# nyrahealth/CrisperWhisper

Measured on AMD Instinct MI355X. Metric: aligned words/s (RTF alongside), CrisperWhisper large-v3 geometry, 30 s chunks, full mel->encoder->decoder->DTW->words path, higher is better.
Workload: dtype bf16

## Files before the change

### crisperwhisper_amd/_native.py

```python
from __future__ import annotations

import ctypes as C
import os

_HERE = os.path.dirname(os.path.abspath(__file__))
LIB_PATH = os.environ.get("CW_LIB_PATH") or os.path.join(_HERE, "libcrisperwhisper.so")

CW_DTYPE_F32, CW_DTYPE_BF16, CW_DTYPE_F16 = 0, 1, 2
N_SAMPLES, N_FRAMES, N_CTX = 480000, 3000, 1500
STAGES = ("mel", "encoder", "cross_kv", "decode", "timestamps")
ALIGN_HEADS_MAX_BYTES = 8 << 30


class NativeLibraryError(RuntimeError):
    pass


class ModelDesc(C.Structure):
    _fields_ = [(n, C.c_int32) for n in (
        "d_model", "n_heads", "ffn_dim", "enc_layers", "dec_layers", "n_mels", "vocab_size",
        "max_target_positions", "median_filter_width", "dtype", "max_batch", "n_align")] + [
        ("align_layers", C.POINTER(C.c_int32)), ("align_heads", C.POINTER(C.c_int32))]


# ... 73 lines not shown
    "cw_get_top_logprobs": (_I, [_P, _P, _P, _I]),
    "cw_get_transcribe_top_logprobs": (_I, [_P, _P, _P, _I, _I]),
    "cw_set_sequence_bias": (_I, [_P, _I, _P, _P, _P]),
    "cw_get_logits": (_I, [_P, _P, _I]),
    "cw_set_logits_capture": (_I, [_P, _P, _I]),
    "cw_get_alignment": (_I, [_P, _P, _I, _I]),
    "cw_resampled_length": (C.c_int64, [C.c_int64, _I, _I]),
    "cw_ingest": (_I, [_P, _P, _I, _I, C.c_int64, _I, _I, _I, _P]),
    "cw_resample_taps": (_I, [_I, _I, _P, _I, _P, _P, _P]),
    "cw_flac_info": (_I, [_P, C.c_int64, _P, _P, _P, _P]),
    "cw_flac_decode": (_I, [_P, C.c_int64, _P, C.c_int64, _P]),
    "cw_flac_last_error": (C.c_char_p, []),
    "cw_token_timestamps": (_I, [_P, _I, _I, _I, _P, _P]),
    "cw_beam_begin": (_I, [_P, _I, _I, _P, _I, _I, _I]),
    "cw_beam_step": (_I, [_P, _I, _P, _P]),
    "cw_beam_advance": (_I, [_P, _P, _P]),
    "cw_beam_finish": (_I, [_P, _I, _I, _P]),
    "cw_transcribe": (_I, [_P, _I, _P, C.POINTER(TranscribeCfg), _P, _P, _P, _I, _P]),
    "cw_transcribe_prompted": (_I, [_P, _I, _P, C.POINTER(TranscribeCfg), _P, _I, _P, _P, _P, _I, _P]),
    "cw_align_tokens": (_I, [_P, _I, _P, _P, _I, _P, _I, _P]),
    "cw_align_prefill_runs": (_I, [_P]),
    "cw_align_heads": (_I, [_P, _I, _P, _P, _I, _P, _I, _I, _P, _P, _P, _P, _P, _I, _P]),
    "cw_align_heads_times": (_I, [_P, _P]),
    "cw_test_align_similarity": (_I, [_P, _P, _I, _I, _I, _I, _P, _P, _P, _I, _P]),
    "cw_set_alignment_scores": (_I, [_P, _I, _I]),
    "cw_get_alignment_scores": (_I, [_P, _P, _P, _I, _I]),
    "cw_get_transcribe_alignment_scores": (_I, [_P, _P, _P, _I, _I]),
    "cw_test_align_path_scores": (_I, [_P, _P, _I, _I, _I, _I, _P, _P, _I, _P, _P]),
    "cw_score_tokens": (_I, [_P, _I, _I, _P, _I, _P, _I, _P, _P, _P]),
    "cw_align_score_tokens": (_I, [_P, _I, _P, _P, _I, _P, _I, _P, _P, _P, _P]),
    "cw_align_cut_tokens": (_I, [_P, _I, _P, _P, _I, _P, _I, _P, _P, _P, _P, _P, _P, _P, _P, _P]),
    "cw_test_score_head_stop": (_I, [_P, _I, _I, _I, _P, _P, _P, _P, _P, _I, _I, _P, _P, _P, _P]),
    "cw_test_align_cut": (_I, [_P, _I, _I, _P, _P, _P, _P, _P, _P, _P]),
    "cw_score_prefill_runs": (_I, [_P]),
    "cw_set_score_top_logprobs": (_I, [_P, _I]),
    "cw_get_score_top_logprobs": (_I, [_P, _P, _P, _I, _I]),
    "cw_test_score_head_top": (_I, [_P, _I, _I, _I, _P, _P, _P, _P, _P, _I, _P, _P, _P, _P, _P, _P]),
    "cw_test_score_head_stop_top": (_I, [_P, _I, _I, _I, _P, _P, _P, _P, _P, _I, _I, _I, _P, _P, _P, _P, _P, _P, _P]),
    "cw_test_score_rows_top": (_I, [_P, _I, _I, _I, _P, _P, _I, _I, _I, _P, _P, _P, _P, _P, _P]),
    "cw_time_score_head_top": (_I, [_P, _I, _I, _I, _I, _P]),
    "cw_align_matrix": (_I, [_P, _P, _I, _I, _I, _I, _P, _I, _P]),
    "cw_dtw": (_I, [_P, _P, _I, _I, _P, _P, _P]),
    "cw_adjust_pauses": (_I, [_P, _P, _P, _I, C.c_double]),
    "cw_vocab_create": (_P, [_I, _P, _P, _P, _P, _I, _I, _I, _I, _I]),
    "cw_vocab_destroy": (None, [_P]),
    "cw_collate_begin": (_P, [_P, C.c_double]),
    "cw_beam_host_new": (_P, [_I, _I, _I, _I, _I, _I, _I, C.c_double, _I, _P]),
    "cw_beam_host_step": (_I, [_P, _P, _P, _P, _P]),
    "cw_beam_host_result": (_I, [_P, _P, _P, _P]),
    "cw_beam_host_token_logprobs": (_I, [_P, _P]),
    "cw_beam_host_free": (None, [_P]),
    "cw_collate_set_mode": (_I, [_P, _I]),
    "cw_collate_feed": (_I, [_P, _P, _I, _P, _I, _I, C.c_double, C.c_double, C.c_double]),
    "cw_collate_finish": (_I, [_P, _P, _P, _P, _P]),
    "cw_collate_get": (_I, [_P, _P, _P, _P, _P, _P]),
    "cw_collate_token_groups_total": (C.c_int64, [_P]),
    "cw_collate_get_token_groups": (_I, [_P, _P, _P]),
    "cw_collate_get_languages": (_I, [_P, _P]),
    "cw_collate_free": (None, [_P]),
    "cw_set_option": (_I, [_P, C.c_char_p, _I]),
    "cw_test_set_option": (_I, [C.c_char_p, _I]),
    "cw_test_gemm": (_I, [_P, _I, _I, _I, _P, _P, _P, _I, _P]),
    "cw_test_gemm_fp8": (_I, [_P, _I, _I, _I, _P, _P, _P, _I, _P]),
    "cw_test_gemm_epi": (_I, [_P, C.POINTER(GemmEpiArgs)]),
    "cw_test_rownorm": (_I, [_P, _I, _I, _I, _P, _P, _P, _P, _P, _P]),
    "cw_test_gemv": (_I, [_P, _I, _I, _I, _P, _P, _P, _P, _P, _I, _P]),
    "cw_has_experiments": (_I, []),
    "cw_test_skinny": (_I, [_P, _I, _I, _I, _I, _P, _P, _P, _I, _I, _P, _P]),
    "cw_test_attention": (_I, [_P, _I, _I, _I, _P, _P, _P, _P]),
    "cw_test_cross_attention": (_I, [_P, _I, _I, _I, _I, _P, _P, _P, _I, _P, _P, _P, _P]),
    "cw_test_cross_attention_fused": (_I, [_P, _I, _I, _I, _I, _P, _P, _P, _P, _P, _I, _P, _P, _I, _P, _P, _P, _P]),
    "cw_test_fold": (_I, [_P, C.POINTER(FoldArgs)]),
    "cw_test_gemv_stack": (_I, [_P, C.POINTER(GemvStackArgs)]),
    "cw_test_gemv_epi": (_I, [_P, C.POINTER(GemvEpiArgs)]),
    "cw_test_self_attention": (_I, [_P, _I, _I, _I, _I, _P, _P, _P, _P, _I, _P, _I, _I, _I, _I, _P, _P, _P]),
    "cw_test_beam_state": (_I, [_P, _I, _P, _P, _P]),
    "cw_test_prefill_gemm": (_I, [_P, _I, _I, _I, _I, _P, _P, _P, _P]),
    "cw_test_prefill_attention": (_I, [_P, _I, _I, _I, _I, _I, _I, _I, _P, _P, _P, _P]),
    "cw_test_prefill_align_attention": (_I, [_P, _I, _I, _I, _I, _I, _I, _P, _P, _P, _P, _P]),
    "cw_test_score_head": (_I, [_P, _I, _I, _I, _P, _P, _P, _P, _P, _P, _P, _P]),
    "cw_time_score_head": (_I, [_P, _I, _I, _I, _P]),
    "cw_test_beam_topk": (_I, [_P, _I, _P, _P, _I, _I, _I, _I, _P, _P]),
    "cw_test_beam_x": (_I, [_P, _I, _P]),
    "cw_test_sample": (_I, [_P, _I, _P, _P, _I, _I, _I, _I, _P]),
    "cw_test_sample_seeded": (_I, [_P, _I, _P, _P, _I, _I, _I, _I, C.c_float, C.c_uint64, _P, _P]),
    "cw_test_sample_logprobs": (_I, [_P, _I, _P, _P, _I, _I, _I, _I, C.c_float, C.c_uint64, _P, _P, _P, _P]),
    "cw_test_sample_top_logprobs": (_I, [_P, _I, _P, _P, _I, _I, _I, _I, C.c_float, C.c_uint64, _P, _P, _I, _P, _P, _P, _P]),
    "cw_test_sample_biased": (_I, [_P, _I, _P, _P, _I, _I, _I, _I, C.c_float, C.c_uint64, _P, _P, _I, _I, _P, _P, _P, _P, _P, _P, _P, _P]),
    "cw_stage_times": (_I, [_P, _P, _P, _I]),
    "cw_time_kernel": (_I, [_P, _I, _I, _I, _P, _P]),
    "cw_time_decode_stage": (_I, [_P, _I, _I, _I, _P, _P, _P, _P]),
    "cw_decode_stage_name": (C.c_char_p, [_I]),
    "cw_handoff_fallbacks": (_I, [_P]),
    "cw_handoff_resumes": (_I, [_P]),
    "cw_decode_stage_launches": (_I, [_P, _I]),
}

_lib = None


def exported_symbols():
    return sorted(_SIGS)


def load():
    global _lib
    if _lib is not None:
        return _lib
    if not os.path.exists(LIB_PATH):
        raise NativeLibraryError(
            f"{LIB_PATH} not found: build it with `python -c 'import __graft_entry__ as g; g.build()'` "
            "or `make -C crisperwhisper_amd/csrc` (hipcc, gfx950).  There is no CPU fallback.")
    try:
        lib = C.CDLL(LIB_PATH)
    except OSError as e:
        raise NativeLibraryError(f"cannot load {LIB_PATH}: {e}") from e
    for name, (res, args) in _SIGS.items():
        try:
            fn = getattr(lib, name)
        except AttributeError as e:
            raise NativeLibraryError(f"{LIB_PATH} does not export {name}") from e
        fn.restype = res
        fn.argtypes = args
    _lib = lib
    return lib
```

### crisperwhisper_amd/csrc/decfuse.hip

```cpp
#include "common.h"
#include "kernels.h"

namespace CW_NS {

typedef __attribute__((ext_vector_type(4))) unsigned int u32x4_t;
__device__ static inline f32x4_t mfma16x(bf16x8_t a, bf16x8_t b, f32x4_t c) { return cw_mfma_16x16x32(a, b, c); }

__global__ __launch_bounds__(256) void fold_product_kernel(const float* __restrict__ A, const float* __restrict__ s,
                                                           float scale, const float* __restrict__ B, int N, int J, int K,
                                                           bf16_t* __restrict__ C) {
    __shared__ float As[16][65];
    __shared__ float Bs[16][64];
    const int tid = threadIdx.x, tx = tid & 15, ty = tid >> 4;
    const int n0 = blockIdx.y * 64, k0 = blockIdx.x * 64;
    float acc[4][4] = {};
    for (int j0 = 0; j0 < J; j0 += 16) {
#pragma unroll
        for (int i = 0; i < 4; ++i) {
            const int idx = tid + 256 * i;
            const int n = idx >> 4, j = idx & 15;
            As[j][n] = A[(size_t)(n0 + n) * J + j0 + j] * (s ? s[j0 + j] : 1.0f) * scale;
            const int jb = idx >> 6, k = idx & 63;
            Bs[jb][k] = B[(size_t)(j0 + jb) * K + k0 + k];
        }
// ... 203 lines not shown
        const int r = tid >> 6;
        const float v = red[((0 * NT + t) * 4 + r) * 64 + lane] + red[((1 * NT + t) * 4 + r) * 64 + lane] +
                        red[((2 * NT + t) * 4 + r) * 64 + lane] + red[((3 * NT + t) * 4 + r) * 64 + lane];
        const int m = g * 4 + r, n = nloc[t];
        if (m < Mb && n >= 0) {
            const size_t o = (size_t)m * ldo + n;
            const float back = wsum ? smean[m] * wsum_v[t] : 0.f;
            if (epi == 0) {
                out[o] = v + bias_v[t] + back;
            } else if (epi == 2) {
                atomicAdd(out + o, v + bias_v[t] + back);
            } else {
                const float rv = resid_pre[t] + resid_grid(v + bias_v[t]);
                out[o] = rv;
                if (out2) out2[o] = rv;
                ps1 += rv; ps2 += rv * rv;
            }
        }
    }
    if (epi == 1 && pstats) {
#pragma unroll
        for (int sft = 0; sft < 4; ++sft) {
            ps1 += sft == 0 ? dpp_mov<0x111, 0xf>(0.f, ps1) : sft == 1 ? dpp_mov<0x112, 0xf>(0.f, ps1) : sft == 2 ? dpp_mov<0x114, 0xf>(0.f, ps1) : dpp_mov<0x118, 0xf>(0.f, ps1);
            ps2 += sft == 0 ? dpp_mov<0x111, 0xf>(0.f, ps2) : sft == 1 ? dpp_mov<0x112, 0xf>(0.f, ps2) : sft == 2 ? dpp_mov<0x114, 0xf>(0.f, ps2) : dpp_mov<0x118, 0xf>(0.f, ps2);
        }
        const int m = g * 4 + (tid >> 6);
        if (l15 == 15) *(float2*)(pstats + ((size_t)(bid - block0) * 16 + m) * 2) = make_float2(ps1, ps2);
    }
}

template <int RPW, int NT>
static int launch_stack_nt(StackParams& p, hipStream_t st) {
    int blocks = 0;
    for (int s = 0; s < p.nseg; ++s) {
        if (p.seg[s].nt <= 0 || p.seg[s].nt > NT) p.seg[s].nt = NT;
        p.seg[s].block0 = blocks;
        blocks += (p.seg[s].n_tiles + p.seg[s].nt - 1) / p.seg[s].nt;
    }
    if (p.zero && (long long)blocks * 256 < p.zero_n4) return CW_ERR_INVALID;
    const size_t lds = (size_t)16 * (p.K + 8) * 2 + (size_t)4 * NT * 4 * 64 * 4 + 16 * 4;
    const dim3 grid(blocks, (p.Mb + 15) / 16);
    if (p.K > 0xffff || p.Mb > 0xff || blocks > 0xffff) return CW_ERR_INVALID;
#define CW_STACK_LEAD(p)                                                                                                     \
    (p).W, (p).zero, (p).zero_n4, (unsigned)(p).K | (unsigned)(p).Mb << 16 | (unsigned)(p).nseg << 24 | ((p).wpk ? 1u << 26 : 0u), \
        (unsigned)((p).nseg > 1 ? (p).seg[1].block0 : 0) | (unsigned)((p).nseg > 2 ? (p).seg[2].block0 : 0) << 16, (p)
    if (p.K <= 256) hipLaunchKernelGGL((gemv_stack_kernel<RPW, 1, 1, NT>), grid, dim3(256), lds, st, CW_STACK_LEAD(p));
    else if (p.K <= 768) hipLaunchKernelGGL((gemv_stack_kernel<RPW, 2, 3, NT>), grid, dim3(256), lds, st, CW_STACK_LEAD(p));
    else {
        bool uni = p.wpk != 0;
        for (int s = 0; s < p.nseg; ++s) uni = uni && p.seg[s].nt == NT;
        if (uni && p.wnt && grid.y == 1) hipLaunchKernelGGL((gemv_stack_kernel<RPW, 3, 5, NT, true, true>), grid, dim3(256), lds, st, CW_STACK_LEAD(p));
        else if (uni) hipLaunchKernelGGL((gemv_stack_kernel<RPW, 3, 5, NT, true>), grid, dim3(256), lds, st, CW_STACK_LEAD(p));
        else hipLaunchKernelGGL((gemv_stack_kernel<RPW, 3, 5, NT>), grid, dim3(256), lds, st, CW_STACK_LEAD(p));
    }
#undef CW_STACK_LEAD
    return CW_OK;
}

int cw_launch_gemv_stack(const StackParams& p_in, int nt, hipStream_t st) {
    StackParams p = p_in;
    if (p.Mb < 1 || p.Mb > 64 || p.K % 128 || p.K > 1280 || p.nseg < 1 || p.nseg > 3) return CW_ERR_INVALID;
    if (nt <= 0) {
        nt = 1;
        for (;;) {
            int blocks = 0;
            for (int s = 0; s < p.nseg; ++s) {
                const int snt = p.seg[s].nt > 0 && p.seg[s].nt < nt ? p.seg[s].nt : nt;
                blocks += (p.seg[s].n_tiles + snt - 1) / snt;
            }
            if (blocks <= 256 || nt == 3) break;
            ++nt;
        }
    }
    if (p.Mb > 8) {
        if (nt == 1) return launch_stack_nt<4, 1>(p, st);
        if (nt == 2) return launch_stack_nt<4, 2>(p, st);
        return launch_stack_nt<4, 3>(p, st);
    }
    if (nt == 1) return launch_stack_nt<2, 1>(p, st);
    if (nt == 2) return launch_stack_nt<2, 2>(p, st);
    return launch_stack_nt<2, 3>(p, st);
}

#ifdef CW_EXPERIMENTS
#include "decfuse_experiments.inc"
#else
int cw_launch_gemv_fc2x(const Fc2xParams&, hipStream_t) { return CW_ERR_INVALID; }
int cw_launch_mlp_pair(const MlpPairParams&, hipStream_t) { return CW_ERR_INVALID; }
int cw_launch_rows_prep(const float*, int, int, void*, float*, int, hipStream_t) { return CW_ERR_INVALID; }
int cw_launch_gemv_rows(int, bool, const RowsParams&, hipStream_t) { return CW_ERR_INVALID; }
#endif

}
```

### crisperwhisper_amd/csrc/declayer.hip

```cpp
#include "common.h"
#include "kernels.h"
#include <mutex>

namespace CW_NS {

typedef __attribute__((ext_vector_type(4))) unsigned int dl_u32x4_t;
typedef unsigned long long dl_u64_t;

#define DL_THREADS 1024
#define DL_SPIN_LIMIT (1 << 17)

#if defined(CW_PHASE_TIMING) && !defined(CW_F16)
__device__ unsigned long long g_dl_phase[256 * 3 * 16];
#define DLPH(i)                                                                                                     \
    do {                                                                                                            \
        if ((threadIdx.x & 63) == 0 && blockIdx.x < 256) {                                                          \
            const int w_ = threadIdx.x >> 6;                                                                        \
            if (w_ == 0 || w_ == 4 || w_ == 8) g_dl_phase[(blockIdx.x * 3 + (w_ >> 2)) * 16 + (i)] = wall_clock64(); \
        }                                                                                                           \
    } while (0)
extern "C" int cw_debug_dl_phases(unsigned long long* out) {
    return (int)hipMemcpyFromSymbol(out, HIP_SYMBOL(g_dl_phase), sizeof(unsigned long long) * 256 * 3 * 16);
}
#define DLPHV(i, v)                                                                                                 \
// ... 324 lines not shown
                    }
                }
            }
#pragma unroll
            for (int r = 0; r < 4; ++r) red[(wave * 4 + r) * 64 + lane] = acc[r];
        }
        dl_chain_sync(cb, 2, lane);
        DLPH(6);
        {
            const int r = wave;
            const float v = red[(0 * 4 + r) * 64 + lane] + red[(1 * 4 + r) * 64 + lane] + red[(2 * 4 + r) * 64 + lane] + red[(3 * 4 + r) * 64 + lane];
            const int m = g * 4 + r;
            float ps1 = 0.f, ps2 = 0.f;
            if (m < Mb) {
                const size_t o = (size_t)m * K + ncl;
                const float back = wsum ? smean[m] * wsum_v : 0.f;
                if (si < 2) {
                    dl_gran_st(p.gq + ((size_t)si * 16 + m) * K + ncl, tag, __float_as_uint(v + bias_v + back));
                } else {
                    const float rv = resid_v + resid_grid(v + bias_v);
                    p.x1[o] = rv;
                    ps1 += rv; ps2 += rv * rv;
                }
            }
            if (si == 2) {
#pragma unroll
                for (int sft = 0; sft < 4; ++sft) {
                    ps1 += sft == 0 ? dpp_mov<0x111, 0xf>(0.f, ps1) : sft == 1 ? dpp_mov<0x112, 0xf>(0.f, ps1) : sft == 2 ? dpp_mov<0x114, 0xf>(0.f, ps1) : dpp_mov<0x118, 0xf>(0.f, ps1);
                    ps2 += sft == 0 ? dpp_mov<0x111, 0xf>(0.f, ps2) : sft == 1 ? dpp_mov<0x112, 0xf>(0.f, ps2) : sft == 2 ? dpp_mov<0x114, 0xf>(0.f, ps2) : dpp_mov<0x118, 0xf>(0.f, ps2);
                }
                if (l15 == 15) {
                    dl_gran_st(p.gps + ((size_t)tl * 16 + m) * 2, tag, __float_as_uint(ps1));
                    dl_gran_st(p.gps + ((size_t)tl * 16 + m) * 2 + 1, tag, __float_as_uint(ps2));
                }
            }
        }
    }
    DLPH(7);
    {
        const size_t col = (size_t)qh * 64 + lane;
        const dl_u64_t* ga = p.gq + ((size_t)0 * 16 + qb_row) * K + col;
        const dl_u64_t* gb = p.gq + ((size_t)1 * 16 + qb_row) * K + col;
        const dl_u64_t* g0 = p.gps + ((size_t)min(lane, TD - 1) * 16 + qb_row) * 2;
        const dl_u64_t* g1 = p.gps + ((size_t)min(lane + 64, TD - 1) * 16 + qb_row) * 2;
        dl_u64_t va = 0, vb = 0, v00 = 0, v01 = 0, v10 = 0, v11 = 0;
        bool ready = !q_mine;
        int npoll = 0; (void)npoll;
#pragma unroll 1
        for (int spins = 0; !ready; ++spins) {
            if (spins > DL_SPIN_LIMIT) { if (lane == 0) atomicCAS(p.err, 0, 1); break; }
            va = dl_gran_ld(ga); vb = dl_gran_ld(gb);
            v00 = dl_gran_ld(g0); v01 = dl_gran_ld(g0 + 1);
            v10 = dl_gran_ld(g1); v11 = dl_gran_ld(g1 + 1);
            const bool ok = (unsigned)(va >> 32) == tag && (unsigned)(vb >> 32) == tag && (unsigned)(v00 >> 32) == tag &&
                            (unsigned)(v01 >> 32) == tag && (unsigned)(v10 >> 32) == tag && (unsigned)(v11 >> 32) == tag;
            ready = __all(ok); ++npoll;
            if (spins == 0) DLPH(8);
        }
        if (q_mine) {
            const float qa1 = __uint_as_float((unsigned)va), qb1 = __uint_as_float((unsigned)vb);
            const float inv_d = 1.0f / (float)(H * 64);
            const float ps1 = (lane < TD ? __uint_as_float((unsigned)v00) : 0.f) + (lane + 64 < TD ? __uint_as_float((unsigned)v10) : 0.f);
            const float ps2 = (lane < TD ? __uint_as_float((unsigned)v01) : 0.f) + (lane + 64 < TD ? __uint_as_float((unsigned)v11) : 0.f);
            const float mean = wave_sum(ps1) * inv_d;
            const float var = fmaxf(wave_sum(ps2) * inv_d - mean * mean, 0.f);
            const float rstd = 1.0f / sqrtf(var + 1e-5f);
            c_q[wave * 64 + lane] = ((qa1 + qb1) - mean * qw1) * rstd + qc1;
        }
        DLPHV(13, npoll);
    }
    DLPH(9);
    dl_barrier();
    DLPH(10);
#pragma unroll
    for (int idx = 0; idx < 16; ++idx) {
        const uint4 t = *(const uint4*)(kvL + ((size_t)(wave * 16 + idx) * 64 + lane) * 16);
        if ((idx >> 2) & 1) vr[idx >> 3][idx & 3].a = t; else kr[idx >> 3][idx & 3].a = t;
    }
    dl_cross_items(p, it, kr, vr, grp, gw, gt, lane, c_q, c_smax, c_redl, c_red);
}
#undef DL_KV_LOAD
#endif

#define QS_THREADS 512
#define QS_GROUPS (QS_THREADS / 8)
#define QS_PRE 2

template <int NSLOT, int PER_LANE, bool WNT>
__global__ __launch_bounds__(QS_THREADS) void qkv_self_kernel(const float* __restrict__ x, const void* __restrict__ Wp,
                                                              const float* __restrict__ bias, void* sk, void* sv,
                                                              const int* __restrict__ pos, unsigned dims, int cap, QkvSelfParams p) {
    extern __shared__ __attribute__((aligned(16))) unsigned char qsm[];
    const int Mb = (int)(dims & 0xffu), H = (int)((dims >> 8) & 0xffu), K = (int)(dims >> 16), N = 3 * K;
    const int xs_stride = K + 8;
    bf16_t* xs = (bf16_t*)qsm;
    float* red = (float*)(qsm + (size_t)16 * xs_stride * 2);
    float* s_q = red + 4 * 4 * 64;
    bf16_t* s_kn = (bf16_t*)(s_q + 64);
    bf16_t* s_vn = s_kn + 64;
    float* dsm = (float*)(s_vn + 64);
    const int tid = threadIdx.x, lane = tid & 63;
    const int wave = __builtin_amdgcn_readfirstlane(tid >> 6);
    const int l15 = lane & 15, g = lane >> 4;
    const int bid = blockIdx.x;
    const int n0 = bid * 16;
    const int steps = K >> 7, nvec = K >> 2;
    const int nn = n0 + l15, ncl = nn < N ? nn : N - 1;

    const int n_items = Mb * H;
    const bool has_item = bid < n_items;
    const int ih = has_item ? bid % H : 0, ib = has_item ? bid / H : 0;
    const int sub = tid & 7, grp = tid >> 3;
    const bf16_t* Kh = (const bf16_t*)sk + ((size_t)ib * H + ih) * cap * 64;
    const bf16_t* Vh = (const bf16_t*)sv + ((size_t)ib * H + ih) * cap * 64;

    float bias_v = 0.f;
    int pos_m = 0;
    float4 xv[2][PER_LANE];
    dl_u32x4_t wq[NSLOT][4];
    if (wave < 4) {
        pos_m = pos[min(g * 4 + wave, Mb - 1)];
        bias_v = bias ? bias[ncl] : 0.f;
#pragma unroll
        for (int i = 0; i < 2; ++i) {
            int row = wave + 4 * i;
            row = row < Mb ? row : Mb - 1;
#pragma unroll
            for (int c = 0; c < PER_LANE; ++c) {
                int v4 = lane + 64 * c;
                v4 = v4 < nvec ? v4 : nvec - 1;
                xv[i][c] = *(const float4*)(x + (size_t)row * K + v4 * 4);
            }
        }
        const bf16_t* __restrict__ W = (const bf16_t*)Wp;
#pragma unroll
        for (int s = 0; s < NSLOT; ++s) {
            int step = wave + 4 * s;
            step = step < steps ? step : steps - 1;
            const dl_u32x4_t* wp = (const dl_u32x4_t*)(W + ((((size_t)(ncl >> 4) * (K >> 5)) + step * 4) * 64 + g * 16 + (ncl & 15)) * 8);
#pragma unroll
            for (int j = 0; j < 4; ++j) wq[s][j] = WNT ? CW_STREAM_LD(wp + j * 64) : wp[j * 64];
        }
    }
    __builtin_amdgcn_sched_barrier(0);
    DlRaw8 kpre[QS_PRE], vpre[QS_PRE];
#pragma unroll
    for (int u = 0; u < QS_PRE; ++u) kpre[u].ld(Kh + (size_t)min(grp + u * QS_GROUPS, cap - 1) * 64 + sub * 8);
#pragma unroll
    for (int u = 0; u < QS_PRE; ++u) vpre[u].ld(Vh + (size_t)min(grp + u * QS_GROUPS, cap - 1) * 64 + sub * 8);
    const int n_keys = pos[ib] + 1;
    const int pos0 = pos[0];
    __builtin_amdgcn_sched_barrier(0);
    const unsigned tag = (p.epoch[0] << 6) | (unsigned)p.layer;
    asm volatile("" : "+v"(pos_m));

    if (wave < 4) {
#pragma unroll
        for (int i = 0; i < 2; ++i) {
            float sx = 0.f;
#pragma unroll
            for (int c = 0; c < PER_LANE; ++c) {
                const float ok = (lane + 64 * c < nvec) ? 1.f : 0.f;
                sx += ok * ((xv[i][c].x + xv[i][c].y) + (xv[i][c].z + xv[i][c].w));
            }
            const float mean = wave_sum(sx) / (float)K;
            float q = 0.f;
#pragma unroll
            for (int c = 0; c < PER_LANE; ++c) {
                const float ok = (lane + 64 * c < nvec) ? 1.f : 0.f;
                const float a = xv[i][c].x - mean, b = xv[i][c].y - mean, cc = xv[i][c].z - mean, d = xv[i][c].w - mean;
                q += ok * cw_sumsq4(a, b, cc, d);
            }
            const float rstd = 1.0f / sqrtf(wave_sum(q) / (float)K + 1e-5f);
            const int row = wave + 4 * i;
#pragma unroll
            for (int c = 0; c < PER_LANE; ++c) {
// ... 52 lines not shown
        const dl_u64_t* gkp = p.gkv + ((size_t)(lane >> 5) * 16 + ib) * (K >> 1) + ih * 32 + (lane & 31);
        dl_u64_t vq = 0, vk = 0;
        bool ready = false;
        const int give_up_tag = pos0 + 1;
        const bool forced_fail = p.fail_pos >= 0 && pos0 == p.fail_pos && p.layer == 0;
#pragma unroll 1
        for (int spins = 0; !ready; ++spins) {
            if (forced_fail || spins > DL_SPIN_LIMIT || ((spins & 255) == 255 && __hip_atomic_load(p.err, __ATOMIC_RELAXED, __HIP_MEMORY_SCOPE_AGENT) != 0)) {
                if (lane == 0) atomicCAS(p.err, 0, give_up_tag);
                if (forced_fail) { vq = 0x3f800000ull; vk = 0; }
                break;
            }
            vq = dl_gran_ld(gqp); vk = dl_gran_ld(gkp);
            ready = __all((unsigned)(vq >> 32) == tag && (unsigned)(vk >> 32) == tag);
        }
        s_q[lane] = __uint_as_float((unsigned)vq);
        ((unsigned*)s_kn)[lane] = (unsigned)vk;
    }
    dl_barrier();
    float* sc = dsm;
    float* redd = dsm + ((cap + 63) & ~63);
    float* scratch = redd + QS_GROUPS * 64;
    float qv[8];
#pragma unroll
    for (int e = 0; e < 8; ++e) qv[e] = s_q[sub * 8 + e];
    const int kn = n_keys - 1;
    const uint4 kn_raw = *(const uint4*)(s_kn + sub * 8), vn_raw = *(const uint4*)(s_vn + sub * 8);
#pragma unroll
    for (int u = 0; u < QS_PRE; ++u)
        if (grp + u * QS_GROUPS == kn) { kpre[u].a = kn_raw; vpre[u].a = vn_raw; }

    if (n_keys <= QS_PRE * QS_GROUPS) {
        float* s_max = scratch;
        float* red8 = redd;
        float d[QS_PRE], mxl = -INFINITY;
#pragma unroll
        for (int u = 0; u < QS_PRE; ++u) {
            float kv[8];
            kpre[u].cvt(kv);
            float t = 0.f;
#pragma unroll
            for (int e = 0; e < 8; ++e) t = fmaf(qv[e], kv[e], t);
            t += __shfl_xor(t, 1, 64); t += __shfl_xor(t, 2, 64); t += __shfl_xor(t, 4, 64);
            d[u] = (grp + u * QS_GROUPS < n_keys) ? t : -INFINITY;
            mxl = fmaxf(mxl, d[u]);
        }
        mxl = wave_max(mxl);
        if (lane == 0) s_max[wave] = mxl;
        dl_barrier();
        mxl = s_max[0];
#pragma unroll
        for (int w = 1; w < QS_THREADS / 64; ++w) mxl = fmaxf(mxl, s_max[w]);
        float acc[8] = {};
        float lsum = 0.f;
#pragma unroll
        for (int u = 0; u < QS_PRE; ++u) {
            if (grp + u * QS_GROUPS < n_keys) {
                const float pk = expf(d[u] - mxl);
                if (sub == 0) lsum += pk;
                float vv[8];
                vpre[u].cvt(vv);
#pragma unroll
                for (int e = 0; e < 8; ++e) acc[e] = fmaf(pk, vv[e], acc[e]);
            }
        }
#pragma unroll
        for (int e = 0; e < 8; ++e) {
            float v = acc[e] + dpp_mov<0x128, 0xf>(0.f, acc[e]);
            acc[e] = xor32_sum(xor16_sum(v));
        }
        lsum = wave_sum(lsum);
        if (lane < 8) {
#pragma unroll
            for (int e = 0; e < 8; ++e) red8[wave * 64 + sub * 8 + e] = acc[e];
        }
        if (lane == 0) red8[8 * 64 + wave] = lsum;
        dl_barrier();
        if (tid < 64) {
            float r = 0.f, l = 0.f;
#pragma unroll
            for (int w = 0; w < QS_THREADS / 64; ++w) { r += red8[w * 64 + tid]; l += red8[8 * 64 + w]; }
            r *= 1.0f / l;
            p.out[(size_t)ib * H * 64 + ih * 64 + tid] = r;
        }
        return;
    }

    float mx = -INFINITY;
#pragma unroll
    for (int u = 0; u < QS_PRE; ++u) {
        const int k = grp + u * QS_GROUPS;
        float kv[8];
        kpre[u].cvt(kv);
        float d = 0.f;
#pragma unroll
        for (int e = 0; e < 8; ++e) d = fmaf(qv[e], kv[e], d);
        d += __shfl_xor(d, 1, 64); d += __shfl_xor(d, 2, 64); d += __shfl_xor(d, 4, 64);
        if (k < n_keys) {
            if (sub == 0) sc[k] = d;
            mx = fmaxf(mx, d);
        }
    }
    for (int k0 = grp + QS_PRE * QS_GROUPS; k0 < n_keys; k0 += 4 * QS_GROUPS) {
        float kv[4][8];
#pragma unroll
        for (int u = 0; u < 4; ++u) {
            const int k = min(k0 + u * QS_GROUPS, n_keys - 1);
            uint4 raw = *(const uint4*)(Kh + (size_t)k * 64 + sub * 8);
            if (k == kn) raw = kn_raw;
            h16_unpack8(raw, kv[u]);
        }
#pragma unroll
        for (int u = 0; u < 4; ++u) {
            const int k = k0 + u * QS_GROUPS;
            if (k < n_keys) {
                float d = 0.f;
#pragma unroll
                for (int e = 0; e < 8; ++e) d = fmaf(qv[e], kv[u][e], d);
                d += __shfl_xor(d, 1, 64); d += __shfl_xor(d, 2, 64); d += __shfl_xor(d, 4, 64);
                if (sub == 0) sc[k] = d;
                mx = fmaxf(mx, d);
            }
        }
    }
    mx = block_max(mx, scratch);
    float sum = 0.f;
    for (int k = tid; k < n_keys; k += QS_THREADS) { float e = expf(sc[k] - mx); sc[k] = e; sum += e; }
    sum = block_sum(sum, scratch);
    const float inv = 1.0f / sum;
    float acc[8] = {};
#pragma unroll
    for (int u = 0; u < QS_PRE; ++u) {
        const int k = grp + u * QS_GROUPS;
        float vv[8];
        vpre[u].cvt(vv);
        const float pk = (k < n_keys) ? sc[k] * inv : 0.f;
        if (k < n_keys) {
#pragma unroll
            for (int e = 0; e < 8; ++e) acc[e] = fmaf(pk, vv[e], acc[e]);
        }
    }
    for (int k0 = grp + QS_PRE * QS_GROUPS; k0 < n_keys; k0 += 4 * QS_GROUPS) {
        float vv[4][8];
#pragma unroll
        for (int u = 0; u < 4; ++u) {
            const int k = min(k0 + u * QS_GROUPS, n_keys - 1);
            uint4 raw = *(const uint4*)(Vh + (size_t)k * 64 + sub * 8);
            if (k == kn) raw = vn_raw;
            h16_unpack8(raw, vv[u]);
        }
#pragma unroll
        for (int u = 0; u < 4; ++u) {
            const int k = k0 + u * QS_GROUPS;
            if (k < n_keys) {
                const float pk = sc[k] * inv;
#pragma unroll
                for (int e = 0; e < 8; ++e) acc[e] = fmaf(pk, vv[u][e], acc[e]);
            }
        }
    }
#pragma unroll
    for (int e = 0; e < 8; ++e) redd[grp * 64 + sub * 8 + e] = acc[e];
    __syncthreads();
    if (tid < 64) {
        float r = 0.f;
        for (int gI = 0; gI < QS_GROUPS; ++gI) r += redd[gI * 64 + tid];
        p.out[(size_t)ib * H * 64 + ih * 64 + tid] = r;
    }
}

int cw_qkv_self_blocks_per_cu(int D, int cap) {
    const size_t lds = (size_t)16 * (D + 8) * 2 + (size_t)(4 * 4 * 64 + 64) * 4 + 2 * 64 * 2 + ((size_t)((cap + 63) & ~63) + QS_GROUPS * 64 + 64) * 4;
    const int by_lds = (int)((size_t)160 * 1024 / lds), by_threads = 2048 / QS_THREADS;
    return by_lds < by_threads ? by_lds : by_threads;
}

int cw_launch_qkv_self(const QkvSelfParams& p, hipStream_t st) {
    const int D = p.D;
    if (p.Mb < 1 || p.Mb > 8 || D % 128 || D > 1280 || p.H * 64 != D || p.cap < 1 || p.cap > 512) return CW_ERR_INVALID;
    if (p.Mb * p.H > 3 * (D / 16) || !p.gq || !p.gkv || !p.epoch || !p.err || !p.W || !p.x || !p.pos) return CW_ERR_INVALID;
    if (p.layer < 0 || p.layer >= 64) return CW_ERR_INVALID;
    const size_t lds = (size_t)16 * (D + 8) * 2 + (size_t)(4 * 4 * 64 + 64) * 4 + 2 * 64 * 2 +
                       ((size_t)((p.cap + 63) & ~63) + QS_GROUPS * 64 + 64) * 4;
    const dim3 grid(3 * (D / 16));
#define QS_LAUNCH_P(NS, PL, NTL)                                                                                            \
    do {                                                                                                                     \
        static std::once_flag attr;                                                                                          \
        std::call_once(attr, [] { (void)hipFuncSetAttribute((const void*)qkv_self_kernel<NS, PL, NTL>, hipFuncAttributeMaxDynamicSharedMemorySize, 100 * 1024); }); \
        hipLaunchKernelGGL((qkv_self_kernel<NS, PL, NTL>), grid, dim3(QS_THREADS), lds, st, p.x, p.W, p.bias, p.sk, p.sv, p.pos, \
                           (unsigned)p.Mb | (unsigned)p.H << 8 | (unsigned)D << 16, p.cap, p);                                \
    } while (0)
#define QS_LAUNCH(NS, PL) do { if (p.wnt) QS_LAUNCH_P(NS, PL, true); else QS_LAUNCH_P(NS, PL, false); } while (0)
    if (D <= 256) QS_LAUNCH(1, 1);
    else if (D <= 768) QS_LAUNCH(2, 3);
    else QS_LAUNCH(3, 5);
#undef QS_LAUNCH
#undef QS_LAUNCH_P
    return CW_OK;
}

#ifdef CW_EXPERIMENTS
template <int NS1, int PL1, int NS2>
__global__ __launch_bounds__(256) void mlp_chain_kernel(MlpChainParams p) {
    extern __shared__ __attribute__((aligned(16))) unsigned char msm[];
    const int tid = threadIdx.x, lane = tid & 63;
    const int wave = __builtin_amdgcn_readfirstlane(tid >> 6);
    const int l15 = lane & 15, g = lane >> 4;
    const int D = p.D, F = p.F, Mb = p.Mb;
    const int n1 = F >> 5;
    const unsigned tag = (p.epoch[0] << 6) | (unsigned)p.layer;
    const int bid = blockIdx.x;
    constexpr int NT = 2;
    if (bid < n1) {
        DLPH(0);
        const int K = D, N = F;
        const int xs_stride = K + 8;
        bf16_t* xs = (bf16_t*)msm;
        float* red = (float*)(msm + (size_t)16 * xs_stride * 2);
        const int n0 = bid * 16 * NT;
        const int steps = K >> 7, nvec = K >> 2;
        int nn[NT], ncl[NT];
#pragma unroll
        for (int t = 0; t < NT; ++t) { nn[t] = n0 + t * 16 + l15; ncl[t] = nn[t] < N ? nn[t] : N - 1; }
        float bias_v[NT];
#pragma unroll
        for (int t = 0; t < NT; ++t) bias_v[t] = p.b1 ? p.b1[ncl[t]] : 0.f;
        float4 xv[2][PL1];
#pragma unroll
        for (int i = 0; i < 2; ++i) {
            int row = wave + 4 * i;
            row = row < Mb ? row : Mb - 1;
#pragma unroll
            for (int c = 0; c < PL1; ++c) {
                int v4 = lane + 64 * c;
                v4 = v4 < nvec ? v4 : nvec - 1;
                xv[i][c] = *(const float4*)(p.x + (size_t)row * K + v4 * 4);
            }
        }
        dl_u32x4_t wq[NT][NS1][4];
        const bf16_t* __restrict__ W = (const bf16_t*)p.W1;
#pragma unroll
        for (int t = 0; t < NT; ++t) {
#pragma unroll
            for (int s = 0; s < NS1; ++s) {
                int step = wave + 4 * s;
                step = step < steps ? step : steps - 1;
                const dl_u32x4_t* wp = (const dl_u32x4_t*)(W + ((((size_t)(ncl[t] >> 4) * (K >> 5)) + step * 4) * 64 + g * 16 + (ncl[t] & 15)) * 8);
#pragma unroll
                for (int j = 0; j < 4; ++j) wq[t][s][j] = wp[j * 64];
            }
        }
        DLPH(1);
#pragma unroll
        for (int i = 0; i < 2; ++i) {
            float sx = 0.f;
#pragma unroll
            for (int c = 0; c < PL1; ++c) {
                const float ok = (lane + 64 * c < nvec) ? 1.f : 0.f;
                sx += ok * ((xv[i][c].x + xv[i][c].y) + (xv[i][c].z + xv[i][c].w));
            }
            const float mean = wave_sum(sx) / (float)K;
            float q = 0.f;
#pragma unroll
            for (int c = 0; c < PL1; ++c) {
                const float ok = (lane + 64 * c < nvec) ? 1.f : 0.f;
                const float a = xv[i][c].x - mean, b = xv[i][c].y - mean, cc = xv[i][c].z - mean, d = xv[i][c].w - mean;
                q += ok * cw_sumsq4(a, b, cc, d);
            }
            const float rstd = 1.0f / sqrtf(wave_sum(q) / (float)K + 1e-5f);
#pragma unroll
            for (int c = 0; c < PL1; ++c) {
                xv[i][c].x = (xv[i][c].x - mean) * rstd; xv[i][c].y = (xv[i][c].y - mean) * rstd;
                xv[i][c].z = (xv[i][c].z - mean) * rstd; xv[i][c].w = (xv[i][c].w - mean) * rstd;
            }
        }
// ... 229 lines not shown
```

### crisperwhisper_amd/csrc/engine.hip

```cpp
#include "engine_internal.h"

static thread_local char g_err[512] = "";

int fail(cw_ctx* c, int code, const char* fmt, ...) {
    va_list ap;
    va_start(ap, fmt);
    vsnprintf(c ? c->err : g_err, 512, fmt, ap);
    va_end(ap);
    if (c) c->err_set = true;
    return code;
}
int fail_ctx(cw_ctx* c, int code, const char* call, const char* file, int line) {
    if (c && c->err_set) return code;
    return fail(c, code, "%s -> %d (%s:%d)", call, code, file, line);
}

int upload_T(cw_ctx* c, void* dst, size_t off, const float* src, size_t n, float scale) {
    if (c->bf16) {
        std::vector<bf16_t> tmp(n);
        if (c->f16) for (size_t i = 0; i < n; ++i) tmp[i] = cw_host_f32_to_f16(src[i] * scale);
        else for (size_t i = 0; i < n; ++i) tmp[i] = cw_host_f32_to_bf16(src[i] * scale);
        HIPCHK(c, hipMemcpy((bf16_t*)dst + off, tmp.data(), n * 2, hipMemcpyHostToDevice));
    } else if (scale != 1.0f) {
        std::vector<float> tmp(n);
// ... 52 lines not shown
#pragma unroll
                for (int u = 0; u < 8; ++u) v[u] = *(const unsigned int*)(base + ((s + u * nthr) << 6));
#pragma unroll
                for (int u = 0; u < 8; ++u) acc ^= v[u];
            }
            for (; s < sectors; s += nthr) acc ^= *(const unsigned int*)(base + (s << 6));
        }
    }
    if (acc == 0x9e3779b9u && sink) *sink = acc;
}


#endif

extern "C" {

int32_t cw_abi_version(void) { return 1; }

const char* cw_last_error(cw_ctx* ctx) {
    if (!ctx) return g_err;
    ctx->err_set = false;
    return ctx->err;
}

int32_t cw_sync(cw_ctx* c) {
    HIPCHK(c, hipStreamSynchronize(c->st));
    return CW_OK;
}

static int create_impl(cw_ctx* c) {
    const cw_model_desc& d = c->d;
    const int D = d.d_model, H = d.n_heads, F = d.ffn_dim, V = d.vocab_size, Bm = d.max_batch;
    if (D != H * 64) return fail(c, CW_ERR_INVALID, "head_dim must be 64 (d_model=%d heads=%d)", D, H);
    if (D % 128 || F % 128 || d.n_mels % 64) return fail(c, CW_ERR_INVALID, "d_model/ffn must be multiples of 128, n_mels of 64");
    if (Bm < 1 || Bm > 64) return fail(c, CW_ERR_INVALID, "max_batch must be in 1..64");
    if (d.max_target_positions > 512) return fail(c, CW_ERR_INVALID, "max_target_positions > 512 unsupported");
    HIPCHK(c, hipSetDevice(c->device));
    HIPCHK(c, hipStreamCreate(&c->st));
    HIPCHK(c, hipEventCreate(&c->ev0));
    HIPCHK(c, hipEventCreate(&c->ev1));
    HIPCHK(c, hipEventCreateWithFlags(&c->ev_step[0], hipEventDisableTiming));
    HIPCHK(c, hipEventCreateWithFlags(&c->ev_step[1], hipEventDisableTiming));
#ifdef CW_EXPERIMENTS
    HIPCHK(c, hipStreamCreateWithFlags(&c->st2, hipStreamNonBlocking));
    HIPCHK(c, hipEventCreateWithFlags(&c->ev_pf[0], hipEventDisableTiming));
    HIPCHK(c, hipEventCreateWithFlags(&c->ev_pf[1], hipEventDisableTiming));
#endif
    HIPCHK(c, hipHostMalloc((void**)&c->h_nunf, 2 * 1024 * sizeof(int), hipHostMallocDefault));
    if (d.dtype != CW_DTYPE_F32 && d.dtype != CW_DTYPE_BF16 && d.dtype != CW_DTYPE_F16) return fail(c, CW_ERR_INVALID, "unknown dtype %d", d.dtype);
    c->f16 = d.dtype == CW_DTYPE_F16;
    c->bf16 = d.dtype == CW_DTYPE_BF16 || c->f16;
    const cw_sw::Switches sw = cw_sw::read_switches();
#ifndef CW_EXPERIMENTS
    {
        const struct { const char* name; bool set; } rejected[] = {{"CW_ROWS_LN", sw.rows_ln}, {"CW_FUSE_MLP", sw.fuse_mlp}, {"CW_MLP_PAIR", sw.mlp_pair},
                                                                   {"CW_SKINNY", sw.skinny != 0}, {"CW_PREFETCH", sw.prefetch != 0},
                                                                   {"CW_DECLAYER", sw.declayer}, {"CW_MLP_CHAIN", sw.mlp_chain}};
        for (const auto& r : rejected)
            if (r.set)
                return fail(c, CW_ERR_INVALID, "%s selects a measured-and-rejected kernel variant that is not in this build: make EXTRA=-DCW_EXPERIMENTS", r.name);
    }
#endif
    c->use_graph = !sw.no_graph;
    c->fuse_rows = !sw.no_fuse_rows;
    c->fuse_rows8 = !sw.no_fuse_rows8;
    c->fuse_beam = !sw.no_fuse_beam;
    c->own_cols = !sw.no_own_cols;
    c->short_hist_enabled = !sw.no_short_hist;
    c->fold_enabled = !sw.no_ln_fold;
    c->fuse6_enabled = !sw.no_fuse6;
    c->rows_ln_enabled = sw.rows_ln;
    c->rows_hilo = !sw.no_rows_hilo;
    c->skinny_mode = sw.skinny;
    c->stack_center = !sw.no_stack_center;
    c->mid16 = !sw.no_mid16;
    c->dtw_block = sw.dtw_block;
    c->fuse_mlp = sw.fuse_mlp;
    c->wpack_enabled = !sw.no_wpack;
    c->wnt = !sw.no_wnt;
    c->mlp_pair = sw.mlp_pair;
    c->mlp_pair_fence = sw.mlp_pair_fence;
    c->declayer = sw.declayer;
    c->qkv_self = !sw.no_qkv_self;
    c->mlp_chain = sw.mlp_chain;
    c->stack_nt3 = sw.stack_nt3;
    c->stack_nt5 = sw.stack_nt5;
    c->prefetch = sw.prefetch;
    c->esz = c->bf16 ? 2 : 4;
    c->Bm = Bm;
    c->S_pad = 1536;
    const size_t e = c->esz;
    const int TGT = d.max_target_positions;

    CWCHK(c, dmalloc(c, &c->conv1_w, (size_t)D * 3 * d.n_mels * e));
    CWCHK(c, dmalloc(c, &c->conv2_w, (size_t)D * 3 * D * e));
    CWCHK(c, dmalloc(c, &c->conv1_b, (size_t)D * 4));
    CWCHK(c, dmalloc(c, &c->conv2_b, (size_t)D * 4));
    CWCHK(c, dmalloc(c, &c->enc_pos, (size_t)CW_N_CTX * D * 4));
    CWCHK(c, dmalloc(c, &c->dec_pos, (size_t)TGT * D * 4));
    CWCHK(c, dmalloc(c, &c->embed, (size_t)V * D * e));
    CWCHK(c, dmalloc(c, &c->enc_ln_g, D * 4)); CWCHK(c, dmalloc(c, &c->enc_ln_b, D * 4));
    CWCHK(c, dmalloc(c, &c->dec_ln_g, D * 4)); CWCHK(c, dmalloc(c, &c->dec_ln_b, D * 4));
    c->enc.resize(d.enc_layers);
    c->dec.resize(d.dec_layers);
    auto alloc_common = [&](LayerW& L, bool stacked) -> int {
        CWCHK(c, dmalloc(c, &L.wqkv, (size_t)3 * D * D * e)); CWCHK(c, dmalloc(c, &L.bqkv, (size_t)3 * D * 4));
        if (!stacked) CWCHK(c, dmalloc(c, &L.wo, (size_t)D * D * e));
        CWCHK(c, dmalloc(c, &L.bo, D * 4));
        CWCHK(c, dmalloc(c, &L.ln1_g, D * 4)); CWCHK(c, dmalloc(c, &L.ln1_b, D * 4));
        if (!stacked) CWCHK(c, dmalloc(c, &L.w1, (size_t)F * D * e));
        CWCHK(c, dmalloc(c, &L.b1, F * 4));
        CWCHK(c, dmalloc(c, &L.w2, (size_t)D * F * e)); CWCHK(c, dmalloc(c, &L.b2, D * 4));
        CWCHK(c, dmalloc(c, &L.ln2_g, D * 4)); CWCHK(c, dmalloc(c, &L.ln2_b, D * 4));
        return CW_OK;
    };
    for (auto& L : c->enc) CWCHK(c, alloc_common(L, false));
    for (auto& L : c->dec) {
        const bool stacked = c->bf16;
        CWCHK(c, alloc_common(L, stacked));
        if (stacked) {
            CWCHK(c, dmalloc(c, &L.ws3, (size_t)3 * D * D * e));
            CWCHK(c, dmalloc(c, &L.ws5, ((size_t)2 * F + D) * D * e));
            L.wq_c = L.ws3; L.wo = (char*)L.ws3 + (size_t)2 * D * D * e;
            L.w1 = L.ws5;   L.wo_c = (char*)L.ws5 + (size_t)2 * F * D * e;
            CWCHK(c, dmalloc(c, &L.qa_bias, D * 4)); CWCHK(c, dmalloc(c, &L.q_wsum, D * 4));
            CWCHK(c, dmalloc(c, &L.u1_bias, F * 4)); CWCHK(c, dmalloc(c, &L.u1_wsum, F * 4));
            CWCHK(c, dmalloc(c, &L.qkv_wsum, (size_t)3 * D * 4));
        } else {
            CWCHK(c, dmalloc(c, &L.wq_c, (size_t)D * D * e));
            CWCHK(c, dmalloc(c, &L.wo_c, (size_t)D * D * e));
        }
        CWCHK(c, dmalloc(c, &L.bq_c, D * 4));
        CWCHK(c, dmalloc(c, &L.wkv_c, (size_t)2 * D * D * e)); CWCHK(c, dmalloc(c, &L.bkv_c, (size_t)2 * D * 4));
        CWCHK(c, dmalloc(c, &L.bo_c, D * 4));
        CWCHK(c, dmalloc(c, &L.lnc_g, D * 4)); CWCHK(c, dmalloc(c, &L.lnc_b, D * 4));
        CWCHK(c, dmalloc(c, &L.ck, (size_t)Bm * H * CW_N_CTX * 64 * e));
        CWCHK(c, dmalloc(c, &L.cv, (size_t)Bm * H * CW_N_CTX * 64 * e));
        CWCHK(c, dmalloc(c, &L.sk, (size_t)Bm * H * TGT * 64 * e));
        CWCHK(c, dmalloc(c, &L.sv, (size_t)Bm * H * TGT * 64 * e));
    }

    {
        std::vector<double> ct(400), sn(400), win(400);
        for (int i = 0; i < 400; ++i) {
            ct[i] = cos(2.0 * M_PI * i / 400.0);
            sn[i] = sin(2.0 * M_PI * i / 400.0);
            win[i] = (double)(float)(0.5 - 0.5 * cos(2.0 * M_PI * i / 400.0));
        }
        double *dct, *dsn, *dwin;
        CWCHK(c, dmalloc(c, &dct, 400 * 8)); CWCHK(c, dmalloc(c, &dsn, 400 * 8)); CWCHK(c, dmalloc(c, &dwin, 400 * 8));
        HIPCHK(c, hipMemcpy(dct, ct.data(), 400 * 8, hipMemcpyHostToDevice));
        HIPCHK(c, hipMemcpy(dsn, sn.data(), 400 * 8, hipMemcpyHostToDevice));
        HIPCHK(c, hipMemcpy(dwin, win.data(), 400 * 8, hipMemcpyHostToDevice));
        const int nm = d.n_mels, nb = 201;
        auto hz2mel = [](double f) { return f >= 1000.0 ? 15.0 + log(f / 1000.0) * (27.0 / log(6.4)) : 3.0 * f / 200.0; };
        auto mel2hz = [](double m) { return m >= 15.0 ? 1000.0 * exp((log(6.4) / 27.0) * (m - 15.0)) : 200.0 * m / 3.0; };
        std::vector<double> ff(nm + 2);
        const double m_lo = hz2mel(0.0), m_hi = hz2mel(8000.0);
        for (int i = 0; i < nm + 2; ++i) {
            double step = (m_hi - m_lo) / (nm + 1);
            double mv = (i == nm + 1) ? m_hi : m_lo + step * i;
            ff[i] = mel2hz(mv);
        }
        std::vector<float> fb((size_t)nb * nm);
        for (int k = 0; k < nb; ++k) {
            double fk = (k == nb - 1) ? 8000.0 : (8000.0 / (nb - 1)) * k;
            for (int m = 0; m < nm; ++m) {
                double down = -(ff[m] - fk) / (ff[m + 1] - ff[m]);
                double up = (ff[m + 2] - fk) / (ff[m + 2] - ff[m + 1]);
                double v = fmax(0.0, fmin(down, up));
                v *= 2.0 / (ff[m + 2] - ff[m]);
                fb[(size_t)k * nm + m] = (float)v;
            }
        }
        float* dfb;
        CWCHK(c, dmalloc(c, &dfb, fb.size() * 4));
        HIPCHK(c, hipMemcpy(dfb, fb.data(), fb.size() * 4, hipMemcpyHostToDevice));
        c->mel.cos_t = dct; c->mel.sin_t = dsn; c->mel.window = dwin; c->mel.filters = dfb;
        {
            std::vector<int> lo(nm, nb), hi(nm, -1);
            for (int m = 0; m < nm; ++m)
                for (int k = 0; k < nb; ++k)
                    if (fb[(size_t)k * nm + m] != 0.f) { if (k < lo[m]) lo[m] = k; if (k > hi[m]) hi[m] = k; }
            int *dlo, *dhi;
            CWCHK(c, dmalloc(c, &dlo, nm * 4)); CWCHK(c, dmalloc(c, &dhi, nm * 4));
            HIPCHK(c, hipMemcpy(dlo, lo.data(), nm * 4, hipMemcpyHostToDevice));
            HIPCHK(c, hipMemcpy(dhi, hi.data(), nm * 4, hipMemcpyHostToDevice));
            c->mel.fb_lo = dlo; c->mel.fb_hi = dhi;
        }
    }
    CWCHK(c, dmalloc(c, &c->d_pcm, (size_t)Bm * CW_N_SAMPLES * 4));
    CWCHK(c, dmalloc(c, &c->d_logspec, (size_t)Bm * CW_N_FRAMES * d.n_mels * 4));
    CWCHK(c, dmalloc(c, &c->d_gmax, Bm * 4));
    CWCHK(c, dmalloc(c, &c->d_feats_tm, (size_t)Bm * CW_N_FRAMES * d.n_mels * e));
    c->n_frames_items.assign(Bm, CW_N_FRAMES);

    const size_t MR = (size_t)Bm * CW_N_CTX;
    CWCHK(c, dmalloc(c, &c->c1, (size_t)Bm * CW_N_FRAMES * D * e));
    CWCHK(c, dmalloc(c, &c->x, MR * D * 4));
    CWCHK(c, dmalloc(c, &c->h, MR * D * e));
    CWCHK(c, dmalloc(c, &c->ao, MR * D * e));
    CWCHK(c, dmalloc(c, &c->enc_out, MR * D * e));
    CWCHK(c, dmalloc(c, &c->mid, MR * F * e));
    CWCHK(c, dmalloc(c, &c->qb, (size_t)Bm * H * c->S_pad * 64 * e));
    CWCHK(c, dmalloc(c, &c->kb, (size_t)Bm * H * c->S_pad * 64 * e));
    CWCHK(c, dmalloc(c, &c->vb, (size_t)Bm * H * c->S_pad * 64 * e));
    CWCHK(c, dmalloc(c, &c->d_row_off, Bm * 4)); CWCHK(c, dmalloc(c, &c->d_row_valid, Bm * 4));
    CWCHK(c, dmalloc(c, &c->d_row_off2, Bm * 4)); CWCHK(c, dmalloc(c, &c->d_row_valid2, Bm * 4));
    {
        std::vector<int> off2(Bm), val2(Bm, CW_N_FRAMES);
        for (int i = 0; i < Bm; ++i) off2[i] = i * CW_N_FRAMES;
        HIPCHK(c, hipMemcpy(c->d_row_off2, off2.data(), Bm * 4, hipMemcpyHostToDevice));
        HIPCHK(c, hipMemcpy(c->d_row_valid2, val2.data(), Bm * 4, hipMemcpyHostToDevice));
    }

    CWCHK(c, dmalloc(c, &c->dx, (size_t)Bm * D * 4)); CWCHK(c, dmalloc(c, &c->dxn, (size_t)Bm * D * 4));
    CWCHK(c, dmalloc(c, &c->dq, (size_t)Bm * D * 4)); CWCHK(c, dmalloc(c, &c->dattn, (size_t)Bm * D * 4));
    CWCHK(c, dmalloc(c, &c->dmid, (size_t)Bm * F * 4));
    CWCHK(c, dmalloc(c, &c->dx1, (size_t)Bm * D * 4)); CWCHK(c, dmalloc(c, &c->dx2c, (size_t)Bm * D * 4));
    CWCHK(c, dmalloc(c, &c->d_qa, (size_t)2 * Bm * D * 4)); c->d_qb = c->d_qa + (size_t)Bm * D;
    CWCHK(c, dmalloc(c, &c->d_u1, (size_t)Bm * F * 4)); CWCHK(c, dmalloc(c, &c->d_pstats, (size_t)128 * 64 * 2 * 4));
    CWCHK(c, dmalloc(c, &c->d_rstats, (size_t)((D > F ? D : F) / 16 + 1) * 64 * 2 * 4));
    CWCHK(c, dmalloc(c, &c->d_bar, 64 * 4));
    {
        CWCHK(c, dmalloc(c, &c->d_gq, (size_t)2 * 16 * D * 8)); CWCHK(c, dmalloc(c, &c->d_gps, (size_t)(D / 16) * 16 * 2 * 8));
        CWCHK(c, dmalloc(c, &c->d_gq2, (size_t)16 * D * 8)); CWCHK(c, dmalloc(c, &c->d_gkv, (size_t)2 * 16 * (D / 2) * 8));
        CWCHK(c, dmalloc(c, &c->d_gflag, (size_t)512 * 8));
        CWCHK(c, dmalloc(c, &c->d_epoch, 4));
        const unsigned int one = 1;
        HIPCHK(c, hipMemcpy(c->d_epoch, &one, 4, hipMemcpyHostToDevice));
        hipDeviceProp_t prop;
        HIPCHK(c, hipGetDeviceProperties(&prop, c->device));
        c->n_cu = prop.multiProcessorCount;
    }
    CWCHK(c, dmalloc(c, &c->d_xfrag, (size_t)64 * 5120 * 2));
#ifdef CW_EXPERIMENTS
    if (Bm > 16) {
        c->planes_cap = (size_t)4 * 64 * (3 * D > F ? 3 * D : F);
        CWCHK(c, dmalloc(c, &c->d_planes, c->planes_cap * 4, false));
        CWCHK(c, dmalloc(c, &c->d_sk_stats, (size_t)16 * 64 * 2 * 4));
    }
#endif
    CWCHK(c, dmalloc(c, &c->d_xfrag2, (size_t)64 * 5120 * 2));
    CWCHK(c, dmalloc(c, &c->d_cvec, 64 * 4)); CWCHK(c, dmalloc(c, &c->d_ostats, (size_t)96 * 64 * 2 * 4));
    c->Vpad = (V + 3) & ~3;
    CWCHK(c, dmalloc(c, &c->dlogits, (size_t)Bm * c->Vpad * 4));
    CWCHK(c, dmalloc(c, &c->d_ids, (size_t)Bm * TGT * 4)); CWCHK(c, dmalloc(c, &c->d_forced, (size_t)Bm * TGT * 4));
    CWCHK(c, dmalloc(c, &c->d_argmax, (size_t)Bm * TGT * 4));
    CWCHK(c, dmalloc(c, &c->d_last_ts, Bm * 4)); CWCHK(c, dmalloc(c, &c->d_finished, Bm * 4));
    CWCHK(c, dmalloc(c, &c->d_nunf, 8));
    c->d_err = c->d_nunf + 1;
#ifdef CW_EXPERIMENTS
    CWCHK(c, dmalloc(c, &c->d_pf_sink, 4));
#endif
    CWCHK(c, dmalloc(c, &c->d_pos, 64 * 4)); CWCHK(c, dmalloc(c, &c->d_cfg, 4 * 4));
    CWCHK(c, dmalloc(c, &c->d_mask, (size_t)V + 16));
    CWCHK(c, dmalloc(c, &c->d_sample_part, (size_t)Bm * 16 * 32));
    CWCHK(c, dmalloc(c, &c->d_sample_pert, (size_t)Bm * 16 * 16));
    CWCHK(c, dmalloc(c, &c->d_samp, (size_t)(4 + 2 * Bm) * 4));
    c->samp_host.assign((size_t)4 + 2 * Bm, 0u);
    CWCHK(c, dmalloc(c, &c->d_lp_sum, (size_t)Bm * 4)); CWCHK(c, dmalloc(c, &c->d_lp_cnt, (size_t)Bm * 4));
    CWCHK(c, dmalloc(c, &c->d_align_slot, (size_t)d.dec_layers * H * 4));
    {
        std::vector<int> slot((size_t)d.dec_layers * H, -1);
        for (int a = 0; a < d.n_align; ++a) {
            int l = c->align_layers[a], hh = c->align_heads[a];
            if (l < 0 || l >= d.dec_layers || hh < 0 || hh >= H) return fail(c, CW_ERR_INVALID, "bad alignment head (%d,%d)", l, hh);
            slot[(size_t)l * H + hh] = a;
        }
        HIPCHK(c, hipMemcpy(c->d_align_slot, slot.data(), slot.size() * 4, hipMemcpyHostToDevice));
    }
    const int Ha = d.n_align > 0 ? d.n_align : 1;
    c->align_rows = TGT;
    CWCHK(c, dmalloc(c, &c->d_align, (size_t)Bm * Ha * TGT * CW_N_CTX * 4));
    CWCHK(c, dmalloc(c, &c->d_part_o, (size_t)ATT_NS * Bm * D * 4));
    CWCHK(c, dmalloc(c, &c->d_part_ml, (size_t)Bm * H * ATT_NS * 2 * 4));
    CWCHK(c, dmalloc(c, &c->d_align_ml, (size_t)Bm * Ha * TGT * ATT_NS * 2 * 4));

    CWCHK(c, dmalloc(c, &c->d_mean, (size_t)Bm * Ha * CW_N_CTX * 4));
    CWCHK(c, dmalloc(c, &c->d_std, (size_t)Bm * Ha * CW_N_CTX * 4));
    CWCHK(c, dmalloc(c, &c->d_mat, (size_t)Bm * TGT * CW_N_CTX * 4));
    CWCHK(c, dmalloc(c, &c->d_trace, (size_t)Bm * TGT * CW_N_CTX));
    CWCHK(c, dmalloc(c, &c->d_first_col, (size_t)Bm * TGT * 4));
    CWCHK(c, dmalloc(c, &c->d_path_text, (size_t)Bm * (TGT + CW_N_CTX + 2) * 4));
    CWCHK(c, dmalloc(c, &c->d_path_time, (size_t)Bm * (TGT + CW_N_CTX + 2) * 4));
    CWCHK(c, dmalloc(c, &c->d_path_len, Bm * 4));
    CWCHK(c, dmalloc(c, &c->d_ncols, Bm * 4));
    HIPCHK(c, hipDeviceSynchronize());
    return CW_OK;
}

cw_ctx* cw_create(const cw_model_desc* desc, int32_t device) {
    if (!desc) { fail(nullptr, CW_ERR_INVALID, "null desc"); return nullptr; }
    cw_ctx* c = new cw_ctx();
    c->d = *desc;
    c->device = device;
    c->align_layers.assign(desc->align_layers, desc->align_layers + desc->n_align);
    c->align_heads.assign(desc->align_heads, desc->align_heads + desc->n_align);
    c->d.align_layers = c->align_layers.data();
    c->d.align_heads = c->align_heads.data();
    int r = create_impl(c);
    if (r != CW_OK) {
        snprintf(g_err, sizeof(g_err), "%s", c->err);
        cw_destroy(c);
        return nullptr;
    }
    return c;
}

void cw_destroy(cw_ctx* c) {
// ... 344 lines not shown
        EpiParams ep = epi0(); ep.out = c->c1; ep.bias = c->conv1_b; ep.ldo = D;
        CWCHK(c, KD(c, cw_launch_gemm, bf, EPI_GELU, ap, c->conv1_w, nb * CW_N_FRAMES, D, 3 * NM, ep, c->st));
    }
    {
        AParams ap{c->c1, 0, 1, S, D, 2, c->d_row_off2, c->d_row_valid2};
        EpiParams ep = epi0(); ep.outf = c->x; ep.bias = c->conv2_b; ep.ldo = D; ep.pos = c->enc_pos; ep.T = S;
        CWCHK(c, KD(c, cw_launch_gemm, bf, EPI_GELU_POS_F32, ap, c->conv2_w, nb * S, D, 3 * D, ep, c->st));
    }
    const int M = nb * S;
    for (int l = 0; l < c->d.enc_layers; ++l) {
        LayerW& L = c->enc[l];
        if (c->enc8_mask & 1) CWCHK(c, KD(c, cw_launch_layernorm_fp8, c->x, L.ln1_g, L.ln1_b, c->h8, c->sa8, M, D, c->st));
        else CWCHK(c, KD(c, cw_launch_layernorm, bf, c->x, L.ln1_g, L.ln1_b, c->h, M, D, c->st));
        {
            AParams ap{c->h, D, 0, 0, 0, 0, nullptr, nullptr};
            EpiParams ep = epi0(); ep.out = c->qb; ep.out1 = c->kb; ep.out2 = c->vb; ep.bias = L.bqkv;
            ep.T = S; ep.S_pad = c->S_pad; ep.H = H; ep.d_model = D;
            if (c->enc8_mask & 1) CWCHK(c, KD(c, cw_launch_gemm_fp8, EPI_HEADS, c->h8, D, L.wqkv8, M, 3 * D, D, c->sa8, L.sqkv, ep, c->st));
            else CWCHK(c, KD(c, cw_launch_gemm, bf, EPI_HEADS, ap, L.wqkv, M, 3 * D, D, ep, c->st));
        }
        CWCHK(c, KD(c, cw_launch_attn_encoder, bf, c->qb, c->kb, c->vb, c->ao, nb, H, S, c->S_pad, c->st));
        {
            AParams ap{c->ao, D, 0, 0, 0, 0, nullptr, nullptr};
            EpiParams ep = epi0(); ep.outf = c->x; ep.resid = c->x; ep.bias = L.bo; ep.ldo = D;
            CWCHK(c, KD(c, cw_launch_gemm, bf, EPI_RESID_F32, ap, L.wo, M, D, D, ep, c->st));
        }
        if (c->enc8_mask & 2) CWCHK(c, KD(c, cw_launch_layernorm_fp8, c->x, L.ln2_g, L.ln2_b, c->h8, c->sa8, M, D, c->st));
        else CWCHK(c, KD(c, cw_launch_layernorm, bf, c->x, L.ln2_g, L.ln2_b, c->h, M, D, c->st));
        {
            AParams ap{c->h, D, 0, 0, 0, 0, nullptr, nullptr};
            EpiParams ep = epi0(); ep.out = c->mid; ep.bias = L.b1; ep.ldo = F;
            if (c->enc8_mask & 2) CWCHK(c, KD(c, cw_launch_gemm_fp8, EPI_GELU, c->h8, D, L.w18, M, F, D, c->sa8, L.s1, ep, c->st));
            else CWCHK(c, KD(c, cw_launch_gemm, bf, EPI_GELU, ap, L.w1, M, F, D, ep, c->st));
        }
        {
            AParams ap{c->mid, F, 0, 0, 0, 0, nullptr, nullptr};
            EpiParams ep = epi0(); ep.outf = c->x; ep.resid = c->x; ep.bias = L.b2; ep.ldo = D;
            if (c->enc8_mask & 4) {
                CWCHK(c, KD(c, cw_launch_quant_rows_fp8, c->mid, M, F, c->mid8, c->smid8, c->st));
                CWCHK(c, KD(c, cw_launch_gemm_fp8, EPI_RESID_F32, c->mid8, F, L.w28, M, D, F, c->smid8, L.s2, ep, c->st));
            } else CWCHK(c, KD(c, cw_launch_gemm, bf, EPI_RESID_F32, ap, L.w2, M, D, F, ep, c->st));
        }
    }
    CWCHK(c, KD(c, cw_launch_layernorm, bf, c->x, c->enc_ln_g, c->enc_ln_b, c->enc_out, M, D, c->st));
    if (c->enc8_mask & 8) CWCHK(c, KD(c, cw_launch_layernorm_fp8, c->x, c->enc_ln_g, c->enc_ln_b, c->h8, c->sa8, M, D, c->st));
    KCHK(c);
    tm.stop();
    StageTimer tk(c, CW_STAGE_CROSS_KV);
    for (int l = 0; l < c->d.dec_layers; ++l) {
        LayerW& L = c->dec[l];
        AParams ap{c->enc_out, D, 0, 0, 0, 0, nullptr, nullptr};
        EpiParams ep = epi0(); ep.out = L.ck; ep.out1 = L.cv; ep.bias = L.bkv_c;
        ep.T = S; ep.S_pad = S; ep.H = H; ep.d_model = D;
        if (c->enc8_mask & 8) CWCHK(c, KD(c, cw_launch_gemm_fp8, EPI_HEADS, c->h8, D, L.wkv_c8, M, 2 * D, D, c->sa8, L.skv_c, ep, c->st));
        else CWCHK(c, KD(c, cw_launch_gemm, bf, EPI_HEADS, ap, L.wkv_c, M, 2 * D, D, ep, c->st));
        if (c->kv8) CWCHK(c, KD(c, cw_launch_kv_quant_fp8, L.ck, L.cv, L.ck8, L.cv8, L.kvs, nb, H, S, c->st));
    }
    KCHK(c);
    tk.stop();
    c->nb_encoded = nb;
    return CW_OK;
}

int32_t cw_get_encoder_output(cw_ctx* c, float* out, int32_t nb) {
    if (nb < 1 || nb > c->nb_encoded) return fail(c, CW_ERR_STATE, "only %d windows encoded", c->nb_encoded);
    HIPCHK(c, hipStreamSynchronize(c->st));
    return download_T(c, c->enc_out, 0, out, (size_t)nb * CW_N_CTX * c->d.d_model);
}

int gemv_ln(cw_ctx* c, int epi, const float* x, int Mb, int K, const void* W, int N, const float* g,
                   const float* b, const EpiParams& ep) {
    if (c->bf16 || !g) return KD(c, cw_launch_gemv, c->bf16, epi, x, Mb, K, W, N, g, b, ep, c->st, nullptr, (Mb <= 16 || c->wpacked) ? c->d_xfrag : nullptr, c->bf16 && c->wpacked, c->wnt);
    int r = KD(c, cw_launch_layernorm_f32, x, g, b, c->dxn, Mb, K, c->st);
    if (r != CW_OK) return r;
    return KD(c, cw_launch_gemv, false, epi, c->dxn, Mb, K, W, N, nullptr, nullptr, ep, c->st);
}

int launch_logits(cw_ctx* c, int nb, const float* x) {
    EpiParams ep = epi0(); ep.outf = c->dlogits; ep.ldo = c->Vpad;
    return gemv_ln(c, EPI_STORE_F32, x, nb, c->d.d_model, (c->bf16 && c->wpacked) ? c->embed_pk : c->embed, c->d.vocab_size, c->dec_ln_g, c->dec_ln_b, ep);
}

struct StepPlan {
    bool frag, fuse, own, qs, short_hist, mid16; int nt3;
#ifdef CW_EXPERIMENTS
    bool fuse_mlp, mlp_pair, mlp_chain, dl, sk_ok, skinny, xfull, rows, pf; int lo_off;
#else
    static constexpr bool fuse_mlp = false, mlp_pair = false, mlp_chain = false, dl = false, sk_ok = false, skinny = false, xfull = false, rows = false, pf = false;
    static constexpr int lo_off = 0;
#endif
};
static StepPlan plan_step(const cw_ctx* c, int nb) {
    const int D = c->d.d_model, H = c->d.n_heads, F = c->d.ffn_dim, TGT = c->d.max_target_positions;
    StepPlan P{};
    P.frag = c->bf16 && nb > 16 && c->wpacked;
    const bool ab17 = nb > 16 && (c->rows_ln_enabled || c->skinny_mode != 0);
    P.fuse = c->bf16 && c->fuse6_ready && c->fuse6_enabled && c->ln_folded && !ab17 && (nb <= 16 || P.frag) && (nb <= 16 || (c->fuse_rows && nb <= 64 && (!c->kv8 || c->fuse_rows8))) &&
             (c->beam_K == 0 || (c->fuse_beam && !c->kv8 && c->beam_K <= 16 && !c->fuse_mlp)) &&
             (!c->kv8 || (KD(c, cw_cross8_is_mfma, CW_N_CTX) && !c->fuse_mlp)) && !((c->fuse_mlp || c->mlp_pair) && nb > 8);
    P.own = c->own_cols && P.fuse && P.frag && nb > 32 && !c->fuse_mlp && !c->mlp_pair && c->rows_ln_ready && D % 32 == 0 && D / 16 <= 96 && D <= 1536 &&
            D % 128 == 0 && F % 32 == 0;
    P.nt3 = c->stack_nt3 > 0 ? c->stack_nt3 : (nb > 16 ? 2 : 1);
    P.qs = c->qkv_self && c->bf16 && c->ln_folded && c->wpacked && nb <= 8 && c->beam_K == 0 && D <= 1280 && nb * H <= 3 * (D / 16) && TGT <= 512 &&
           c->d.dec_layers <= 64 && 3 * (D / 16) <= c->n_cu * KD(c, cw_qkv_self_blocks_per_cu, D, TGT);
    P.short_hist = c->hist_short && c->short_hist_enabled && nb > 8;
    P.mid16 = P.fuse && !P.frag && F > 1280 && c->mid16;
#ifdef CW_EXPERIMENTS
    P.fuse_mlp = c->fuse_mlp;
    P.mlp_pair = c->mlp_pair && F % D == 0 && D % 32 == 0 && F / 32 <= 256 && F / D <= 32;
    P.mlp_chain = c->mlp_chain && c->wpacked && c->mid16 && nb <= 8 && KD(c, cw_mlp_chain_ok, nb, D, F);
    P.dl = P.fuse && c->declayer && !c->kv8 && !c->fuse_mlp && P.nt3 == 1 && c->wpacked && nb <= 8 && 3 * (D / 16) <= c->n_cu &&
           nb * H * ATT_NS <= 4 * c->n_cu && D / 16 <= 128 && KD(c, cw_dec_layer_lds, D) <= (size_t)160 * 1024;
    P.sk_ok = P.frag && c->wpacked && c->ln_folded && c->rows_ln_ready && c->d_planes;
    P.skinny = P.sk_ok && c->skinny_mode >= 2;
    P.xfull = P.frag && c->skinny_mode >= 1 && c->beam_K == 0 && !c->kv8 && !c->rows_ln_enabled && H <= 20 && CW_N_CTX <= 24 * 64;
    P.rows = !P.skinny && P.frag && c->rows_ln_ready && c->rows_ln_enabled && c->ln_folded && D <= 1280;
    P.lo_off = (c->rows_hilo && !c->f16) ? 64 * (D / 8) : 0;
    P.pf = c->prefetch > 0 && c->bf16 && c->beam_K == 0 && !c->kv8;
#endif
    return P;
}
static int stage_launches(const StepPlan& P, int kind) {
    const bool prepared = kind == DST_QKV || kind == DST_CROSS_Q || kind == DST_FC1 || kind == DST_CROSS_O, owned = P.own && (kind == DST_FC1 || kind == DST_CROSS_O);
    return (P.frag && !P.skinny && !P.rows && !P.xfull && prepared && !owned) ? 2 : 1;
}
static bool stage(cw_ctx* c, const StepPlan& P, int kind) {
    const int s = c->stage_count++;
    if (s < CW_MAX_DEC_STAGES) { c->stage_kind[s] = kind; c->stage_launches[s] = stage_launches(P, kind); }
    return c->stage_sel < 0 || c->stage_sel == s;
}
#define STG(kind, call) do { if (stage(c, P, (kind))) CWCHK(c, call); } while (0)
static EpiParams resid_epi(float* x, const float* bias, int D) { EpiParams ep = epi0(); ep.outf = x; ep.resid = x; ep.bias = bias; ep.ldo = D; return ep; }
EpiParams qkv_epi(cw_ctx* c, LayerW& L) {
    EpiParams ep = epi0(); ep.outf = c->dq; ep.out1 = L.sk; ep.out2 = L.sv; ep.bias = L.bqkv;
    ep.H = c->d.n_heads; ep.S_pad = c->d.max_target_positions; ep.d_model = c->d.d_model; ep.row_pos = c->d_pos;
    return ep;
}
EpiParams cross_q_epi(cw_ctx* c, LayerW& L) { EpiParams ep = epi0(); ep.outf = c->dq; ep.bias = L.bq_c; ep.ldo = c->d.d_model; return ep; }
static EpiParams fc1_epi(cw_ctx* c, LayerW& L) { EpiParams ep = epi0(); ep.outf = c->dmid; ep.out = c->d_xfrag2; ep.bias = L.b1; ep.ldo = c->d.ffn_dim; return ep; }
int gemv_resid(cw_ctx* c, bool frag, const float* a, void* xf, int nb, int K, const void* W, const float* bias, float* x, int x16) {
    const int D = c->d.d_model;
    EpiParams ep = resid_epi(x, bias, D); ep.x16 = x16;
    if (frag) return KD(c, cw_launch_gemv, true, EPI_RESID_F32, nullptr, nb, K, W, D, nullptr, nullptr, ep, c->st, nullptr, xf, c->wpacked);
    return gemv_ln(c, EPI_RESID_F32, a, nb, K, W, D, nullptr, nullptr, ep);
}
static CrossSplitParams cross_params(cw_ctx* c, const StepPlan& P, LayerW& L, int l, int nb, const float* q) {
    const int H = c->d.n_heads;
    CrossSplitParams p{q, L.ck, L.cv, CW_N_CTX, c->d_part_o, c->d_part_ml, c->d.n_align > 0 ? c->d_align : nullptr, c->d_align_ml,
                       c->d_align_slot + (size_t)l * H, c->d_pos, c->d.n_align, c->align_rows, nb, H};
    p.kv_div = c->beam_K > 0 ? c->beam_K : 1;
    if (!q) { p.qa = c->d_qa; p.qb = c->d_qb; p.qw = L.q_wsum; p.qbias = L.bq_c; p.pstats = c->d_pstats; p.n_pstats = (c->d.d_model / 16 + P.nt3 - 1) / P.nt3; }
    return p;
}
int cross_attn(cw_ctx* c, LayerW& L, CrossSplitParams p) {
    if (c->kv8) { p.K = L.ck8; p.V = L.cv8; p.kv_scale = L.kvs; return KD(c, cw_launch_attn_cross_split_fp8, p, c->st); }
    return KD(c, cw_launch_attn_cross_split, true, p, c->st);
}
static int cross_out(cw_ctx* c, const StepPlan& P, LayerW& L, int nb, float* x) {
    const int D = c->d.d_model;
    const CombineParams cb{c->d_part_ml, c->d.n_heads, nb * D};
    return KD(c, cw_launch_gemv, true, EPI_RESID_F32, c->d_part_o, nb, D, L.wo_c, D, nullptr, nullptr, resid_epi(x, L.bo_c, D), c->st, &cb, (nb <= 16 || P.frag) ? c->d_xfrag : nullptr, c->wpacked);
}
static int launch_mlp(cw_ctx* c, const StepPlan& P, LayerW& L, int nb, float* x) {
    const int D = c->d.d_model, F = c->d.ffn_dim;
    STG(DST_FC1, gemv_ln(c, P.frag ? EPI_GELU_FRAG : P.mid16 ? EPI_GELU : EPI_GELU_F32, x, nb, D, L.w1, F, L.ln2_g, c->ln_folded ? nullptr : L.ln2_b, fc1_epi(c, L)));
    STG(DST_FC2, gemv_resid(c, P.frag, P.mid16 ? (const float*)c->d_xfrag2 : c->dmid, c->d_xfrag2, nb, F, L.w2, L.b2, x, P.mid16 ? 1 : 0));
    return CW_OK;
}
static int self_attn(cw_ctx* c, const StepPlan& P, LayerW& L, int nb) {
    DecAttnParams p = dec_attn(c->dq, L.sk, L.sv, c->d.max_target_positions, 0, c->d_pos, c->dattn, nb, c->d.n_heads);
    if (P.frag && !P.fuse) p.out_frag = (unsigned short*)c->d_xfrag2;
    if (c->beam_K > 0) p.anc = c->d_anc;
    p.short_hist = P.short_hist ? 1 : 0;
    return KD(c, cw_launch_attn_decode, c->bf16, p, c->st);
}
static int layer_self_attention(cw_ctx* c, const StepPlan& P, int l, int nb, const float* x) {
    const int D = c->d.d_model, H = c->d.n_heads, TGT = c->d.max_target_positions;
    LayerW& L = c->dec[l];
    if (!P.qs) {
        STG(DST_QKV, gemv_ln(c, EPI_QKV_CACHE, x, nb, D, L.wqkv, 3 * D, L.ln1_g, c->ln_folded ? nullptr : L.ln1_b, qkv_epi(c, L)));
        STG(DST_SELF_ATTN, self_attn(c, P, L, nb));
        return CW_OK;
    }
    QkvSelfParams qp = zeroed<QkvSelfParams>();
    qp.x = x; qp.W = L.wqkv; qp.bias = L.bqkv; qp.sk = L.sk; qp.sv = L.sv; qp.cap = TGT; qp.pos = c->d_pos; qp.out = c->dattn;
    qp.gq = c->d_gq2; qp.gkv = c->d_gkv; qp.epoch = c->d_epoch; qp.layer = l; qp.err = c->d_err; qp.Mb = nb; qp.D = D; qp.H = H; qp.fail_pos = c->fail_pos; qp.wnt = c->wnt ? 1 : 0;
    const int dbg = cw_sw::cw_switches().qkv_self_dbg;
    if (dbg) { qp.q_plain = c->dq; qp.no_attn = 1; }
    STG(DST_QKV_SELF, KD(c, cw_launch_qkv_self, qp, c->st));
    if (dbg) STG(DST_SELF_ATTN, self_attn(c, P, L, nb));
    return CW_OK;
}
static StackParams stack_params(cw_ctx* c, LayerW& L, int nb, const float* xin, float* xalt) {
    const int D = c->d.d_model, TD = D / 16;
    StackParams sp = zeroed<StackParams>();
    sp.W = L.ws3; sp.wpk = c->wpacked ? 1 : 0; sp.wnt = c->wnt ? 1 : 0; sp.K = D; sp.Mb = nb; sp.nseg = 3;
    sp.seg[0].x = xin;      sp.seg[0].bias = L.qa_bias; sp.seg[0].out = c->d_qa; sp.seg[0].tile0 = 0;      sp.seg[0].n_tiles = TD; sp.seg[0].epi = 0;
    sp.seg[0].wsum = c->stack_center ? L.q_wsum : nullptr;
    sp.seg[1].x = c->dattn; sp.seg[1].bias = nullptr;   sp.seg[1].out = c->d_qb; sp.seg[1].tile0 = TD;     sp.seg[1].n_tiles = TD; sp.seg[1].epi = 0;
    sp.seg[2].x = c->dattn; sp.seg[2].bias = L.bo;      sp.seg[2].out = xalt;    sp.seg[2].tile0 = 2 * TD; sp.seg[2].n_tiles = TD; sp.seg[2].epi = 1;
    sp.seg[2].resid = xin; sp.seg[2].pstats = c->d_pstats;
    return sp;
}
static int layer_fused(cw_ctx* c, const StepPlan& P, int l, int nb, float*& xin, float*& xalt) {
    const int D = c->d.d_model, H = c->d.n_heads, F = c->d.ffn_dim;
    LayerW& L = c->dec[l];
    STG(DST_STACK, KD(c, cw_launch_gemv_stack, stack_params(c, L, nb, xin, xalt), P.nt3, c->st));
    const CrossSplitParams p = cross_params(c, P, L, l, nb, nullptr);
    STG(DST_CROSS_ATTN, cross_attn(c, L, p));
    if (P.own) {
        const CombineParams cb{c->d_part_ml, H, nb * D, c->d_pstats, p.n_pstats, c->d_cvec};
        STG(DST_OTHER, KD(c, cw_launch_rows_combine, c->d_part_o, nb, D, cb, c->d_xfrag, c->st));
        STG(DST_CROSS_O, KD(c, cw_launch_gemv_own, c->d_xfrag, nb, D, L.wo_c, D, resid_epi(xalt, L.bo_c, D), c->d_cvec, c->d_xfrag2, c->d_ostats, c->st, c->wpacked));
        EpiParams ep = epi0(); ep.out = c->d_xfrag; ep.bias = L.b1; ep.ldo = F;
        STG(DST_FC1, KD(c, cw_launch_gemv_lna, c->d_xfrag2, nb, D, L.w1, F, ep, c->d_ostats, D / (16 * KD(c, cw_gemv_own_nt, D)), L.u1_wsum, c->st, c->wpacked));
        STG(DST_FC2, gemv_resid(c, true, nullptr, c->d_xfrag, nb, F, L.w2, L.b2, xalt));
    } else {
        STG(DST_CROSS_O, cross_out(c, P, L, nb, xalt));
        CWCHK(c, launch_mlp(c, P, L, nb, xalt));
    }
    std::swap(xin, xalt);
    return CW_OK;
}
static int layer_unfused(cw_ctx* c, const StepPlan& P, int l, int nb) {
    const int D = c->d.d_model, H = c->d.n_heads;
    LayerW& L = c->dec[l];
    STG(DST_O_PROJ, gemv_resid(c, P.frag, c->dattn, c->d_xfrag2, nb, D, L.wo, L.bo, c->dx));
    STG(DST_CROSS_Q, gemv_ln(c, EPI_STORE_F32, c->dx, nb, D, L.wq_c, D, L.lnc_g, c->ln_folded ? nullptr : L.lnc_b, cross_q_epi(c, L)));
    if (c->bf16) {
        STG(DST_CROSS_ATTN, cross_attn(c, L, cross_params(c, P, L, l, nb, c->dq)));
        STG(DST_CROSS_O, cross_out(c, P, L, nb, c->dx));
    } else {
        DecAttnParams p = dec_attn(c->dq, L.ck, L.cv, CW_N_CTX, CW_N_CTX, c->d_pos, c->dattn, nb, H);
        p.align_out = c->d.n_align > 0 ? c->d_align : nullptr; p.align_slot = c->d_align_slot + (size_t)l * H;
        p.n_align = c->d.n_align; p.align_rows = c->align_rows; p.kv_div = c->beam_K > 0 ? c->beam_K : 1;
        STG(DST_CROSS_ATTN, KD(c, cw_launch_attn_decode, c->bf16, p, c->st));
        STG(DST_CROSS_O, gemv_resid(c, false, c->dattn, nullptr, nb, D, L.wo_c, L.bo_c, c->dx));
    }
    return launch_mlp(c, P, L, nb, c->dx);
}
DecLayerParams dec_layer_params(cw_ctx* c, int l, int nb, const float* xin, float* xalt) {
    const int D = c->d.d_model, H = c->d.n_heads, TGT = c->d.max_target_positions;
    LayerW& L = c->dec[l];
    DecLayerParams dp = zeroed<DecLayerParams>();
    dp.Ws = L.ws3; dp.x = xin; dp.a = c->dattn; dp.qa_bias = L.qa_bias; dp.q_wsum = c->stack_center ? L.q_wsum : nullptr;
    dp.bo = L.bo; dp.x1 = xalt;
    dp.K = L.ck; dp.V = L.cv; dp.n_keys = CW_N_CTX; dp.part_o = c->d_part_o; dp.part_ml = c->d_part_ml;
    dp.align_out = c->d.n_align > 0 ? c->d_align : nullptr; dp.align_ml = c->d_align_ml;
    dp.align_slot = c->d_align_slot + (size_t)l * H; dp.pos = c->d_pos; dp.n_align = c->d.n_align; dp.align_rows = c->align_rows;
    dp.qw = L.q_wsum; dp.qbias = L.bq_c;
    dp.gq = c->d_gq; dp.gps = c->d_gps; dp.epoch = c->d_epoch; dp.layer = l; dp.err = c->d_err;
    dp.Mb = nb; dp.D = D; dp.H = H;
    dp.kv_wait = cw_sw::cw_switches().dl_kvwait;
    return dp;
}

#ifdef CW_EXPERIMENTS
static int launch_prefetch_layer(cw_ctx* c, const StepPlan& P, int l, int nb) {
    HIPCHK(c, hipEventRecord(c->ev_pf[0], c->st));
    HIPCHK(c, hipStreamWaitEvent(c->st2, c->ev_pf[0], 0));
    const int D = c->d.d_model, F = c->d.ffn_dim, H = c->d.n_heads;
    const size_t e = c->esz;
    LayerW& L = c->dec[l];
    PrefetchRanges r = zeroed<PrefetchRanges>();
    auto add = [&](const void* p, size_t bytes) { if (p && bytes && r.count < 8) { r.p[r.count] = (const char*)p; r.n[r.count] = bytes; ++r.count; } };
    add(L.wqkv, (size_t)3 * D * D * e);
    if (P.fuse) add(L.ws3, (size_t)3 * D * D * e);
    else { add(L.wo, (size_t)D * D * e); add(L.wq_c, (size_t)D * D * e); }
    add(L.ck, (size_t)nb * H * CW_N_CTX * 64 * e);
    add(L.cv, (size_t)nb * H * CW_N_CTX * 64 * e);
    add(L.wo_c, (size_t)D * D * e);
    add(L.w1, (size_t)F * D * e);
    add(L.w2, (size_t)D * F * e);
    const int wide = cw_sw::cw_switches().prefetch_wide;
    const int what = cw_sw::cw_switches().prefetch_what;
    if (!(what & 1)) { int k = 0; for (int i = 0; i < r.count; ++i) if (r.p[i] == (const char*)L.ck || r.p[i] == (const char*)L.cv) { r.p[k] = r.p[i]; r.n[k] = r.n[i]; ++k; } r.count = k; }
    if (!(what & 2)) { int k = 0; for (int i = 0; i < r.count; ++i) if (r.p[i] != (const char*)L.ck && r.p[i] != (const char*)L.cv) { r.p[k] = r.p[i]; r.n[k] = r.n[i]; ++k; } r.count = k; }
    if (wide) hipLaunchKernelGGL(prefetch_kernel<1>, dim3(c->prefetch), dim3(256), 0, c->st2, r, c->d_pf_sink);
    else hipLaunchKernelGGL(prefetch_kernel<0>, dim3(c->prefetch), dim3(256), 0, c->st2, r, c->d_pf_sink);
    return CW_OK;
}

static int layer_unfused_ab(cw_ctx* c, const StepPlan& P, int l, int nb, int& ln_nblk) {
    const int D = c->d.d_model, H = c->d.n_heads, F = c->d.ffn_dim;
    LayerW& L = c->dec[l];
    auto sk_ln = [&](int epi, const void* W, int N, const float* wsum, const EpiParams& ep) -> int {
        SkinnyParams sp = zeroed<SkinnyParams>();
        sp.x = c->dx; sp.W = W; sp.Mb = nb; sp.K = D; sp.N = N; sp.planes = c->d_planes; sp.stats = c->d_sk_stats;
        int smax = (int)(c->planes_cap / ((size_t)nb * N));
        if (smax > 16) smax = 16;
// ... 1948 lines not shown
    }
    for (auto& L : c->dec) CWCHK(c, KD(c, cw_launch_quant_rows_fp8, L.wkv_c, 2 * D, D, L.wkv_c8, L.skv_c, c->st));
    KCHK(c);
    c->enc8_stale = false;
    return CW_OK;
}

int32_t cw_set_option(cw_ctx* c, const char* name, int32_t value) {
    if (!name) return fail(c, CW_ERR_INVALID, "cw_set_option: null option name");
    if (!strcmp(name, "prompt_prefix")) {
        if (value < 0 || value >= c->d.max_target_positions) return fail(c, CW_ERR_INVALID, "prompt_prefix=%d out of range", value);
        c->pf_prefix = value;
        return CW_OK;
    }
    if (!strcmp(name, "prompt_prefill")) {
        c->prompt_prefill = value != 0;
        return CW_OK;
    }
    if (!strcmp(name, "align_prefill")) {
        c->align_prefill = value != 0;
        return CW_OK;
    }
    if (!strcmp(name, "score_prefill")) {
        c->score_prefill = value != 0;
        return CW_OK;
    }
    if (!strcmp(name, "cross_kv_fp8")) {
        if (!value) { c->kv8 = false; return CW_OK; }
        if (!c->bf16) return fail(c, CW_ERR_INVALID, "cross_kv_fp8 needs the bf16 engine (the f32 engine is the parity mode)");
        if (!c->dec[0].ck8) {
            const size_t n = (size_t)c->Bm * c->d.n_heads * CW_N_CTX * 64;
            const size_t nv = (size_t)c->Bm * cw_bf16::cw_kv8_v_bytes(c->d.n_heads, CW_N_CTX);
            for (auto& L : c->dec) {
                CWCHK(c, dmalloc(c, &L.ck8, n, false)); CWCHK(c, dmalloc(c, &L.cv8, nv, false));
                CWCHK(c, dmalloc(c, &L.kvs, (size_t)c->Bm * c->d.n_heads * 2 * 4));
            }
        }
        c->kv8 = true;
        c->nb_encoded = 0;
        drop_step_graphs(c);
        return CW_OK;
    }
    if (!strcmp(name, "encoder_gemm_fp8")) {
        if (!value) { c->enc8 = false; c->enc8_mask = 0; c->nb_encoded = 0; return CW_OK; }
        if (!c->bf16) return fail(c, CW_ERR_INVALID, "encoder_gemm_fp8 needs a 16-bit engine (the f32 engine is the parity mode)");
        const int D = c->d.d_model, F = c->d.ffn_dim;
        if (D % 256 != 0 || F % 256 != 0 || D > 2048) return fail(c, CW_ERR_INVALID, "encoder_gemm_fp8: d_model / ffn_dim must be multiples of 256 (d_model <= 2048)");
        CWCHK(c, cw_check_weights(c));
        if (!c->h8) {
            const size_t MR = (size_t)c->Bm * CW_N_CTX;
            CWCHK(c, dmalloc(c, &c->h8, MR * D, false)); CWCHK(c, dmalloc(c, &c->mid8, MR * F, false));
            CWCHK(c, dmalloc(c, &c->sa8, MR * 4)); CWCHK(c, dmalloc(c, &c->smid8, MR * 4));
            for (auto& L : c->enc) {
                CWCHK(c, dmalloc(c, &L.wqkv8, (size_t)3 * D * D, false)); CWCHK(c, dmalloc(c, &L.sqkv, (size_t)3 * D * 4));
                CWCHK(c, dmalloc(c, &L.w18, (size_t)F * D, false)); CWCHK(c, dmalloc(c, &L.s1, (size_t)F * 4));
                CWCHK(c, dmalloc(c, &L.w28, (size_t)D * F, false)); CWCHK(c, dmalloc(c, &L.s2, (size_t)D * 4));
            }
            for (auto& L : c->dec) { CWCHK(c, dmalloc(c, &L.wkv_c8, (size_t)2 * D * D, false)); CWCHK(c, dmalloc(c, &L.skv_c, (size_t)2 * D * 4)); }
        }
        CWCHK(c, enc8_quantise(c));
        c->enc8 = true;
        c->enc8_mask = value >= 16 ? ((value - 16) & 15) : 15;
        c->nb_encoded = 0;
        return CW_OK;
    }
#ifndef CW_EXPERIMENTS
    if ((!strcmp(name, "rows_ln") || !strcmp(name, "skinny")) && value != 0)
        return fail(c, CW_ERR_INVALID, "option %s selects a measured-and-rejected kernel variant that is not in this build (make EXTRA=-DCW_EXPERIMENTS)", name);
#endif
    if (!strcmp(name, "test_epoch_forwards")) {
        c->forwards_since_reset = (long long)value;
        return CW_OK;
    }
    if (!strcmp(name, "handoff_fail_pos")) {
        c->fail_pos = value;
        drop_step_graphs(c);
        return CW_OK;
    }
    if (!strcmp(name, "no_wnt")) {
        c->wnt = value == 0;
        drop_step_graphs(c);
        return CW_OK;
    }
    if (!strcmp(name, "rows_ln")) {
        c->rows_ln_enabled = value != 0;
        drop_step_graphs(c);
        return CW_OK;
    }
    if (!strcmp(name, "skinny")) {
        c->skinny_mode = value;
        drop_step_graphs(c);
        return CW_OK;
    }
    return fail(c, CW_ERR_INVALID, "unknown option %s", name);
}

int32_t cw_has_experiments(void) {
#ifdef CW_EXPERIMENTS
    return 1;
#else
    return 0;
#endif
}

}
```

### crisperwhisper_amd/csrc/engine_hooks.hip

```cpp
#include "engine_internal.h"

extern "C" {

static int g_test_no_wnt = 0;
static int g_test_cross_fp8 = 0;
static int g_test_attn_poison_qpad = 0;
int32_t cw_test_set_option(const char* name, int32_t value) {
    if (!strcmp(name, "no_wnt")) { g_test_no_wnt = value; return CW_OK; }
    if (!strcmp(name, "cross_test_fp8")) { g_test_cross_fp8 = value; return CW_OK; }
    if (!strcmp(name, "attn_poison_qpad")) { g_test_attn_poison_qpad = value; return CW_OK; }
    if (!strcmp(name, "gemm256_min_tiles")) { cw_bf16::cw_gemm_set_256_min_tiles(value); cw_f16::cw_gemm_set_256_min_tiles(value); return CW_OK; }
    if (!strcmp(name, "beam_topk_1block")) { cw_bf16::cw_beam_topk_set_1block(value); cw_f16::cw_beam_topk_set_1block(value); return CW_OK; }
    if (!strcmp(name, "gemm_pp")) { cw_bf16::cw_gemm_set_pp(value); cw_f16::cw_gemm_set_pp(value); return CW_OK; }
    if (!strcmp(name, "gemm_8ph")) { cw_bf16::cw_gemm_set_8ph(value); cw_f16::cw_gemm_set_8ph(value); return CW_OK; }
    if (!strcmp(name, "gemm_gm")) {
#ifndef CW_EXPERIMENTS
        return CW_ERR_INVALID;
#endif
        cw_bf16::cw_gemm_set_gm(value); cw_f16::cw_gemm_set_gm(value); return CW_OK;
    }
    if (!strcmp(name, "gemv_loop")) { cw_bf16::cw_gemv_set_loop(value); cw_f16::cw_gemv_set_loop(value); return CW_OK; }
    if (!strcmp(name, "mt_variant")) { cw_bf16::cw_gemv_set_mt_variant(value); cw_f16::cw_gemv_set_mt_variant(value); return CW_OK; }
    if (!strcmp(name, "comb_rowgroups")) { cw_bf16::cw_gemv_set_comb_rowgroups(value); cw_f16::cw_gemv_set_comb_rowgroups(value); return CW_OK; }
    if (!strcmp(name, "gemm_w128")) { cw_bf16::cw_gemm_set_w128(value); cw_f16::cw_gemm_set_w128(value); return CW_OK; }
// ... 1291 lines not shown
    }
    int r = KD(c, cw_launch_attn_decode, c->bf16, p, c->st);
    if (r != CW_OK) return fail(c, r, "test_self_attention: launch rejected");
    { hipError_t er = hipStreamSynchronize(c->st); if (er != hipSuccess) return fail(c, CW_ERR_HIP, "test_self_attention: %s", hipGetErrorString(er)); }
    if (out_frag) {
        std::vector<unsigned short> f((size_t)Mpad * D);
        HIPCHK(c, hipMemcpy(f.data(), dfrag, f.size() * 2, hipMemcpyDeviceToHost));
        for (int b = 0; b < B; ++b)
            for (int j = 0; j < D; ++j) {
                const unsigned short h = f[frag_index(b, j, D)];
                out[(size_t)b * D + j] = c->f16 ? cw_host_f16_to_f32(h) : cw_host_bf16_to_f32(h);
            }
        int ok = 1;
        for (int b = B; b < Mpad; ++b)
            for (int j = 0; j < D; ++j) ok &= f[frag_index(b, j, D)] == 0xA5A5;
        *frag_tail_ok = ok;
    } else {
        HIPCHK(c, hipMemcpy(out, dout, (size_t)B * D * 4, hipMemcpyDeviceToHost));
    }
    if (align_head >= 0) HIPCHK(c, hipMemcpy(align, dal, nal * 4, hipMemcpyDeviceToHost));
    return CW_OK;
}

int32_t cw_test_beam_state(cw_ctx* c, int32_t rows, int32_t* ids, int32_t* anc, int32_t* pos) {
    const int TGT = c->d.max_target_positions;
    if (c->beam_K <= 0 || !c->d_anc) return fail(c, CW_ERR_STATE, "cw_beam_begin not called");
    if (rows < 1 || rows > c->Bm || rows > 64 || !ids || !anc || !pos) return fail(c, CW_ERR_INVALID, "test_beam_state: rows=%d", rows);
    HIPCHK(c, hipStreamSynchronize(c->st));
    HIPCHK(c, hipMemcpy(ids, c->d_ids, (size_t)rows * TGT * 4, hipMemcpyDeviceToHost));
    HIPCHK(c, hipMemcpy(anc, c->d_anc, (size_t)rows * TGT * 4, hipMemcpyDeviceToHost));
    HIPCHK(c, hipMemcpy(pos, c->d_pos, (size_t)rows * 4, hipMemcpyDeviceToHost));
    return CW_OK;
}

int32_t cw_test_beam_topk(cw_ctx* c, int32_t nb, const float* logits, const int32_t* ids, int32_t t, int32_t n_prompt,
                          int32_t min_new_tokens, int32_t n_cand, float* cand_val, int32_t* cand_id) {
    const int V = c->d.vocab_size, TGT = c->d.max_target_positions, Bm = c->Bm;
    if (!logits || !ids || !cand_val || !cand_id) return fail(c, CW_ERR_INVALID, "test_beam_topk: null argument");
    if (!c->gen_set) return fail(c, CW_ERR_STATE, "cw_set_generation not called");
    if (c->beam_K > 0) return fail(c, CW_ERR_STATE, "test_beam_topk: a beam search is open (the hook overwrites its state)");
    if (nb < 1 || nb > Bm || nb > 64) return fail(c, CW_ERR_INVALID, "test_beam_topk: nb=%d outside 1 .. %d", nb, Bm < 64 ? Bm : 64);
    if (n_cand < 1 || n_cand > 64) return fail(c, CW_ERR_INVALID, "test_beam_topk: n_cand=%d outside 1 .. 64", n_cand);
    if (n_prompt < 1 || t < n_prompt || t >= TGT) return fail(c, CW_ERR_INVALID, "test_beam_topk: t=%d / n_prompt=%d out of range", t, n_prompt);
    if (min_new_tokens < 0) return fail(c, CW_ERR_INVALID, "test_beam_topk: min_new_tokens=%d is negative", min_new_tokens);
    std::vector<int> hid((size_t)nb * TGT, c->gen.pad_token_id), posv(nb, t - 1);
    for (int b = 0; b < nb; ++b)
        for (int k = 0; k < t; ++k) {
            const int tok = ids[(size_t)b * t + k];
            if (tok < 0 || tok >= V) return fail(c, CW_ERR_INVALID, "test_beam_topk: token %d out of range", tok);
            hid[(size_t)b * TGT + k] = tok;
        }
    CWCHK(c, beam_alloc(c));
    HIPCHK(c, hipStreamSynchronize(c->st));
    HIPCHK(c, hipMemcpy(c->d_ids, hid.data(), hid.size() * 4, hipMemcpyHostToDevice));
    HIPCHK(c, hipMemcpy(c->d_pos, posv.data(), (size_t)nb * 4, hipMemcpyHostToDevice));
    const int cfg[4] = {n_prompt, min_new_tokens, TGT, 0};
    HIPCHK(c, hipMemcpy(c->d_cfg, cfg, sizeof(cfg), hipMemcpyHostToDevice));
    HIPCHK(c, hipMemcpy2D(c->dlogits, (size_t)c->Vpad * 4, logits, (size_t)V * 4, (size_t)V * 4, nb, hipMemcpyHostToDevice));
    const int n_padcol = c->Vpad - V;
    if (n_padcol > 0) {
        const std::vector<float> hot((size_t)nb * n_padcol, 75.0f);
        HIPCHK(c, hipMemcpy2D(c->dlogits + V, (size_t)c->Vpad * 4, hot.data(), (size_t)n_padcol * 4, (size_t)n_padcol * 4, nb, hipMemcpyHostToDevice));
    }
    HIPCHK(c, hipMemset(c->d_cand_val, 0xff, (size_t)Bm * 64 * 4));
    HIPCHK(c, hipMemset(c->d_cand_id, 0xff, (size_t)Bm * 64 * 4));
    const std::vector<float> poison(KD(c, cw_beam_topk_scratch_floats, Bm), 1e30f);
    HIPCHK(c, hipMemcpy(c->d_topk_scratch, poison.data(), poison.size() * 4, hipMemcpyHostToDevice));
    const int r = launch_beam_topk(c, nb, n_cand);
    if (r != CW_OK) fail(c, r, "test_beam_topk: launch rejected");
    hipError_t er = hipStreamSynchronize(c->st);
    if (er == hipSuccess) er = hipGetLastError();
    if (n_padcol > 0) HIPCHK(c, hipMemset2D(c->dlogits + V, (size_t)c->Vpad * 4, 0, (size_t)n_padcol * 4, nb));
    if (r != CW_OK) return r;
    if (er != hipSuccess) return fail(c, CW_ERR_HIP, "test_beam_topk: %s", hipGetErrorString(er));
    HIPCHK(c, hipMemcpy(cand_val, c->d_cand_val, (size_t)Bm * 64 * 4, hipMemcpyDeviceToHost));
    HIPCHK(c, hipMemcpy(cand_id, c->d_cand_id, (size_t)Bm * 64 * 4, hipMemcpyDeviceToHost));
    return CW_OK;
}

int32_t cw_test_beam_x(cw_ctx* c, int32_t rows, float* x) {
    if (rows < 1 || rows > c->Bm || !x) return fail(c, CW_ERR_INVALID, "test_beam_x: rows=%d", rows);
    HIPCHK(c, hipStreamSynchronize(c->st));
    HIPCHK(c, hipMemcpy(x, c->dx, (size_t)rows * c->d.d_model * 4, hipMemcpyDeviceToHost));
    return CW_OK;
}

static int test_sample(cw_ctx* c, int32_t nb, const float* logits, const int32_t* ids, int32_t t, int32_t n_prompt,
                       int32_t min_new_tokens, int32_t max_length, int32_t* choice_out, const int32_t* forced_tok = nullptr,
                       float* lp_out = nullptr, int32_t* top_id_out = nullptr, float* top_lp_out = nullptr);
int32_t cw_test_sample(cw_ctx* c, int32_t nb, const float* logits, const int32_t* ids, int32_t t, int32_t n_prompt,
                       int32_t min_new_tokens, int32_t max_length, int32_t* choice_out) {
    return test_sample(c, nb, logits, ids, t, n_prompt, min_new_tokens, max_length, choice_out);
}
int32_t cw_test_sample_seeded(cw_ctx* c, int32_t nb, const float* logits, const int32_t* ids, int32_t t, int32_t n_prompt,
                              int32_t min_new_tokens, int32_t max_length, float temperature, uint64_t seed,
                              const uint64_t* row_streams, int32_t* choice_out) {
    if (!logits || !ids || !choice_out) return fail(c, CW_ERR_INVALID, "test_sample_seeded: null argument");
    if (nb < 1 || nb > c->Bm || nb > 64) return fail(c, CW_ERR_INVALID, "test_sample_seeded: nb=%d outside 1 .. %d", nb, c->Bm < 64 ? c->Bm : 64);
    if (max_length <= n_prompt || max_length > c->d.max_target_positions || min_new_tokens < 0)
        return fail(c, CW_ERR_INVALID, "test_sample_seeded: max_length=%d / min_new_tokens=%d out of range", max_length, min_new_tokens);
    if (temperature > 0.f && !row_streams) return fail(c, CW_ERR_INVALID, "test_sample_seeded: a positive temperature needs row_streams");
    const std::vector<unsigned int> keep = c->samp_host;
    CWCHK(c, write_sampling(c, temperature, seed, row_streams, nb, "test_sample_seeded"));
    const int r = test_sample(c, nb, logits, ids, t, n_prompt, min_new_tokens, max_length, choice_out);
    HIPCHK(c, hipStreamSynchronize(c->st));
    HIPCHK(c, hipMemcpy(c->d_samp, keep.data(), keep.size() * 4, hipMemcpyHostToDevice));
    c->samp_host = keep;
    return r;
}
int32_t cw_test_sample_logprobs(cw_ctx* c, int32_t nb, const float* logits, const int32_t* ids, int32_t t, int32_t n_prompt,
                                int32_t min_new_tokens, int32_t max_length, float temperature, uint64_t seed,
                                const uint64_t* row_streams, const int32_t* forced_tok, int32_t* choice_out, float* lp_out) {
    if (!logits || !ids || !choice_out || !lp_out) return fail(c, CW_ERR_INVALID, "test_sample_logprobs: null argument");
    if (nb < 1 || nb > c->Bm || nb > 64) return fail(c, CW_ERR_INVALID, "test_sample_logprobs: nb=%d outside 1 .. %d", nb, c->Bm < 64 ? c->Bm : 64);
    if (max_length <= n_prompt || max_length > c->d.max_target_positions || min_new_tokens < 0)
        return fail(c, CW_ERR_INVALID, "test_sample_logprobs: max_length=%d / min_new_tokens=%d out of range", max_length, min_new_tokens);
    if (temperature > 0.f && !row_streams) return fail(c, CW_ERR_INVALID, "test_sample_logprobs: a positive temperature needs row_streams");
    if (forced_tok)
        for (int b = 0; b < nb; ++b)
            if (forced_tok[b] >= c->d.vocab_size) return fail(c, CW_ERR_INVALID, "test_sample_logprobs: forced token %d out of range", forced_tok[b]);
    const bool was_on = c->tok_lp_on;
    CWCHK(c, cw_set_token_logprobs(c, 1));
    const std::vector<unsigned int> keep = c->samp_host;
    CWCHK(c, write_sampling(c, temperature, seed, row_streams, nb, "test_sample_logprobs"));
    const int r = test_sample(c, nb, logits, ids, t, n_prompt, min_new_tokens, max_length, choice_out, forced_tok, lp_out);
    HIPCHK(c, hipStreamSynchronize(c->st));
    HIPCHK(c, hipMemcpy(c->d_samp, keep.data(), keep.size() * 4, hipMemcpyHostToDevice));
    c->samp_host = keep;
    if (!was_on) CWCHK(c, cw_set_token_logprobs(c, 0));
    return r;
}
int32_t cw_test_sample_top_logprobs(cw_ctx* c, int32_t nb, const float* logits, const int32_t* ids, int32_t t, int32_t n_prompt,
                                    int32_t min_new_tokens, int32_t max_length, float temperature, uint64_t seed,
                                    const uint64_t* row_streams, const int32_t* forced_tok, int32_t k, int32_t* choice_out,
                                    float* lp_out, int32_t* top_id_out, float* top_lp_out) {
    if (!logits || !ids || !choice_out || !lp_out || !top_id_out || !top_lp_out) return fail(c, CW_ERR_INVALID, "test_sample_top_logprobs: null argument");
    if (k < 1 || k > CW_TOP_LOGPROBS_MAX) return fail(c, CW_ERR_INVALID, "test_sample_top_logprobs: k=%d outside 1 .. %d", k, CW_TOP_LOGPROBS_MAX);
    if (nb < 1 || nb > c->Bm || nb > 64) return fail(c, CW_ERR_INVALID, "test_sample_top_logprobs: nb=%d outside 1 .. %d", nb, c->Bm < 64 ? c->Bm : 64);
    if (max_length <= n_prompt || max_length > c->d.max_target_positions || min_new_tokens < 0)
        return fail(c, CW_ERR_INVALID, "test_sample_top_logprobs: max_length=%d / min_new_tokens=%d out of range", max_length, min_new_tokens);
    if (temperature > 0.f && !row_streams) return fail(c, CW_ERR_INVALID, "test_sample_top_logprobs: a positive temperature needs row_streams");
    if (forced_tok)
        for (int b = 0; b < nb; ++b)
            if (forced_tok[b] >= c->d.vocab_size) return fail(c, CW_ERR_INVALID, "test_sample_top_logprobs: forced token %d out of range", forced_tok[b]);
    const bool was_on = c->tok_lp_on;
    const int was_k = c->top_k;
    CWCHK(c, cw_set_token_logprobs(c, 1));
    CWCHK(c, cw_set_top_logprobs(c, k));
    const std::vector<unsigned int> keep = c->samp_host;
    CWCHK(c, write_sampling(c, temperature, seed, row_streams, nb, "test_sample_top_logprobs"));
    const int r = test_sample(c, nb, logits, ids, t, n_prompt, min_new_tokens, max_length, choice_out, forced_tok, lp_out, top_id_out, top_lp_out);
    HIPCHK(c, hipStreamSynchronize(c->st));
    HIPCHK(c, hipMemcpy(c->d_samp, keep.data(), keep.size() * 4, hipMemcpyHostToDevice));
    c->samp_host = keep;
    CWCHK(c, cw_set_top_logprobs(c, was_on ? was_k : 0));
    if (!was_on) CWCHK(c, cw_set_token_logprobs(c, 0));
    return r;
}
int32_t cw_test_sample_biased(cw_ctx* c, int32_t nb, const float* logits, const int32_t* ids, int32_t t, int32_t n_prompt,
                              int32_t min_new_tokens, int32_t max_length, float temperature, uint64_t seed,
                              const uint64_t* row_streams, const int32_t* forced_tok, int32_t k, int32_t n_seq,
                              const int32_t* seq_tokens, const int32_t* seq_lengths, const float* seq_bias, int32_t* choice_out,
                              float* lp_out, int32_t* top_id_out, float* top_lp_out, float* proc_lp_out) {
    if (!proc_lp_out) return fail(c, CW_ERR_INVALID, "test_sample_biased: null argument");
    if (c->beam_K > 0) return fail(c, CW_ERR_STATE, "test_sample_biased: a beam search is open");
    std::vector<int> tab;
// ... 325 lines not shown
```

### crisperwhisper_amd/csrc/engine_internal.h

```cpp
#pragma once
#include <chrono>
#include <hip/hip_runtime.h>
#include <stdarg.h>
#include <stdlib.h>
#include <string.h>
#include <set>
#include <string>
#include <vector>
#include <limits>
#include <functional>
#include <algorithm>

#include "../../include/crisperwhisper.h"
#include "kernels.h"

#pragma GCC visibility push(hidden)

#define KD(c, fn, ...) ((c)->f16 ? cw_f16::fn(__VA_ARGS__) : cw_bf16::fn(__VA_ARGS__))

#define CW_MAX_DEC_STAGES 24
enum DecStageKind { DST_OTHER = 0, DST_QKV_SELF, DST_QKV, DST_SELF_ATTN, DST_O_PROJ, DST_STACK, DST_STACK_CROSS, DST_CROSS_Q, DST_CROSS_ATTN,
                    DST_CROSS_O, DST_FC1, DST_FC2, DST_MLP_PAIR, DST_MLP_CHAIN, DST_N };
static const char* const kDecStageName[DST_N] = {
    "other (A/B path)", "LayerNorm + q/k/v projection + self-attention (qkv_self_kernel)", "LayerNorm + q/k/v projection + cache append",
    "self-attention", "self-attention out-projection", "fused out-projection + cross-query stage (gemv_stack_kernel)",
    "fused stage + cross-attention (dec_layer_a_kernel)", "LayerNorm + cross-attention query projection", "cross-attention",
    "cross-attention out-projection (combines the key-split partials)", "LayerNorm + fc1 + GELU", "fc2", "fc1 + fc2 (mlp_pair_kernel)",
    "LayerNorm + fc1 + GELU + fc2 in one launch (mlp_chain_kernel)"};

struct LayerW {
    void* wqkv = nullptr; float* bqkv = nullptr;
    void *wqkv8 = nullptr, *w18 = nullptr, *w28 = nullptr, *wkv_c8 = nullptr;
    float *sqkv = nullptr, *s1 = nullptr, *s2 = nullptr, *skv_c = nullptr;
    void* wo = nullptr; float* bo = nullptr;
    float *ln1_g = nullptr, *ln1_b = nullptr;
    void* wq_c = nullptr; float* bq_c = nullptr;
    void* wkv_c = nullptr; float* bkv_c = nullptr;
    void* wo_c = nullptr; float* bo_c = nullptr;
    float *lnc_g = nullptr, *lnc_b = nullptr;
    void* w1 = nullptr; float* b1 = nullptr;
    void* w2 = nullptr; float* b2 = nullptr;
    float *ln2_g = nullptr, *ln2_b = nullptr;
    void *ck = nullptr, *cv = nullptr;
    void *ck8 = nullptr, *cv8 = nullptr;
    float* kvs = nullptr;
    void *sk = nullptr, *sv = nullptr;
    void *ws3 = nullptr, *ws5 = nullptr;
    float *qa_bias = nullptr, *q_wsum = nullptr;
    float *u1_bias = nullptr, *u1_wsum = nullptr;
    float* qkv_wsum = nullptr;
};

struct cw_ctx {
    cw_model_desc d;
    bool bf16 = false;
    bool f16 = false;
    int device = 0;
    int Bm = 0, S_pad = 0, Vpad = 0;
    size_t esz = 4;
    hipStream_t st = nullptr;
    hipStream_t st2 = nullptr;
    hipEvent_t ev_pf[2] = {nullptr, nullptr};
    int prefetch = 0;
    unsigned int* d_pf_sink = nullptr;
    std::vector<void*> allocs;
    char err[512] = "";
    bool err_set = false;
    std::vector<int> align_layers, align_heads;
    struct Fold { float* stage; int N, K; void* w_dst; size_t w_off; float* b_dst; size_t b_off; float scale; int layer, which; };
    std::vector<Fold> folds;
    struct OutStage { float* stage; int layer, which; };
    std::vector<OutStage> out_stages;
    bool fuse6_ready = false;
    bool rows_ln_ready = false;
    bool rows_ln_enabled = false;
    bool rows_hilo = true;
    bool mid16 = true;
    bool dtw_block = false;
    bool stack_center = true;
    int skinny_mode = 0;
    float* d_planes = nullptr;
    size_t planes_cap = 0;
    float* d_sk_stats = nullptr;
    float* d_rstats = nullptr;
    bool fuse6_enabled = true;
    bool fuse_mlp = false;
    bool mlp_pair_fence = false;
    bool mlp_pair = false;
    unsigned int* d_bar = nullptr; int* d_err = nullptr;
    int handoff_fallbacks = 0;
    int handoff_resumes = 0;
    long long forwards_since_reset = 0;
    int fail_pos = -1;
    bool declayer = false;
    bool qkv_self = true;
    unsigned long long *d_gq = nullptr, *d_gps = nullptr, *d_gq2 = nullptr, *d_gkv = nullptr, *d_gflag = nullptr;
    bool mlp_chain = false;
    unsigned int* d_epoch = nullptr;
    int n_cu = 0;
    int stack_nt3 = 0, stack_nt5 = 0;
    bool ln_folded = false;
    bool fold_enabled = true;
    std::set<std::string> loaded;
    bool weights_ok = false;
    bool wpacked = false;
    bool wpack_enabled = true;
    bool wnt = true;
    void* embed_pk = nullptr;

    void *conv1_w = nullptr, *conv2_w = nullptr, *embed = nullptr;
    float *conv1_b = nullptr, *conv2_b = nullptr, *enc_pos = nullptr, *dec_pos = nullptr;
    float *enc_ln_g = nullptr, *enc_ln_b = nullptr, *dec_ln_g = nullptr, *dec_ln_b = nullptr;
    std::vector<LayerW> enc, dec;

    MelTables mel{};
    float *d_pcm = nullptr, *d_logspec = nullptr, *d_feats_hf = nullptr;
    unsigned int* d_gmax = nullptr;
    void* d_feats_tm = nullptr;
    std::vector<int> n_frames_items;

    void *c1 = nullptr, *h = nullptr, *qb = nullptr, *kb = nullptr, *vb = nullptr, *ao = nullptr, *mid = nullptr,
         *enc_out = nullptr;
    float* x = nullptr;
    int *d_row_off = nullptr, *d_row_valid = nullptr, *d_row_off2 = nullptr, *d_row_valid2 = nullptr;
    int nb_encoded = 0;

    float *dx = nullptr, *dxn = nullptr, *dq = nullptr, *dattn = nullptr, *dmid = nullptr, *dlogits = nullptr;
    float *dx1 = nullptr, *dx2c = nullptr, *d_qa = nullptr, *d_qb = nullptr, *d_u1 = nullptr, *d_pstats = nullptr;
    float *d_cvec = nullptr, *d_ostats = nullptr;
    bool own_cols = true;
    void *d_xfrag = nullptr, *d_xfrag2 = nullptr;
    int *d_ids = nullptr, *d_forced = nullptr, *d_argmax = nullptr, *d_last_ts = nullptr, *d_finished = nullptr,
        *d_nunf = nullptr, *d_align_slot = nullptr;
    unsigned char* d_mask = nullptr;
    float* d_lp_sum = nullptr; int* d_lp_cnt = nullptr;
    bool score_tokens = false;
    float* d_tok_lp = nullptr;
    bool tok_lp_on = false;
    std::vector<std::vector<float>> tr_lp;
    int top_k = 0;
    int* d_top_id = nullptr; float* d_top_lp = nullptr;
    void* d_top_part = nullptr;
    std::vector<std::vector<int>> tr_top_id;
    std::vector<std::vector<float>> tr_top_lp;
    int* d_seq_bias = nullptr;
    std::vector<int> sb_host;
    int sb_n = 0;
    float logprob_thr = NAN, no_speech_thr = NAN;
    void* d_sample_part = nullptr;
    void* d_sample_pert = nullptr;
    unsigned int* d_samp = nullptr;
    std::vector<unsigned int> samp_host;
    float* d_align = nullptr;
    int align_rows = 0;
    float *d_part_o = nullptr, *d_part_ml = nullptr, *d_align_ml = nullptr;
    bool align_unnormalized = false;
    int* h_nunf = nullptr;
    int *d_pos = nullptr, *d_cfg = nullptr;
    hipGraphExec_t step_graph[130] = {};
    bool hist_short = false;
    bool short_hist_enabled = true;
    bool use_graph = true;
    bool fuse_rows = true;
    bool fuse_beam = true;
    bool fuse_rows8 = true;
    cw_gen_cfg gen{};
    bool gen_set = false;
    bool kv8 = false;
    bool enc8 = false;
    int enc8_mask = 0;
    bool enc8_stale = false;
    void *h8 = nullptr, *mid8 = nullptr; float *sa8 = nullptr, *smid8 = nullptr;
    int beam_K = 0, beam_items = 0, beam_n_prompt = 0;
    int beam_pos = 0, beam_max_len = 0;
    int *d_anc = nullptr, *d_anc_tmp = nullptr, *d_ids_tmp = nullptr, *d_parent = nullptr, *d_tok = nullptr, *d_cand_id = nullptr,
        *d_rowmap = nullptr;
    float *d_cand_val = nullptr, *d_align_g = nullptr, *d_topk_scratch = nullptr;
    const float* align_cur = nullptr;
    float* logits_capture = nullptr;
// ... 47 lines not shown
    int *cut_base = nullptr, *cut_ntok = nullptr, *cut_out = nullptr;
    float* cut_score = nullptr;
    unsigned char *cut_force = nullptr, *cut_ok = nullptr;
    int sc_top_k = 0;
    size_t sc_tparts = 0, sc_alt_rows = 0;
    ScoreTopPart* sc_tpart = nullptr;
    int *sc_alt_id = nullptr, *sc_step_alt_id = nullptr;
    float *sc_alt_lp = nullptr, *sc_step_alt_lp = nullptr;
    std::vector<int32_t> sc_top_ids;
    std::vector<float> sc_top_lps;
    int sc_top_rows = 0, sc_top_stride = 0;
    int stage_kind[CW_MAX_DEC_STAGES] = {};
    int stage_launches[CW_MAX_DEC_STAGES] = {};
    float stage_ms[CW_N_STAGES] = {};
    int stage_calls[CW_N_STAGES] = {};
};

int fail(cw_ctx* c, int code, const char* fmt, ...);
int fail_ctx(cw_ctx* c, int code, const char* call, const char* file, int line);

#define HIPCHK(c, call)                                                                             \
    do {                                                                                            \
        hipError_t e_ = (call);                                                                     \
        if (e_ != hipSuccess) return fail(c, CW_ERR_HIP, "%s failed: %s (%s:%d)", #call,            \
                                          hipGetErrorString(e_), __FILE__, __LINE__);               \
    } while (0)
#define CWCHK(c, call)                                                          \
    do {                                                                        \
        int r_ = (call);                                                        \
        if (r_ != CW_OK) return fail_ctx(c, r_, #call, __FILE__, __LINE__); \
    } while (0)
#define KCHK(c) HIPCHK(c, hipGetLastError())

template <typename P>
static int dmalloc(cw_ctx* c, P** p, size_t bytes, bool zero = true) {
    void* q = nullptr;
    if (bytes == 0) bytes = 16;
    hipError_t e = hipMalloc(&q, bytes);
    if (e != hipSuccess) return fail(c, CW_ERR_NOMEM, "hipMalloc(%zu) failed: %s", bytes, hipGetErrorString(e));
    if (zero) hipMemset(q, 0, bytes);
    c->allocs.push_back(q);
    *p = (P*)q;
    return CW_OK;
}

struct StageTimer {
    cw_ctx* c; int stage;
    StageTimer(cw_ctx* c_, int s) : c(c_), stage(s) { hipEventRecord(c->ev0, c->st); }
    void stop() {
        hipEventRecord(c->ev1, c->st);
        hipEventSynchronize(c->ev1);
        float ms = 0.f;
        hipEventElapsedTime(&ms, c->ev0, c->ev1);
        c->stage_ms[stage] += ms;
        c->stage_calls[stage] += 1;
    }
};

struct DevScope {
    std::vector<void*> ptrs;
    template <typename P> hipError_t get(P** p, size_t bytes) {
        void* q = nullptr;
        const hipError_t e = hipMalloc(&q, bytes ? bytes : 1);
        if (e == hipSuccess) ptrs.push_back(q);
        *p = (P*)q;
        return e;
    }
    ~DevScope() { for (void* q : ptrs) hipFree(q); }
};

int upload_T(cw_ctx* c, void* dst, size_t off, const float* src, size_t n, float scale = 1.0f);
int download_T(cw_ctx* c, const void* src, size_t off, float* dst, size_t n);
extern "C" {
EpiParams epi0();
DecAttnParams dec_attn(const float* q, const void* K, const void* V, int cap, int n_keys, const int* pos, float* out, int B, int H);
int gemv_ln(cw_ctx* c, int epi, const float* x, int Mb, int K, const void* W, int N, const float* g, const float* b, const EpiParams& ep);
int launch_logits(cw_ctx* c, int nb, const float* x);
EpiParams qkv_epi(cw_ctx* c, LayerW& L);
EpiParams cross_q_epi(cw_ctx* c, LayerW& L);
int gemv_resid(cw_ctx* c, bool frag, const float* a, void* xf, int nb, int K, const void* W, const float* bias, float* x, int x16 = 0);
int cross_attn(cw_ctx* c, LayerW& L, CrossSplitParams p);
DecLayerParams dec_layer_params(cw_ctx* c, int l, int nb, const float* xin, float* xalt);
int decode_step(cw_ctx* c, int nb, bool want_logits);
int launch_sample(cw_ctx* c, int nb);
void drop_step_graphs(cw_ctx* c);
int epoch_hygiene(cw_ctx* c, long long upcoming_forwards);
int seq_bias_table(cw_ctx* c, int n_seq, const int32_t* tokens, const int32_t* lengths, const float* bias, std::vector<int>* out, const char* who);
int seq_bias_install(cw_ctx* c, const std::vector<int>& tab, int n_seq);
int write_sampling(cw_ctx* c, float temperature, uint64_t seed, const uint64_t* row_streams, int nb, const char* who);
int check_lang_ids(cw_ctx* c, const char* who, const int32_t* lang_ids, int n_lang);
int language_probs(cw_ctx* c, int nb, const int32_t* lang_ids, int n_lang, int ns_tok, int32_t* best, float* prob, float* no_speech);
int beam_alloc(cw_ctx* c);
int launch_beam_topk(cw_ctx* c, int rows, int n_cand);
}

#pragma GCC visibility pop
```

### crisperwhisper_amd/csrc/kernels.h

```cpp
#pragma once
#include "switches.h"
#include "common.h"

struct AParams {
    const void* A;
    int lda;
    int amode;
    int T_out, C_in, stride;
    const int* row_off;
    const int* row_valid;
};

struct CombineParams;


struct SampleParams {
    const float* logits;
    int V, B, ldv;
    const unsigned char* mask;
    int eos, pad, timestamp_begin, max_initial_timestamp_index;
    const int* cfg;
    int* pos;
    int ids_stride;
    int* ids;
// ... 39 lines not shown
};

struct DecAttnParams {
    const float* q;
    const void* K;
    const void* V;
    int cap;
    int n_keys;
    const int* pos;
    float* out;
    unsigned short* out_frag;
    float* align_out;
    const int* align_slot;
    int n_align, align_rows;
    int B, H;
    int kv_div;
    const int* anc;
    int short_hist;
};

#ifndef ATT_NS
#define ATT_NS 6
#endif
#ifndef CROSS_THREADS
#define CROSS_THREADS 512
#endif
struct CrossSplitParams {
    const float* q;
    const void* K;
    const void* V;
    int n_keys;
    float* part_o;
    float* part_ml;
    float* align_out;
    float* align_ml;
    const int* align_slot;
    const int* pos;
    int n_align, align_rows, B, H;
    const float* kv_scale;
    int kv_div;
    const float* xstat;
    const float* pstats;
    int n_pstats;
    const float* qa;
    const float* qb;
    const float* qw;
    const float* qbias;
    float* a_out;
    void* a_frag;
    int q_planes;
    int q_plane_stride;
};
struct CombineParams {
    const float* part_ml;
    int H;
    int plane;
    const float* pstats;
    int n_pstats;
    float* cvec_out;
};

struct StackSeg {
    const float* x;
    const float* bias;
    const float* wsum;
    const float* resid;
    float* out;
    float* out2;
    float* pstats;
    int tile0, n_tiles;
    int nt;
    int block0;
    int epi;
};
struct StackParams {
    const void* W;
    int wpk;
    int K, Mb, nseg;
    StackSeg seg[3];
    float* zero;
    int zero_n4;
    int wnt;
};
struct Fc2xParams {
    const float* xstat;
    const float* u;
    const float* w1sum;
    const float* b1;
    const void* W2;
    const float* b2;
    float* x;
    int Mb, D, F;
    int wpk;
};

struct MlpPairParams {
    float* x;
    const void* W1;
    const float* b1;
    const void* W2;
    const float* b2;
    void* mid;
    unsigned int* bar;
    int* err;
    int Mb, D, F;
    int wpk;
    int fence;
};

struct RowsParams {
    const void* xf;
    const void* W;
    int Mb, K, N, wpk;
    EpiParams ep;
    const float* ln_pstats;
    int ln_nblk;
    const float* ln_wsum;
    int lo_off;
    void* xf_out;
    float* pstats_out;
};

struct SkinnyParams {
    const float* x;
    const void* xf;
    const void* W;
    int Mb, K, N;
    int Kb;
    float* planes;
    float* stats;
    float* outf;
    const float* bias;
    int ldo;
    int dbg;
};
struct SkinnyFinishParams {
    const float* planes;
    int S, Mb, N;
    const float* x;
    const float* stats;
    int K;
    const float* wsum;
    EpiParams ep;
};

struct DecLayerParams {
    const void* Ws;
    const float* x;
    const float* a;
    const float* qa_bias;
    const float* q_wsum;
    const float* bo;
    float* x1;
    const void* K;
    const void* V;
    int n_keys;
    float* part_o;
    float* part_ml;
    float* align_out;
    float* align_ml;
    const int* align_slot;
    const int* pos;
    int n_align, align_rows;
    const float* qw;
    const float* qbias;
    unsigned long long* gq;
    unsigned long long* gps;
    const unsigned int* epoch;
    int layer;
    int* err;
    int Mb, D, H;
    int kv_wait;
};

struct QkvSelfParams {
    const float* x;
    const void* W;
    const float* bias;
    void* sk;
    void* sv;
    int cap;
    const int* pos;
    float* out;
    float* q_plain;
    int no_attn;
    unsigned long long* gq;
    unsigned long long* gkv;
    const unsigned int* epoch;
    int layer;
    int* err;
    int Mb, D, H;
    int fail_pos;
    int wnt;
};

struct MlpChainParams {
    const float* x;
    const void* W1;
    const float* b1;
    const void* W2;
    const float* b2;
    float* xio;
    void* mid;
    unsigned long long* flags;
    const unsigned int* epoch;
    int layer;
    int* err;
    int Mb, D, F;
    int Kb2;
    int delay;
};

struct MelTables {
    const double* cos_t;
    const double* sin_t;
    const double* window;
    const float* filters;
    const int* fb_lo;
    const int* fb_hi;
    int dbg;
};


enum PrefillMode { PF_STORE = 0, PF_QKV = 1, PF_RESID = 2, PF_GELU = 3 };
struct PrefillEpi {
    int mode;
    const float* bias;
    void* out;
    float* x;
    void* sk; void* sv;
    int D, H, cap, n_pos;
};
struct PrefillAlign {
    float* out;
    float* ml;
    const int* slot;
    int n_align, rows;
};

struct ScorePart {
    float mx, sum;
    float tl;
    float bv; int bi;
};
struct ScoreStopPart {
    float mx, sum;
};
struct ScoreTopPart {
    float v; int i;
};
struct ScoreRowsOut {
    float* logprob; int* top_id; float* top_logprob;
    float* stop_logprob; int eos, ts_begin;
    int k; int* alt_id; float* alt_logprob;
};
struct ScoreHeadOut : ScoreRowsOut {
    ScorePart* part; ScoreStopPart* spart; ScoreTopPart* tpart;
};

#define CW_DTYPE_KERNEL_DECLS \
    int cw_launch_gemm(bool bf16, int epi, const AParams& ap, const void* W, int M, int N, int K, const EpiParams& ep, hipStream_t st); \
    void cw_gemm_set_256_min_tiles(int n); \
    void cw_gemm_set_pp(int on); \
    void cw_gemm_set_8ph(int on); \
    void cw_gemm_set_gm(int gm); \
    void cw_gemm_set_w128(int on); \
    void cw_gemv_set_comb_rowgroups(int on); \
    void cw_gemv_set_mt_variant(int v); \
    void cw_gemv_set_loop(int on); \
    int cw_launch_gemm_w128(int epi, const bf16_t* A, int lda, const bf16_t* W, int M, int N, int K, const EpiParams& ep, int tm2, int tn2, hipStream_t st); \
    void cw_cross_set_valu(int on); \
    void cw_cross_set_per_row(int on); \
    int cw_launch_layernorm_fp8(const float* x, const float* g, const float* b, void* out8, float* scale, int rows, int d, hipStream_t st); \
    int cw_launch_quant_rows_fp8(const void* x, int rows, int K, void* out8, float* scale, hipStream_t st); \
    int cw_launch_gemm_fp8(int epi, const void* A8, int lda, const void* W8, int M, int N, int K, const float* sa, const float* sw, const EpiParams& ep, hipStream_t st); \
    int cw_launch_fold_layernorm(const float* Wf, int N, int K, const float* g, const float* beta, float scale, void* w_out, float* bias, hipStream_t st); \
    int cw_launch_gemv(bool bf16, int epi, const float* x, int Mb, int K, const void* W, int N, const float* ln_g, const float* ln_b, const EpiParams& ep, hipStream_t st, const CombineParams* comb = nullptr, void* scratch = nullptr, bool wpacked = false, bool wnt = false); \
    int cw_gemv_own_nt(int N); \
    int cw_launch_gemv_own(const void* xf, int Mb, int K, const void* W, int N, const EpiParams& ep, const float* cvec, void* xf_out, float* stats_out, hipStream_t st, bool wpacked); \
    int cw_launch_gemv_lna(const void* xf, int Mb, int K, const void* W, int N, const EpiParams& ep, const float* stats_in, int n_stats, const float* wsum, hipStream_t st, bool wpacked); \
    size_t cw_wfrag_elems(int N, int K); \
    int cw_launch_wfrag_pack(const void* src, int N, int K, void* dst, hipStream_t st); \
    int cw_launch_fold_product(const float* A, const float* s, float scale, const float* B, int N, int J, int K, void* C16, hipStream_t st); \
    int cw_launch_fold_rowvec(const float* A, const float* s, float scale, const float* v, const void* W16, int N, int J, float* c_out, float* w_out, hipStream_t st); \
    int cw_launch_gemv_stack(const StackParams& p, int nt, hipStream_t st); \
    int cw_launch_dec_layer(const DecLayerParams& p, int n_cu, hipStream_t st); \
    bool cw_mlp_chain_ok(int Mb, int D, int F); \
    int cw_launch_mlp_chain(const MlpChainParams& p, hipStream_t st); \
    int cw_launch_qkv_self(const QkvSelfParams& p, hipStream_t st); \
    int cw_qkv_self_blocks_per_cu(int D, int cap); \
    size_t cw_dec_layer_lds(int D); \
    int cw_launch_gemv_fc2x(const Fc2xParams& p, hipStream_t st); \
    int cw_launch_mlp_pair(const MlpPairParams& p, hipStream_t st); \
    int cw_launch_gemv_rows(int epi, bool produce, const RowsParams& p, hipStream_t st); \
    int cw_launch_rows_combine(const float* part_o, int Mb, int K, const CombineParams& cb, void* xf, hipStream_t st); \
    int cw_launch_rows_prep(const float* x, int Mb, int K, void* xf, float* pstats, int lo_off, hipStream_t st); \
    int cw_skinny_pick_nks(int N, int K, int s_max); \
    int cw_launch_skinny(int mode, const SkinnyParams& p, int nks, hipStream_t st); \
    int cw_launch_skinny_finish(int epi, const SkinnyFinishParams& p, hipStream_t st); \
    void cw_launch_skinny_empty(hipStream_t st); \
    int cw_launch_layernorm(bool bf16_out, const float* x, const float* g, const float* b, void* out, int rows, int d, hipStream_t st); \
    int cw_launch_layernorm_f32(const float* x, const float* g, const float* b, float* out, int rows, int d, hipStream_t st); \
    int cw_launch_sample(const SampleParams& p, hipStream_t st); \
    int cw_launch_beam_topk(const SampleParams& p, int n_cand, float* cand_val, int* cand_id, float* scratch, hipStream_t st); \
    size_t cw_beam_topk_scratch_floats(int rows); \
    void cw_beam_topk_set_1block(int on); \
    int cw_launch_beam_advance(const BeamAdvanceParams& p, hipStream_t st); \
    int cw_launch_align_gather(const float* align, const int* row_of_pos, int n_items, int n_align, int align_rows, int L, int n_keys, float* out, hipStream_t st); \
    int cw_launch_set_pos(int* pos, int value, int B, hipStream_t st, unsigned int* epoch = nullptr); \
    int cw_launch_embed(const int* ids, int ids_stride, int t, const void* embed, int embed_bf16, const float* pos_embed, float* x_out, int B, int d, hipStream_t st); \
    int cw_launch_prefill_embed(const int* ids, int ids_stride, int n_pos, const void* embed, const float* pos_embed, float* x, int M, int D, hipStream_t st); \
    int cw_launch_prefill_ln(const float* x, void* out, int M, int D, hipStream_t st); \
    int cw_launch_prefill_gemm(const void* A, const void* W, const PrefillEpi& ep, int M, int N, int K, hipStream_t st); \
    int cw_launch_prefill_attn(const void* Q, const void* K, const void* V, void* out, int rows, int n_q, int H, int cap, int n_keys, int causal, int kv_div, hipStream_t st); \
    int cw_launch_prefill_attn_align(const void* Q, const void* K, const void* V, void* out, int rows, int n_q, int H, int cap, int n_keys, int causal, int kv_div, const PrefillAlign& al, hipStream_t st); \
    int cw_launch_score_ln(const float* x, const int* src, const float* g, const float* b, void* out, int M, int D, hipStream_t st); \
    int cw_score_head_splits(int M, int V, int* tiles_per_split); \
    int cw_launch_score_head(const void* A, const void* W, const int* target, int M, int V, int K, const ScoreHeadOut& out, hipStream_t st); \
    int cw_launch_score_head_unfused(const void* A, const void* W, const int* target, float* logits, int ldv, int M, int V, int K, float* logprob, int* top_id, float* top_logprob, hipStream_t st); \
    int cw_launch_score_rows(const float* logits, int ldv, int V, const int* target, int t_stride, int t, int rows, const ScoreRowsOut& out, hipStream_t st); \
    int cw_launch_score_head_store(const void* A, const void* W, const int* target, float* logits, int ldv, int M, int V, int K, hipStream_t st); \
    int cw_launch_attn_encoder(bool bf16, const void* Q, const void* K, const void* V, void* out, int B, int H, int S, int S_pad, hipStream_t st); \
    int cw_launch_attn_decode(bool bf16, const DecAttnParams& p, hipStream_t st); \
    int cw_launch_attn_cross_split(bool bf16, const CrossSplitParams& p, hipStream_t st); \
    int cw_launch_kv_quant_fp8(const void* K, const void* V, void* K8, void* V8, float* kv_scale, int B, int H, int S, hipStream_t st); \
    bool cw_cross8_is_mfma(int n_keys); \
    int cw_launch_attn_cross_split_fp8(const CrossSplitParams& p, hipStream_t st); \
    size_t cw_kv8_v_bytes(int H, int S); \
    int cw_launch_align_normalize(float* align, const float* align_ml, int B, int n_align, int align_rows, int L, int n_keys, hipStream_t st); \
    int cw_launch_mel(const MelTables& t, const float* pcm, int B, int n_mels, float* logspec_tm, unsigned int* gmax, hipStream_t st); \
    int cw_launch_mel_finish(const float* logspec_tm, const unsigned int* gmax, int B, int n_mels, void* feats_tm, int feats_bf16, float* feats_hf, hipStream_t st);
namespace cw_bf16 { CW_DTYPE_KERNEL_DECLS }
namespace cw_f16 { CW_DTYPE_KERNEL_DECLS }

int cw_launch_pcm_to_mono(const void* raw, int fmt, int channels, long long n_frames, float* out, hipStream_t st);
int cw_launch_normalise(float* x, long long n, double* acc2, hipStream_t st);
int cw_launch_resample(const float* x, long long n_in, const float* taps_t, int orig, int nw, int width,
                       long long n_out, float* out, hipStream_t st);

int cw_launch_language_probs(const float* logits, int ldv, int V, const int* lang_ids, int n_lang, int ns_tok, int rows,
                             float* out, hipStream_t st);

int cw_launch_align_stats(const float* w, int B, int Ha, int rows_cap, int S, int row0, int N, const int* n_cols,
                          float* mean, float* stdv, hipStream_t st);
int cw_launch_align_filter(const float* w, int B, int Ha, int rows_cap, int S, int row0, int N, const int* n_cols,
                           const float* mean, const float* stdv, int width, float* mat, hipStream_t st);
int cw_launch_align_similarity(const float* w, int B, int Ha, int rows_cap, int S, int row0, int N, const int* n_cols,
                               const float* ref_begin, const float* ref_end, int clip, float* out, hipStream_t st);
int cw_launch_align_path_score(const float* w, int B, int Ha, int rows_cap, int S, int row0, int N, const int* n_cols,
                               const int* first_col, int collar, float* mass, float* spread, hipStream_t st);
int cw_launch_align_cut(const float* logprob, const float* stop_logprob, const int* base, const int* n_tok,
                        const unsigned char* cut_ok, int ok_stride, const unsigned char* force, int rows, int* cut,
                        float* cut_score, hipStream_t st);
size_t cw_dtw_skew_floats(int B, int N, int S);
int cw_launch_dtw(const float* mat, int B, int N, int S, const int* n_cols, unsigned char* trace, int* first_col,
                  int* path_text, int* path_time, int* path_len, hipStream_t st, float* skew = nullptr);
int cw_launch_pauses(double* start, double* end, int W, double thr, hipStream_t st);
```

### crisperwhisper_amd/csrc/switches.cpp

```cpp
#include "switches.h"
#include <cstdlib>

namespace cw_sw {

static bool flag(const char* name) { return getenv(name) != nullptr; }
static int num(const char* name, int dflt) { const char* v = getenv(name); return v ? atoi(v) : dflt; }

Switches read_switches() {
    Switches s{};
    s.no_graph = flag("CW_NO_GRAPH");
    s.no_ln_fold = flag("CW_NO_LN_FOLD");
    s.no_fuse6 = flag("CW_NO_FUSE6");
    s.rows_ln = flag("CW_ROWS_LN");
    s.no_rows_hilo = flag("CW_NO_ROWS_HILO");
    s.no_stack_center = flag("CW_NO_STACK_CENTER");
    s.no_mid16 = flag("CW_NO_MID16");
    s.dtw_block = flag("CW_DTW_BLOCK");
    s.fuse_mlp = flag("CW_FUSE_MLP");
    s.no_wpack = flag("CW_NO_WPACK");
    s.no_wnt = flag("CW_NO_WNT");
    s.mlp_pair = flag("CW_MLP_PAIR");
    s.mlp_pair_fence = flag("CW_MLP_PAIR_FENCE");
    s.declayer = flag("CW_DECLAYER");
    s.no_qkv_self = flag("CW_NO_QKV_SELF");
    s.mlp_chain = flag("CW_MLP_CHAIN");
    s.no_fuse_rows = flag("CW_NO_FUSE_ROWS");
    s.no_fuse_rows8 = flag("CW_NO_FUSE_ROWS8");
    s.no_fuse_beam = flag("CW_NO_FUSE_BEAM");
    s.no_own_cols = flag("CW_NO_OWN_COLS");
    s.no_short_hist = flag("CW_NO_SHORT_HIST");
    s.skinny = num("CW_SKINNY", 0);
    s.prefetch = num("CW_PREFETCH", 0);
    s.prefetch_wide = num("CW_PREFETCH_WIDE", 0);
    s.prefetch_what = num("CW_PREFETCH_WHAT", 3);
    s.stack_nt3 = num("CW_STACK_NT3", 0);
    s.stack_nt5 = num("CW_STACK_NT5", 0);
    s.attn_v1 = flag("CW_ATTN_V1");
    s.anc_attn_v1 = flag("CW_ANC_ATTN_V1");
    s.cross_per_row = flag("CW_CROSS_PER_ROW");
    s.cross_valu = flag("CW_CROSS_VALU");
    s.cross_no_tr = flag("CW_CROSS_NO_TR");
    s.cross8_valu = flag("CW_CROSS8_VALU");
    s.cross_mfma1 = flag("CW_CROSS_MFMA1");
    s.cross_lds_pad = num("CW_CROSS_LDS_PAD", 0);
    s.cross8_nsb = num("CW_CROSS8_NSB", 0);
    s.dl_depth = num("CW_DL_DEPTH", 16);
    s.dl_kvwait = num("CW_DL_KVWAIT", 0);
    s.mlp_chain_delay = num("CW_MLP_CHAIN_DELAY", 0);
    s.qkv_self_dbg = num("CW_QKV_SELF_DBG", 0);
    s.no_glds = flag("CW_NO_GLDS");
    s.no_gemm256 = flag("CW_NO_GEMM256");
    s.no_gemm_pp = flag("CW_NO_GEMM_PP");
    s.no_gemm_8ph = flag("CW_NO_GEMM_8PH");
    s.gemm_w128 = flag("CW_GEMM_W128");
    s.no_gemv_loop = flag("CW_NO_GEMV_LOOP");
    s.comb_nt2 = flag("CW_COMB_NT2");
    s.comb_no_rowgroups = flag("CW_COMB_NO_ROWGROUPS");
    s.comb_g4 = flag("CW_COMB_G4");
    s.mt_no_prea = flag("CW_MT_NO_PREA");
    s.gemv_loop_cap = num("CW_GEMV_LOOP_CAP", 512);
    s.fc2_ksplit = num("CW_FC2_KSPLIT", 0);
    s.mt_variant = num("CW_MT_VARIANT", -1);
    s.own_nt = num("CW_OWN_NT", 1);
    if (s.mt_variant < -1 || s.mt_variant > 2) s.mt_variant = -1;
    s.beam_topk_1block = flag("CW_BEAM_TOPK_1BLOCK");
    s.mel_valu = flag("CW_MEL_VALU");
    s.mel_dbg = num("CW_MEL_DBG", 0);
    s.test_gemm_reps = num("CW_TEST_GEMM_REPS", 0);
    s.test_attn_reps = num("CW_TEST_ATTN_REPS", 0);
    if (s.gemv_loop_cap < 1) s.gemv_loop_cap = 1;
    if (s.fc2_ksplit < 0) s.fc2_ksplit = 0;
    if (s.cross_lds_pad < 0) s.cross_lds_pad = 0;
    if (s.cross_lds_pad > 150 * 1024) s.cross_lds_pad = 150 * 1024;
    if (s.stack_nt3 < 0 || s.stack_nt3 > 3) s.stack_nt3 = 0;
    if (s.stack_nt5 < 0 || s.stack_nt5 > 3) s.stack_nt5 = 0;
    if (s.prefetch < 0) s.prefetch = 0;
    if (s.mlp_chain_delay < 0 || s.mlp_chain_delay > 4096) s.mlp_chain_delay = 0;
    if (s.test_gemm_reps < 0) s.test_gemm_reps = 0;
    if (s.test_attn_reps < 0) s.test_attn_reps = 0;
    return s;
}

const Switches& cw_switches() {
    static const Switches s = read_switches();
    return s;
}

}
```

### crisperwhisper_amd/csrc/switches.h

```cpp
#pragma once

namespace cw_sw {

struct Switches {
    bool no_graph, no_ln_fold, no_fuse6, rows_ln, no_rows_hilo, no_stack_center, no_mid16, dtw_block, fuse_mlp, no_wpack, no_wnt, mlp_pair, mlp_pair_fence, declayer, no_qkv_self, mlp_chain, no_fuse_rows, no_fuse_rows8, no_fuse_beam, no_own_cols, no_short_hist;
    int skinny, prefetch, prefetch_wide, prefetch_what, stack_nt3, stack_nt5;
    bool attn_v1, anc_attn_v1, cross_per_row, cross_valu, cross_no_tr, cross8_valu, cross_mfma1;
    int cross_lds_pad, cross8_nsb, dl_depth, dl_kvwait, mlp_chain_delay, qkv_self_dbg;
    bool no_glds, no_gemm256, no_gemm_pp, no_gemm_8ph, gemm_w128, no_gemv_loop, comb_nt2, comb_no_rowgroups, mt_no_prea, comb_g4;
    int gemv_loop_cap, fc2_ksplit, mt_variant, own_nt;
    bool beam_topk_1block, mel_valu;
    int mel_dbg;
    int test_gemm_reps, test_attn_reps;
};

const Switches& cw_switches();
Switches read_switches();

}
```

### crisperwhisper_amd/engine.py

```python
from __future__ import annotations

import ctypes as C
import dataclasses
from typing import Dict, List, Optional, Sequence

import numpy as np

from . import _native as N

_GemvEpiArgs = N.GemvEpiArgs


def _ptr(a: Optional[np.ndarray]):
    return None if a is None else a.ctypes.data_as(C.c_void_p)


def _i32(x) -> np.ndarray:
    return np.ascontiguousarray(np.asarray(x, dtype=np.int32))


@dataclasses.dataclass
class ModelSpec:
    d_model: int
    n_heads: int
# ... 917 lines not shown
            if sg.get("pstats") is not None:
                q.pstats_blocks = int(sg.get("pstats_blocks", sg["pstats"].shape[1]))
        if zero is not None:
            assert zero.dtype == np.float32 and zero.flags["C_CONTIGUOUS"] and zero.size % 4 == 0
            a.zero, a.zero_n4 = _ptr(zero), zero.size // 4
        self._chk(self.lib.cw_test_gemv_stack(self.ctx, C.byref(a)))

    def test_gemv_epi(self, *, op=0, epi=0, Mb, N, K, W=None, ldo=None, wpk=False, x16=False, inplace=False, frag_in=False, H=0, cap=0,
                      d_model=0, x=None, bias=None, ln_g=None, ln_b=None, resid=None, part_o=None, part_ml=None, pstats=None,
                      n_pstats=0, pos=None, cvec_in=None, stats_in=None, n_stats=0, wsum=None, out=None, sk=None, sv=None, y=None,
                      stats=None, cvec=None):
        a = _GemvEpiArgs()
        keep = []
        a.op, a.epi, a.Mb, a.N, a.K = int(op), int(epi), int(Mb), int(N), int(K)
        a.ldo = int(N if ldo is None else ldo)
        a.wpk, a.x16, a.inplace, a.frag_in = int(bool(wpk)), int(bool(x16)), int(bool(inplace)), int(bool(frag_in))
        a.H, a.cap, a.d_model, a.n_pstats, a.n_stats = int(H), int(cap), int(d_model), int(n_pstats), int(n_stats)
        for name, t in (("x", x), ("W", W), ("bias", bias), ("ln_g", ln_g), ("ln_b", ln_b), ("resid", resid), ("part_o", part_o),
                        ("part_ml", part_ml), ("pstats", pstats), ("cvec_in", cvec_in), ("stats_in", stats_in), ("wsum", wsum)):
            if t is not None:
                t = np.ascontiguousarray(t, np.float32)
                keep.append(t)
                setattr(a, name, _ptr(t))
        if pos is not None:
            pos = _i32(pos)
            a.pos = _ptr(pos)
        for name, t in (("out", out), ("sk", sk), ("sv", sv), ("y", y), ("stats", stats), ("cvec", cvec)):
            if t is not None:
                assert t.dtype == np.float32 and t.flags["C_CONTIGUOUS"] and t.flags["WRITEABLE"], name
                setattr(a, name, _ptr(t))
        nt, tail = np.zeros(1, np.int32), np.zeros(1, np.int32)
        a.nt, a.frag_tail_ok = _ptr(nt), _ptr(tail)
        self._chk(self.lib.cw_test_gemv_epi(self.ctx, C.byref(a)))
        return {"nt": int(nt[0]), "frag_tail_ok": bool(tail[0])}

    def test_self_attention(self, q, k, v, pos, n_keys=0, anc=None, kv_div=1, short_hist=False, out_frag=False,
                            align_head=-1, align_rows=0, align_init=None):
        q, k, v = (np.ascontiguousarray(t, np.float32) for t in (q, k, v))
        B = q.shape[0]
        H, cap = k.shape[1], k.shape[2]
        pos = _i32(pos)
        a = None if anc is None else _i32(anc)
        out = np.zeros((B, H * 64), np.float32)
        al = None
        if align_head >= 0:
            al = (np.zeros((B, align_rows, n_keys), np.float32) if align_init is None
                  else np.ascontiguousarray(align_init, np.float32).copy())
        tail = np.zeros(1, np.int32)
        self._chk(self.lib.cw_test_self_attention(self.ctx, B, H, cap, int(kv_div), _ptr(q), _ptr(k), _ptr(v), _ptr(pos),
                                                  int(n_keys), _ptr(a), 1 if short_hist else 0, 1 if out_frag else 0,
                                                  int(align_head), int(align_rows), _ptr(out), _ptr(al), _ptr(tail)))
        res = (out,)
        if out_frag:
            res += (bool(tail[0]),)
        if align_head >= 0:
            res += (al,)
        return res[0] if len(res) == 1 else res

    def test_beam_state(self, rows: int):
        tgt = self.spec.max_target_positions
        ids = np.zeros((rows, tgt), np.int32); anc = np.zeros((rows, tgt), np.int32); pos = np.zeros(rows, np.int32)
        self._chk(self.lib.cw_test_beam_state(self.ctx, int(rows), _ptr(ids), _ptr(anc), _ptr(pos)))
        return ids, anc, pos

    def test_beam_topk(self, logits: np.ndarray, ids: np.ndarray, n_prompt: int, n_cand: int, min_new_tokens: int = 0):
        lg = np.ascontiguousarray(logits, np.float32)
        ids = _i32(ids)
        if ids.ndim != 2 or lg.shape != (ids.shape[0], self.spec.vocab_size):
            raise ValueError(f"logits must be [nb][{self.spec.vocab_size}] and ids [nb][t], got {lg.shape} and {ids.shape}")
        nb, t = ids.shape
        val = np.zeros(self.max_batch * 64, np.float32)
        tok = np.zeros(self.max_batch * 64, np.int32)
        self._chk(self.lib.cw_test_beam_topk(self.ctx, nb, _ptr(lg), _ptr(ids), t, int(n_prompt), int(min_new_tokens), int(n_cand),
                                             _ptr(val), _ptr(tok)))
        n = nb * int(n_cand)
        untouched = bool(np.all(val[n:].view(np.uint32) == 0xffffffff) and np.all(tok[n:] == -1))
        return val[:n].reshape(nb, n_cand).copy(), tok[:n].reshape(nb, n_cand).copy(), untouched

    def test_beam_x(self, rows: int) -> np.ndarray:
        x = np.zeros((int(rows), self.spec.d_model), np.float32)
        self._chk(self.lib.cw_test_beam_x(self.ctx, int(rows), _ptr(x)))
        return x

    def test_sample(self, logits: np.ndarray, ids: np.ndarray, n_prompt: int, min_new_tokens: int = 0,
                    max_length: Optional[int] = None) -> np.ndarray:
        lg = np.ascontiguousarray(logits, np.float32)
        ids = _i32(ids)
        nb, t = ids.shape
        out = np.zeros(nb, np.int32)
        self._chk(self.lib.cw_test_sample(self.ctx, nb, _ptr(lg), _ptr(ids), t, int(n_prompt), int(min_new_tokens),
                                          int(max_length or self.spec.max_target_positions), _ptr(out)))
        return out

    def test_sample_seeded(self, logits: np.ndarray, ids: np.ndarray, n_prompt: int, temperature: float, seed: int,
                           row_streams, min_new_tokens: int = 0, max_length: Optional[int] = None) -> np.ndarray:
        lg = np.ascontiguousarray(logits, np.float32)
        ids = _i32(ids)
        nb, t = ids.shape
        if lg.shape != (nb, self.spec.vocab_size):
            raise ValueError(f"logits must be [{nb}][{self.spec.vocab_size}], got {lg.shape}")
        rs = None if row_streams is None else np.ascontiguousarray(row_streams, dtype=np.uint64)
        if rs is not None and rs.shape != (nb,):
            raise ValueError(f"row_streams must hold one id per row ({nb}), got shape {rs.shape}")
        out = np.zeros(nb, np.int32)
        self._chk(self.lib.cw_test_sample_seeded(self.ctx, nb, _ptr(lg), _ptr(ids), t, int(n_prompt), int(min_new_tokens),
                                                 int(max_length or self.spec.max_target_positions), float(temperature),
                                                 int(seed) & (2 ** 64 - 1), _ptr(rs), _ptr(out)))
        return out

    def test_sample_logprobs(self, logits: np.ndarray, ids: np.ndarray, n_prompt: int, temperature: float = 0.0, seed: int = 0,
                             row_streams=None, forced=None, min_new_tokens: int = 0, max_length: Optional[int] = None):
        lg = np.ascontiguousarray(logits, np.float32)
        ids = _i32(ids)
        nb, t = ids.shape
        if lg.shape != (nb, self.spec.vocab_size):
            raise ValueError(f"logits must be [{nb}][{self.spec.vocab_size}], got {lg.shape}")
        rs = None if row_streams is None else np.ascontiguousarray(row_streams, dtype=np.uint64)
        if rs is not None and rs.shape != (nb,):
            raise ValueError(f"row_streams must hold one id per row ({nb}), got shape {rs.shape}")
        fr = None if forced is None else _i32(forced)
        if fr is not None and fr.shape != (nb,):
            raise ValueError(f"forced must hold one token per row ({nb}), got shape {fr.shape}")
        out = np.zeros(nb, np.int32)
        lp = np.zeros(nb, np.float32)
        self._chk(self.lib.cw_test_sample_logprobs(self.ctx, nb, _ptr(lg), _ptr(ids), t, int(n_prompt), int(min_new_tokens),
                                                   int(max_length or self.spec.max_target_positions), float(temperature),
                                                   int(seed) & (2 ** 64 - 1), _ptr(rs), _ptr(fr), _ptr(out), _ptr(lp)))
        return out, lp

    def test_sample_top_logprobs(self, logits: np.ndarray, ids: np.ndarray, n_prompt: int, k: int, temperature: float = 0.0,
                                 seed: int = 0, row_streams=None, forced=None, min_new_tokens: int = 0,
                                 max_length: Optional[int] = None):
        lg = np.ascontiguousarray(logits, np.float32)
        ids = _i32(ids)
        nb, t = ids.shape
        if lg.shape != (nb, self.spec.vocab_size):
            raise ValueError(f"logits must be [{nb}][{self.spec.vocab_size}], got {lg.shape}")
        if not 1 <= int(k) <= 8:
            raise ValueError(f"k must be in 1 .. 8, got {k}")
        rs = None if row_streams is None else np.ascontiguousarray(row_streams, dtype=np.uint64)
        if rs is not None and rs.shape != (nb,):
            raise ValueError(f"row_streams must hold one id per row ({nb}), got shape {rs.shape}")
        fr = None if forced is None else _i32(forced)
        if fr is not None and fr.shape != (nb,):
            raise ValueError(f"forced must hold one token per row ({nb}), got shape {fr.shape}")
        out = np.zeros(nb, np.int32)
        lp = np.zeros(nb, np.float32)
        top_id = np.zeros((nb, int(k)), np.int32)
        top_lp = np.zeros((nb, int(k)), np.float32)
        self._chk(self.lib.cw_test_sample_top_logprobs(self.ctx, nb, _ptr(lg), _ptr(ids), t, int(n_prompt), int(min_new_tokens),
                                                       int(max_length or self.spec.max_target_positions), float(temperature),
                                                       int(seed) & (2 ** 64 - 1), _ptr(rs), _ptr(fr), int(k), _ptr(out), _ptr(lp),
                                                       _ptr(top_id), _ptr(top_lp)))
        return out, lp, top_id, top_lp

    def test_sample_biased(self, logits: np.ndarray, ids: np.ndarray, n_prompt: int, k: int, table=None, temperature: float = 0.0,
                           seed: int = 0, row_streams=None, forced=None, min_new_tokens: int = 0,
                           max_length: Optional[int] = None):
        lg = np.ascontiguousarray(logits, np.float32)
        ids = _i32(ids)
        nb, t = ids.shape
        if lg.shape != (nb, self.spec.vocab_size):
            raise ValueError(f"logits must be [{nb}][{self.spec.vocab_size}], got {lg.shape}")
        if not 1 <= int(k) <= 8:
            raise ValueError(f"k must be in 1 .. 8, got {k}")
        rs = None if row_streams is None else np.ascontiguousarray(row_streams, dtype=np.uint64)
# ... 44 lines not shown
```

### include/crisperwhisper.h

```cpp
#ifndef CRISPERWHISPER_H
#define CRISPERWHISPER_H

#include <stdint.h>

#ifdef __cplusplus
extern "C" {
#endif

typedef struct cw_ctx cw_ctx;

#define CW_DTYPE_F32 0
#define CW_DTYPE_BF16 1
#define CW_DTYPE_F16 2

#define CW_N_SAMPLES 480000
#define CW_N_FRAMES 3000
#define CW_N_CTX 1500

typedef struct {
    int32_t d_model, n_heads, ffn_dim, enc_layers, dec_layers, n_mels, vocab_size;
    int32_t max_target_positions;
    int32_t median_filter_width;
    int32_t dtype;
    int32_t max_batch;
// ... 220 lines not shown
int32_t cw_test_score_rows_top(cw_ctx* ctx, int32_t rows, int32_t V, int32_t ldv, const float* logits, const int32_t* targets,
                               int32_t k, int32_t eos, int32_t timestamp_begin, float* logprob, int32_t* top_id,
                               float* top_logprob, float* stop_logprob, int32_t* alt_id, float* alt_logprob);
int32_t cw_time_score_head_top(cw_ctx* ctx, int32_t M, int32_t k, int32_t stop, int32_t iters, float* avg_ms);
int32_t cw_test_prefill_gemm(cw_ctx* ctx, int32_t mode, int32_t M, int32_t N, int32_t K, const float* A, const float* W,
                             const float* bias, float* out);
int32_t cw_test_prefill_attention(cw_ctx* ctx, int32_t rows, int32_t n_q, int32_t H, int32_t cap, int32_t n_keys, int32_t causal,
                                  int32_t kv_div, const float* q, const float* k, const float* v, float* out);
int32_t cw_test_prefill_align_attention(cw_ctx* ctx, int32_t rows, int32_t n_q, int32_t H, int32_t n_keys, int32_t kv_div,
                                        int32_t align_head, const float* q, const float* k, const float* v, float* out,
                                        float* align);
int32_t cw_test_cross_attention(cw_ctx* ctx, int32_t B, int32_t H, int32_t S, int32_t kv_div, const float* q, const float* k,
                                const float* v, int32_t align_head, float* part_o, float* part_ml, float* align,
                                float* align_ml);
int32_t cw_test_cross_attention_fused(cw_ctx* ctx, int32_t B, int32_t H, int32_t S, int32_t kv_div, const float* qa,
                                      const float* qb, const float* qw, const float* qbias, const float* pstats,
                                      int32_t n_pstats, const float* k, const float* v, int32_t align_head, float* part_o,
                                      float* part_ml, float* align, float* align_ml);
typedef struct cw_test_fold_args {
    int32_t op, N, J, K;
    float scale;
    const float* a;
    const float* s;
    const float* v;
    const float* w16;
    float* out16;
    float* c_out;
    float* w_out;
    uint16_t* image;
} cw_test_fold_args;
int32_t cw_test_fold(cw_ctx* ctx, const cw_test_fold_args* args);
typedef struct cw_test_stack_seg {
    const float* x;
    const float* bias;
    const float* wsum;
    const float* resid;
    int32_t n_tiles, nt, epi, pstats_blocks;
    float* out;
    float* out2;
    float* pstats;
} cw_test_stack_seg;
typedef struct cw_test_gemv_stack_args {
    int32_t Mb, K, nt, wpk, nseg;
    const float* W;
    cw_test_stack_seg seg[3];
    float* zero;
    int32_t zero_n4;
} cw_test_gemv_stack_args;
int32_t cw_test_gemv_stack(cw_ctx* ctx, const cw_test_gemv_stack_args* args);
typedef struct cw_test_gemv_epi_args {
    int32_t op, epi, Mb, N, K, ldo, wpk, x16, inplace, frag_in;
    int32_t H, cap, d_model, n_pstats, n_stats;
    const float* x;
    const float* W;
    const float* bias;
    const float* ln_g;
    const float* ln_b;
    const float* resid;
    const float* part_o;
    const float* part_ml;
    const float* pstats;
    const int32_t* pos;
    const float* cvec_in;
    const float* stats_in;
    const float* wsum;
    float* out;
    float* sk;
    float* sv;
    float* y;
    float* stats;
    float* cvec;
    int32_t* nt;
    int32_t* frag_tail_ok;
} cw_test_gemv_epi_args;
int32_t cw_test_gemv_epi(cw_ctx* ctx, const cw_test_gemv_epi_args* args);
int32_t cw_test_self_attention(cw_ctx* ctx, int32_t B, int32_t H, int32_t cap, int32_t kv_div, const float* q, const float* k,
                               const float* v, const int32_t* pos, int32_t n_keys, const int32_t* anc, int32_t short_hist,
                               int32_t out_frag, int32_t align_head, int32_t align_rows, float* out, float* align,
                               int32_t* frag_tail_ok);
int32_t cw_test_beam_state(cw_ctx* ctx, int32_t rows, int32_t* ids, int32_t* anc, int32_t* pos);
int32_t cw_test_beam_topk(cw_ctx* ctx, int32_t nb, const float* logits, const int32_t* ids, int32_t t, int32_t n_prompt,
                          int32_t min_new_tokens, int32_t n_cand, float* cand_val, int32_t* cand_id);
int32_t cw_test_beam_x(cw_ctx* ctx, int32_t rows, float* x);
int32_t cw_test_sample(cw_ctx* ctx, int32_t nb, const float* logits, const int32_t* ids, int32_t t, int32_t n_prompt,
                       int32_t min_new_tokens, int32_t max_length, int32_t* choice_out);
int32_t cw_test_sample_seeded(cw_ctx* ctx, int32_t nb, const float* logits, const int32_t* ids, int32_t t, int32_t n_prompt,
                              int32_t min_new_tokens, int32_t max_length, float temperature, uint64_t seed,
                              const uint64_t* row_streams, int32_t* choice_out);
int32_t cw_test_sample_logprobs(cw_ctx* ctx, int32_t nb, const float* logits, const int32_t* ids, int32_t t, int32_t n_prompt,
                                int32_t min_new_tokens, int32_t max_length, float temperature, uint64_t seed,
                                const uint64_t* row_streams, const int32_t* forced_tok, int32_t* choice_out, float* lp_out);
int32_t cw_test_sample_top_logprobs(cw_ctx* ctx, int32_t nb, const float* logits, const int32_t* ids, int32_t t, int32_t n_prompt,
                                    int32_t min_new_tokens, int32_t max_length, float temperature, uint64_t seed,
                                    const uint64_t* row_streams, const int32_t* forced_tok, int32_t k, int32_t* choice_out,
                                    float* lp_out, int32_t* top_id_out, float* top_lp_out);
int32_t cw_test_sample_biased(cw_ctx* ctx, int32_t nb, const float* logits, const int32_t* ids, int32_t t, int32_t n_prompt,
                              int32_t min_new_tokens, int32_t max_length, float temperature, uint64_t seed,
                              const uint64_t* row_streams, const int32_t* forced_tok, int32_t k, int32_t n_seq,
                              const int32_t* seq_tokens, const int32_t* seq_lengths, const float* seq_bias, int32_t* choice_out,
                              float* lp_out, int32_t* top_id_out, float* top_lp_out, float* proc_lp_out);

#define CW_STAGE_MEL 0
#define CW_STAGE_ENCODER 1
#define CW_STAGE_CROSS_KV 2
#define CW_STAGE_DECODE 3
#define CW_STAGE_TIMESTAMPS 4
#define CW_N_STAGES 5
int32_t cw_stage_times(cw_ctx* ctx, float* ms , int32_t* calls , int32_t reset);
int32_t cw_time_kernel(cw_ctx* ctx, int32_t which, int32_t nb, int32_t iters, float* avg_ms, double* algo_bytes);
int32_t cw_time_decode_stage(cw_ctx* ctx, int32_t nb, int32_t stage, int32_t iters, float* avg_ms, double* algo_bytes,
                             int32_t* kind, int32_t* n_stages);
const char* cw_decode_stage_name(int32_t kind);
int32_t cw_decode_stage_launches(cw_ctx* ctx, int32_t stage);
int32_t cw_handoff_fallbacks(cw_ctx* ctx);
int32_t cw_handoff_resumes(cw_ctx* ctx);

#ifdef __cplusplus
}
#endif
#endif
```

Measured before the change: 789.7.

## Fold cross-attention query projection into fused QKV self-attention kernel

Adds an XQ variant of the fused QKV/self-attention kernel in which the V-tile blocks also compute the next cross-attention query projection. They layer-normalise the residual input, optionally mean-centre it, and run a second MFMA GEMV with the cross-Q weights. The attention output is also written as bf16, and a new stack GEMV consumes that bf16 activation directly, fusing the output projection with residual add and layernorm partial stats. The goal is to remove a separate query-projection launch and an fp32 to bf16 conversion per decoder layer. In exchange it adds register and LDS pressure to those blocks and a tighter validity constraint on batch×heads, with an env or config switch to turn it off.

```diff
diff --git a/crisperwhisper_amd/_native.py b/crisperwhisper_amd/_native.py
--- a/crisperwhisper_amd/_native.py
+++ b/crisperwhisper_amd/_native.py
@@ -179,6 +179,7 @@
     "cw_time_score_head": (_I, [_P, _I, _I, _I, _P]),
     "cw_test_beam_topk": (_I, [_P, _I, _P, _P, _I, _I, _I, _I, _P, _P]),
     "cw_test_beam_x": (_I, [_P, _I, _P]),
+    "cw_test_decode_state": (_I, [_P, _I, _I, _I, _I, _P]),
     "cw_test_sample": (_I, [_P, _I, _P, _P, _I, _I, _I, _I, _P]),
     "cw_test_sample_seeded": (_I, [_P, _I, _P, _P, _I, _I, _I, _I, C.c_float, C.c_uint64, _P, _P]),
     "cw_test_sample_logprobs": (_I, [_P, _I, _P, _P, _I, _I, _I, _I, C.c_float, C.c_uint64, _P, _P, _P, _P]),
diff --git a/crisperwhisper_amd/csrc/decfuse.hip b/crisperwhisper_amd/csrc/decfuse.hip
--- a/crisperwhisper_amd/csrc/decfuse.hip
+++ b/crisperwhisper_amd/csrc/decfuse.hip
@@ -309,6 +309,117 @@
     return launch_stack_nt<2, 3>(p, st);
 }
 
+template <int NSLOT, int PL16, bool WNT>
+__global__ __launch_bounds__(256) void gemv_stack_a16_kernel(const void* __restrict__ Wp, const void* a16, const float* resid, const float* bias, unsigned dims,
+                                                             StackA16Out p) {
+    extern __shared__ __attribute__((aligned(16))) unsigned char smem_a[];
+    const int K = (int)(dims & 0xffffu), Mb = (int)(dims >> 16), TD = K >> 4;
+    const int xs_stride = K + 8;
+    bf16_t* xs = (bf16_t*)smem_a;
+    float* red = (float*)(smem_a + (size_t)16 * xs_stride * 2);
+    const int tid = threadIdx.x, lane = tid & 63;
+    const int wave = __builtin_amdgcn_readfirstlane(tid >> 6);
+    const int l15 = lane & 15, g = lane >> 4;
+    const int bid = blockIdx.x;
+    const bool seg_x1 = bid >= TD;
+    const int tl = seg_x1 ? bid - TD : bid;
+    const int steps = K >> 7, nv8 = K >> 3;
+    const int n = tl * 16 + l15;
+    const float bias_ld = bias[n];
+    const float resid_pre = resid[(size_t)min(g * 4 + wave, Mb - 1) * K + n];
+    u32x4_t av[2][PL16];
+#pragma unroll
+    for (int i = 0; i < 2; ++i) {
+        int row = wave + 4 * i;
+        row = row < Mb ? row : Mb - 1;
+#pragma unroll
+        for (int c = 0; c < PL16; ++c) {
+            int v8 = lane + 64 * c;
+            v8 = v8 < nv8 ? v8 : nv8 - 1;
+            av[i][c] = *(const u32x4_t*)((const bf16_t*)a16 + (size_t)row * K + v8 * 8);
+        }
+    }
+    __builtin_amdgcn_sched_barrier(0);
+    u32x4_t wq[NSLOT][4];
+    const bf16_t* __restrict__ W = (const bf16_t*)Wp;
+#pragma unroll
+    for (int s = 0; s < NSLOT; ++s) {
+        int step = wave + 4 * s;
+        step = step < steps ? step : steps - 1;
+        const u32x4_t* wp = (const u32x4_t*)(W + ((((size_t)(TD + bid) * (K >> 5)) + step * 4) * 64 + lane) * 8);
+#pragma unroll
+        for (int j = 0; j < 4; ++j) wq[s][j] = WNT ? CW_STREAM_LD(wp + j * 64) : wp[j * 64];
+    }
+    __builtin_amdgcn_sched_barrier(0);
+#pragma unroll
+    for (int i = 0; i < 2; ++i) {
+        const int row = wave + 4 * i;
+#pragma unroll
+        for (int c = 0; c < PL16; ++c) {
+            int v8 = lane + 64 * c;
+            v8 = v8 < nv8 ? v8 : nv8 - 1;
+            *(u32x4_t*)(xs + (size_t)row * xs_stride + v8 * 8) = av[i][c];
+        }
+    }
+    float bias_v = bias_ld, resid_v = resid_pre;
+    asm volatile("" : "+v"(bias_v), "+v"(resid_v));
+    __syncthreads();
+    f32x4_t acc = (f32x4_t){0.f, 0.f, 0.f, 0.f};
+#pragma unroll
+    for (int s = 0; s < NSLOT; ++s) {
+        const int step = wave + 4 * s, stepc = step < steps ? step : steps - 1;
+        const bf16_t* xr = xs + (size_t)l15 * xs_stride + stepc * 128 + g * 8;
+        f32x4_t nacc = acc;
+#pragma unroll
+        for (int j = 0; j < 4; ++j) {
+            bf16x8_t a = *(const bf16x8_t*)(xr + j * 32);
+            nacc = mfma16x(a, __builtin_bit_cast(bf16x8_t, wq[s][j]), nacc);
+        }
+        acc = step < steps ? nacc : acc;
+    }
+#pragma unroll
+    for (int r = 0; r < 4; ++r) red[(wave * 4 + r) * 64 + lane] = acc[r];
+    __syncthreads();
+    const int r = tid >> 6;
+    const float v = red[(0 * 4 + r) * 64 + lane] + red[(1 * 4 + r) * 64 + lane] + red[(2 * 4 + r) * 64 + lane] + red[(3 * 4 + r) * 64 + lane];
+    const int m = g * 4 + r;
+    const size_t o = (size_t)m * K + n;
+    if (!seg_x1) {
+        if (m < Mb) p.qb[o] = v + 0.f + 0.f;
+        return;
+    }
+    float ps1 = 0.f, ps2 = 0.f;
+    if (m < Mb) {
+        const float rv = resid_v + resid_grid(v + bias_v);
+        p.x1[o] = rv;
+        ps1 += rv; ps2 += rv * rv;
+    }
+#pragma unroll
+    for (int sft = 0; sft < 4; ++sft) {
+        ps1 += sft == 0 ? dpp_mov<0x111, 0xf>(0.f, ps1) : sft == 1 ? dpp_mov<0x112, 0xf>(0.f, ps1) : sft == 2 ? dpp_mov<0x114, 0xf>(0.f, ps1) : dpp_mov<0x118, 0xf>(0.f, ps1);
+        ps2 += sft == 0 ? dpp_mov<0x111, 0xf>(0.f, ps2) : sft == 1 ? dpp_mov<0x112, 0xf>(0.f, ps2) : sft == 2 ? dpp_mov<0x114, 0xf>(0.f, ps2) : dpp_mov<0x118, 0xf>(0.f, ps2);
+    }
+    if (l15 == 15) *(float2*)(p.pstats + ((size_t)tl * 16 + m) * 2) = make_float2(ps1, ps2);
+}
+
+int cw_launch_gemv_stack_a16(const StackA16Params& p, hipStream_t st) {
+    if (p.Mb < 1 || p.Mb > 8 || p.K % 128 || p.K < 128 || p.K > 1280 || !p.W || !p.a16 || !p.resid || !p.bias || !p.qb || !p.x1 || !p.pstats) return CW_ERR_INVALID;
+    const size_t lds = (size_t)16 * (p.K + 8) * 2 + (size_t)4 * 4 * 64 * 4;
+    const dim3 grid(2 * (p.K / 16));
+    const unsigned dims = (unsigned)p.K | (unsigned)p.Mb << 16;
+    const StackA16Out out{p.qb, p.x1, p.pstats};
+#define CW_A16_LAUNCH(NS, PL)                                                                                                        \
+    do {                                                                                                                              \
+        if (p.wnt) hipLaunchKernelGGL((gemv_stack_a16_kernel<NS, PL, true>), grid, dim3(256), lds, st, p.W, p.a16, p.resid, p.bias, dims, out);  \
+        else hipLaunchKernelGGL((gemv_stack_a16_kernel<NS, PL, false>), grid, dim3(256), lds, st, p.W, p.a16, p.resid, p.bias, dims, out);       \
+    } while (0)
+    if (p.K <= 256) CW_A16_LAUNCH(1, 1);
+    else if (p.K <= 768) CW_A16_LAUNCH(2, 2);
+    else CW_A16_LAUNCH(3, 3);
+#undef CW_A16_LAUNCH
+    return CW_OK;
+}
+
 #ifdef CW_EXPERIMENTS
 #include "decfuse_experiments.inc"
 #else
diff --git a/crisperwhisper_amd/csrc/declayer.hip b/crisperwhisper_amd/csrc/declayer.hip
--- a/crisperwhisper_amd/csrc/declayer.hip
+++ b/crisperwhisper_amd/csrc/declayer.hip
@@ -430,16 +430,202 @@
 #undef DL_KV_LOAD
 #endif
 
+template <int NSLOT, int PER_LANE, bool WNT>
+__device__ __forceinline__ void qs_vtile_xq_block(const float* __restrict__ x, const void* __restrict__ Wp, const float* __restrict__ bias,
+                                                  void* sv, const int* __restrict__ pos, int Mb, int H, int K, int cap,
+                                                  const QkvSelfParams& p, unsigned char* qsm) {
+    const int xs_stride = K + 8;
+    bf16_t* xs = (bf16_t*)qsm;
+    float* red = (float*)(qsm + (size_t)16 * xs_stride * 2);
+    float* smean = red + 4 * 4 * 64;
+    const int tid = threadIdx.x, lane = tid & 63;
+    const int wave = __builtin_amdgcn_readfirstlane(tid >> 6);
+    const int l15 = lane & 15, g = lane >> 4;
+    const int bid = blockIdx.x;
+    const int steps = K >> 7, nvec = K >> 2;
+    const int nn = bid * 16 + l15;
+    const int tx = bid - 2 * (K >> 4), nx = tx * 16 + l15;
+    float bias_v = 0.f, xbias_v = 0.f, xwsum_v = 0.f;
+    int pos_m = 0;
+    float4 xv[2][PER_LANE];
+    dl_u32x4_t wq[NSLOT][4], wx[NSLOT][4];
+    if (wave < 4) {
+        pos_m = pos[min(g * 4 + wave, Mb - 1)];
+        bias_v = bias ? bias[nn] : 0.f;
+#pragma unroll
+        for (int i = 0; i < 2; ++i) {
+            int row = wave + 4 * i;
+            row = row < Mb ? row : Mb - 1;
+#pragma unroll
+            for (int c = 0; c < PER_LANE; ++c) {
+                int v4 = lane + 64 * c;
+                v4 = v4 < nvec ? v4 : nvec - 1;
+                xv[i][c] = *(const float4*)(x + (size_t)row * K + v4 * 4);
+            }
+        }
+        const bf16_t* __restrict__ W = (const bf16_t*)Wp;
+#pragma unroll
+        for (int s = 0; s < NSLOT; ++s) {
+            int step = wave + 4 * s;
+            step = step < steps ? step : steps - 1;
+            const dl_u32x4_t* wp = (const dl_u32x4_t*)(W + ((((size_t)bid * (K >> 5)) + step * 4) * 64 + lane) * 8);
+#pragma unroll
+            for (int j = 0; j < 4; ++j) wq[s][j] = WNT ? CW_STREAM_LD(wp + j * 64) : wp[j * 64];
+        }
+        __builtin_amdgcn_sched_barrier(0);
+        const bf16_t* __restrict__ WX = (const bf16_t*)p.xq_W;
+#pragma unroll
+        for (int s = 0; s < NSLOT; ++s) {
+            int step = wave + 4 * s;
+            step = step < steps ? step : steps - 1;
+            const dl_u32x4_t* wp = (const dl_u32x4_t*)(WX + ((((size_t)tx * (K >> 5)) + step * 4) * 64 + lane) * 8);
+#pragma unroll
+            for (int j = 0; j < 4; ++j) wx[s][j] = WNT ? CW_STREAM_LD(wp + j * 64) : wp[j * 64];
+        }
+        xbias_v = p.xq_bias[nx];
+        xwsum_v = (p.xq_wsum ? p.xq_wsum : p.xq_bias)[nx];
+    }
+    __builtin_amdgcn_sched_barrier(0);
+    const unsigned tag = (p.epoch[0] << 6) | (unsigned)p.layer;
+    const bool center = p.xq_wsum != nullptr;
+    asm volatile("" : "+v"(pos_m));
+
+    if (wave < 4) {
+#pragma unroll
+        for (int i = 0; i < 2; ++i) {
+            float sx = 0.f;
+#pragma unroll
+            for (int c = 0; c < PER_LANE; ++c) {
+                const float ok = (lane + 64 * c < nvec) ? 1.f : 0.f;
+                sx += ok * ((xv[i][c].x + xv[i][c].y) + (xv[i][c].z + xv[i][c].w));
+            }
+            const float mean = wave_sum(sx) / (float)K;
+            float q = 0.f;
+#pragma unroll
+            for (int c = 0; c < PER_LANE; ++c) {
+                const float ok = (lane + 64 * c < nvec) ? 1.f : 0.f;
+                const float a = xv[i][c].x - mean, b = xv[i][c].y - mean, cc = xv[i][c].z - mean, d = xv[i][c].w - mean;
+                q += ok * cw_sumsq4(a, b, cc, d);
+            }
+            const float rstd = 1.0f / sqrtf(wave_sum(q) / (float)K + 1e-5f);
+            const int row = wave + 4 * i;
+#pragma unroll
+            for (int c = 0; c < PER_LANE; ++c) {
+                int v4 = lane + 64 * c;
+                v4 = v4 < nvec ? v4 : nvec - 1;
+                ushort4 o;
+                o.x = f32_to_bf16((xv[i][c].x - mean) * rstd); o.y = f32_to_bf16((xv[i][c].y - mean) * rstd);
+                o.z = f32_to_bf16((xv[i][c].z - mean) * rstd); o.w = f32_to_bf16((xv[i][c].w - mean) * rstd);
+                *(ushort4*)(xs + (size_t)row * xs_stride + v4 * 4) = o;
+            }
+        }
+    }
+    dl_barrier();
+    if (wave < 4) {
+        f32x4_t acc = (f32x4_t){0.f, 0.f, 0.f, 0.f};
+#pragma unroll
+        for (int s = 0; s < NSLOT; ++s) {
+            const int step = wave + 4 * s;
+            if (step < steps) {
+                const bf16_t* xr = xs + (size_t)l15 * xs_stride + step * 128 + g * 8;
+#pragma unroll
+                for (int j = 0; j < 4; ++j) {
+                    const bf16x8_t a = *(const bf16x8_t*)(xr + j * 32);
+                    acc = cw_mfma_16x16x32(a, __builtin_bit_cast(bf16x8_t, wq[s][j]), acc);
+                }
+            }
+        }
+#pragma unroll
+        for (int r = 0; r < 4; ++r) red[(wave * 4 + r) * 64 + lane] = acc[r];
+    }
+    dl_barrier();
+    if (wave < 4) {
+        const int r = wave;
+        const float v = (red[(0 * 4 + r) * 64 + lane] + red[(1 * 4 + r) * 64 + lane] + red[(2 * 4 + r) * 64 + lane] + red[(3 * 4 + r) * 64 + lane]) + bias_v;
+        const int m = g * 4 + r;
+        const int rc = nn - 2 * K;
+        const unsigned h16 = f32_to_bf16(v);
+        const unsigned other = (unsigned)__shfl_xor((int)h16, 1, 64);
+        if (m < Mb) {
+            const int hh = rc >> 6, dd = rc & 63;
+            if (!(l15 & 1)) dl_gran_st(p.gkv + ((size_t)16 + m) * (K >> 1) + (rc >> 1), tag, h16 | (other << 16));
+            ((bf16_t*)sv)[(((size_t)m * H + hh) * cap + pos_m) * 64 + dd] = (bf16_t)h16;
+        }
+        if (center) {
+#pragma unroll
+            for (int i = 0; i < 2; ++i) {
+                float sx = 0.f, sq = 0.f;
+#pragma unroll
+                for (int c = 0; c < PER_LANE; ++c)
+                    if (lane + 64 * c < nvec) {
+                        sx += (xv[i][c].x + xv[i][c].y) + (xv[i][c].z + xv[i][c].w);
+                        sq += cw_sumsq4(xv[i][c].x, xv[i][c].y, xv[i][c].z, xv[i][c].w);
+                    }
+                float mu = wave_sum(sx) / (float)K;
+                if (2.f * mu * mu < wave_sum(sq) / (float)K) mu = 0.f;
+#pragma unroll
+                for (int c = 0; c < PER_LANE; ++c) { xv[i][c].x -= mu; xv[i][c].y -= mu; xv[i][c].z -= mu; xv[i][c].w -= mu; }
+                if (lane == 0) smean[wave + 4 * i] = mu;
+            }
+        }
+#pragma unroll
+        for (int i = 0; i < 2; ++i) {
+            const int row = wave + 4 * i;
+#pragma unroll
+            for (int c = 0; c < PER_LANE; ++c) {
+                int v4 = lane + 64 * c;
+                v4 = v4 < nvec ? v4 : nvec - 1;
+                const float4 v = xv[i][c];
+                ushort4 o;
+                o.x = f32_to_bf16(v.x); o.y = f32_to_bf16(v.y); o.z = f32_to_bf16(v.z); o.w = f32_to_bf16(v.w);
+                *(ushort4*)(xs + (size_t)row * xs_stride + v4 * 4) = o;
+            }
+        }
+    }
+    dl_barrier();
+    if (wave < 4) {
+        f32x4_t acc = (f32x4_t){0.f, 0.f, 0.f, 0.f};
+#pragma unroll
+        for (int s = 0; s < NSLOT; ++s) {
+            const int step = wave + 4 * s;
+            if (step < steps) {
+                const bf16_t* xr = xs + (size_t)l15 * xs_stride + step * 128 + g * 8;
+#pragma unroll
+                for (int j = 0; j < 4; ++j) {
+                    const bf16x8_t a = *(const bf16x8_t*)(xr + j * 32);
+                    acc = cw_mfma_16x16x32(a, __builtin_bit_cast(bf16x8_t, wx[s][j]), acc);
+                }
+            }
+        }
+#pragma unroll
+        for (int r = 0; r < 4; ++r) red[(wave * 4 + r) * 64 + lane] = acc[r];
+    }
+    dl_barrier();
+    if (wave < 4) {
+        const int r = wave;
+        const float v = red[(0 * 4 + r) * 64 + lane] + red[(1 * 4 + r) * 64 + lane] + red[(2 * 4 + r) * 64 + lane] + red[(3 * 4 + r) * 64 + lane];
+        const int m = g * 4 + r;
+        if (m < Mb) {
+            const float back = center ? smean[m] * xwsum_v : 0.f;
+            p.xq_out[(size_t)m * K + nx] = v + xbias_v + back;
+        }
+    }
+}
+
 #define QS_THREADS 512
 #define QS_GROUPS (QS_THREADS / 8)
 #define QS_PRE 2
 
-template <int NSLOT, int PER_LANE, bool WNT>
+template <int NSLOT, int PER_LANE, bool WNT, bool XQ>
 __global__ __launch_bounds__(QS_THREADS) void qkv_self_kernel(const float* __restrict__ x, const void* __restrict__ Wp,
                                                               const float* __restrict__ bias, void* sk, void* sv,
                                                               const int* __restrict__ pos, unsigned dims, int cap, QkvSelfParams p) {
     extern __shared__ __attribute__((aligned(16))) unsigned char qsm[];
     const int Mb = (int)(dims & 0xffu), H = (int)((dims >> 8) & 0xffu), K = (int)(dims >> 16), N = 3 * K;
+    if (XQ && (int)blockIdx.x >= 2 * (K >> 4)) {
+        qs_vtile_xq_block<NSLOT, PER_LANE, WNT>(x, Wp, bias, sv, pos, Mb, H, K, cap, p, qsm);
+        return;
+    }
     const int xs_stride = K + 8;
     bf16_t* xs = (bf16_t*)qsm;
     float* red = (float*)(qsm + (size_t)16 * xs_stride * 2);
@@ -658,6 +844,7 @@
             for (int w = 0; w < QS_THREADS / 64; ++w) { r += red8[w * 64 + tid]; l += red8[8 * 64 + w]; }
             r *= 1.0f / l;
             p.out[(size_t)ib * H * 64 + ih * 64 + tid] = r;
+            if (XQ) ((bf16_t*)p.out16)[(size_t)ib * H * 64 + ih * 64 + tid] = f32_to_bf16(r);
         }
         return;
     }
@@ -742,6 +929,7 @@
         float r = 0.f;
         for (int gI = 0; gI < QS_GROUPS; ++gI) r += redd[gI * 64 + tid];
         p.out[(size_t)ib * H * 64 + ih * 64 + tid] = r;
+        if (XQ) ((bf16_t*)p.out16)[(size_t)ib * H * 64 + ih * 64 + tid] = f32_to_bf16(r);
     }
 }
 
@@ -756,17 +944,22 @@
     if (p.Mb < 1 || p.Mb > 8 || D % 128 || D > 1280 || p.H * 64 != D || p.cap < 1 || p.cap > 512) return CW_ERR_INVALID;
     if (p.Mb * p.H > 3 * (D / 16) || !p.gq || !p.gkv || !p.epoch || !p.err || !p.W || !p.x || !p.pos) return CW_ERR_INVALID;
     if (p.layer < 0 || p.layer >= 64) return CW_ERR_INVALID;
+    if (p.xq_W && (!p.xq_out || !p.xq_bias || !p.out16 || p.no_attn || p.Mb * p.H > 2 * (D / 16))) return CW_ERR_INVALID;
     const size_t lds = (size_t)16 * (D + 8) * 2 + (size_t)(4 * 4 * 64 + 64) * 4 + 2 * 64 * 2 +
                        ((size_t)((p.cap + 63) & ~63) + QS_GROUPS * 64 + 64) * 4;
     const dim3 grid(3 * (D / 16));
-#define QS_LAUNCH_P(NS, PL, NTL)                                                                                            \
+#define QS_LAUNCH_P(NS, PL, NTL, XQ)                                                                                            \
     do {                                                                                                                     \
         static std::once_flag attr;                                                                                          \
-        std::call_once(attr, [] { (void)hipFuncSetAttribute((const void*)qkv_self_kernel<NS, PL, NTL>, hipFuncAttributeMaxDynamicSharedMemorySize, 100 * 1024); }); \
-        hipLaunchKernelGGL((qkv_self_kernel<NS, PL, NTL>), grid, dim3(QS_THREADS), lds, st, p.x, p.W, p.bias, p.sk, p.sv, p.pos, \
+        std::call_once(attr, [] { (void)hipFuncSetAttribute((const void*)qkv_self_kernel<NS, PL, NTL, XQ>, hipFuncAttributeMaxDynamicSharedMemorySize, 100 * 1024); }); \
+        hipLaunchKernelGGL((qkv_self_kernel<NS, PL, NTL, XQ>), grid, dim3(QS_THREADS), lds, st, p.x, p.W, p.bias, p.sk, p.sv, p.pos, \
                            (unsigned)p.Mb | (unsigned)p.H << 8 | (unsigned)D << 16, p.cap, p);                                \
     } while (0)
-#define QS_LAUNCH(NS, PL) do { if (p.wnt) QS_LAUNCH_P(NS, PL, true); else QS_LAUNCH_P(NS, PL, false); } while (0)
+#define QS_LAUNCH(NS, PL)                                                                                                   \
+    do {                                                                                                                     \
+        if (p.xq_W) { if (p.wnt) QS_LAUNCH_P(NS, PL, true, true); else QS_LAUNCH_P(NS, PL, false, true); }                   \
+        else { if (p.wnt) QS_LAUNCH_P(NS, PL, true, false); else QS_LAUNCH_P(NS, PL, false, false); }                        \
+    } while (0)
     if (D <= 256) QS_LAUNCH(1, 1);
     else if (D <= 768) QS_LAUNCH(2, 3);
     else QS_LAUNCH(3, 5);
diff --git a/crisperwhisper_amd/csrc/engine.hip b/crisperwhisper_amd/csrc/engine.hip
--- a/crisperwhisper_amd/csrc/engine.hip
+++ b/crisperwhisper_amd/csrc/engine.hip
@@ -158,6 +158,7 @@
     c->mlp_pair_fence = sw.mlp_pair_fence;
     c->declayer = sw.declayer;
     c->qkv_self = !sw.no_qkv_self;
+    c->xq_in_qkv = !sw.no_xq_in_qkv;
     c->mlp_chain = sw.mlp_chain;
     c->stack_nt3 = sw.stack_nt3;
     c->stack_nt5 = sw.stack_nt5;
@@ -302,6 +303,7 @@
         CWCHK(c, dmalloc(c, &c->d_gq, (size_t)2 * 16 * D * 8)); CWCHK(c, dmalloc(c, &c->d_gps, (size_t)(D / 16) * 16 * 2 * 8));
         CWCHK(c, dmalloc(c, &c->d_gq2, (size_t)16 * D * 8)); CWCHK(c, dmalloc(c, &c->d_gkv, (size_t)2 * 16 * (D / 2) * 8));
         CWCHK(c, dmalloc(c, &c->d_gflag, (size_t)512 * 8));
+        CWCHK(c, dmalloc(c, &c->d_attn16, (size_t)8 * D * 2));
         CWCHK(c, dmalloc(c, &c->d_epoch, 4));
         const unsigned int one = 1;
         HIPCHK(c, hipMemcpy(c->d_epoch, &one, 4, hipMemcpyHostToDevice));
@@ -812,7 +814,7 @@
 }
 
 struct StepPlan {
-    bool frag, fuse, own, qs, short_hist, mid16; int nt3;
+    bool frag, fuse, own, qs, xq, short_hist, mid16; int nt3;
 #ifdef CW_EXPERIMENTS
     bool fuse_mlp, mlp_pair, mlp_chain, dl, sk_ok, skinny, xfull, rows, pf; int lo_off;
 #else
@@ -833,6 +835,7 @@
     P.nt3 = c->stack_nt3 > 0 ? c->stack_nt3 : (nb > 16 ? 2 : 1);
     P.qs = c->qkv_self && c->bf16 && c->ln_folded && c->wpacked && nb <= 8 && c->beam_K == 0 && D <= 1280 && nb * H <= 3 * (D / 16) && TGT <= 512 &&
            c->d.dec_layers <= 64 && 3 * (D / 16) <= c->n_cu * KD(c, cw_qkv_self_blocks_per_cu, D, TGT);
+    P.xq = c->xq_in_qkv && P.qs && P.fuse && P.nt3 == 1 && cw_sw::cw_switches().qkv_self_dbg == 0 && !c->fuse_mlp && !c->declayer && !c->mlp_pair && !c->mlp_chain;
     P.short_hist = c->hist_short && c->short_hist_enabled && nb > 8;
     P.mid16 = P.fuse && !P.frag && F > 1280 && c->mid16;
 #ifdef CW_EXPERIMENTS
@@ -850,6 +853,7 @@
 #endif
     return P;
 }
+bool step_plan_xq(const cw_ctx* c, int nb) { return plan_step(c, nb).xq; }
 static int stage_launches(const StepPlan& P, int kind) {
     const bool prepared = kind == DST_QKV || kind == DST_CROSS_Q || kind == DST_FC1 || kind == DST_CROSS_O, owned = P.own && (kind == DST_FC1 || kind == DST_CROSS_O);
     return (P.frag && !P.skinny && !P.rows && !P.xfull && prepared && !owned) ? 2 : 1;
@@ -917,6 +921,7 @@
     qp.gq = c->d_gq2; qp.gkv = c->d_gkv; qp.epoch = c->d_epoch; qp.layer = l; qp.err = c->d_err; qp.Mb = nb; qp.D = D; qp.H = H; qp.fail_pos = c->fail_pos; qp.wnt = c->wnt ? 1 : 0;
     const int dbg = cw_sw::cw_switches().qkv_self_dbg;
     if (dbg) { qp.q_plain = c->dq; qp.no_attn = 1; }
+    if (P.xq) { qp.xq_W = L.ws3; qp.xq_bias = L.qa_bias; qp.xq_wsum = c->stack_center ? L.q_wsum : nullptr; qp.xq_out = c->d_qa; qp.out16 = c->d_attn16; }
     STG(DST_QKV_SELF, KD(c, cw_launch_qkv_self, qp, c->st));
     if (dbg) STG(DST_SELF_ATTN, self_attn(c, P, L, nb));
     return CW_OK;
@@ -935,7 +940,11 @@
 static int layer_fused(cw_ctx* c, const StepPlan& P, int l, int nb, float*& xin, float*& xalt) {
     const int D = c->d.d_model, H = c->d.n_heads, F = c->d.ffn_dim;
     LayerW& L = c->dec[l];
-    STG(DST_STACK, KD(c, cw_launch_gemv_stack, stack_params(c, L, nb, xin, xalt), P.nt3, c->st));
+    if (P.xq) {
+        StackA16Params sp = zeroed<StackA16Params>();
+        sp.W = L.ws3; sp.a16 = c->d_attn16; sp.resid = xin; sp.bias = L.bo; sp.qb = c->d_qb; sp.x1 = xalt; sp.pstats = c->d_pstats; sp.K = D; sp.Mb = nb; sp.wnt = c->wnt ? 1 : 0;
+        STG(DST_STACK, KD(c, cw_launch_gemv_stack_a16, sp, c->st));
+    } else STG(DST_STACK, KD(c, cw_launch_gemv_stack, stack_params(c, L, nb, xin, xalt), P.nt3, c->st));
     const CrossSplitParams p = cross_params(c, P, L, l, nb, nullptr);
     STG(DST_CROSS_ATTN, cross_attn(c, L, p));
     if (P.own) {
@@ -3050,6 +3059,11 @@
         drop_step_graphs(c);
         return CW_OK;
     }
+    if (!strcmp(name, "no_xq_in_qkv")) {
+        c->xq_in_qkv = value == 0;
+        drop_step_graphs(c);
+        return CW_OK;
+    }
     if (!strcmp(name, "rows_ln")) {
         c->rows_ln_enabled = value != 0;
         drop_step_graphs(c);
diff --git a/crisperwhisper_amd/csrc/engine_hooks.hip b/crisperwhisper_amd/csrc/engine_hooks.hip
--- a/crisperwhisper_amd/csrc/engine_hooks.hip
+++ b/crisperwhisper_amd/csrc/engine_hooks.hip
@@ -1397,6 +1397,22 @@
     if (rows < 1 || rows > c->Bm || !x) return fail(c, CW_ERR_INVALID, "test_beam_x: rows=%d", rows);
     HIPCHK(c, hipStreamSynchronize(c->st));
     HIPCHK(c, hipMemcpy(x, c->dx, (size_t)rows * c->d.d_model * 4, hipMemcpyDeviceToHost));
+    return CW_OK;
+}
+
+int32_t cw_test_decode_state(cw_ctx* c, int32_t what, int32_t layer, int32_t rows, int32_t n_pos, void* out) {
+    const int D = c->d.d_model, H = c->d.n_heads, TGT = c->d.max_target_positions;
+    if (!out || rows < 1 || rows > c->Bm || what < 0 || what > 3) return fail(c, CW_ERR_INVALID, "test_decode_state: what=%d rows=%d", what, rows);
+    if (what == 3) { *(int32_t*)out = step_plan_xq(c, rows) ? 1 : 0; return CW_OK; }
+    HIPCHK(c, hipStreamSynchronize(c->st));
+    if (what == 0) {
+        HIPCHK(c, hipMemcpy(out, c->d_qa, (size_t)rows * D * 4, hipMemcpyDeviceToHost));
+        return CW_OK;
+    }
+    if (layer < 0 || layer >= c->d.dec_layers || n_pos < 1 || n_pos > TGT) return fail(c, CW_ERR_INVALID, "test_decode_state: layer=%d n_pos=%d", layer, n_pos);
+    const void* src = what == 1 ? c->dec[layer].sk : c->dec[layer].sv;
+    const size_t row_bytes = (size_t)64 * c->esz;
+    HIPCHK(c, hipMemcpy2D(out, (size_t)n_pos * row_bytes, src, (size_t)TGT * row_bytes, (size_t)n_pos * row_bytes, (size_t)rows * H, hipMemcpyDeviceToHost));
     return CW_OK;
 }
 
diff --git a/crisperwhisper_amd/csrc/engine_internal.h b/crisperwhisper_amd/csrc/engine_internal.h
--- a/crisperwhisper_amd/csrc/engine_internal.h
+++ b/crisperwhisper_amd/csrc/engine_internal.h
@@ -95,6 +95,8 @@
     bool declayer = false;
     bool qkv_self = true;
     unsigned long long *d_gq = nullptr, *d_gps = nullptr, *d_gq2 = nullptr, *d_gkv = nullptr, *d_gflag = nullptr;
+    bool xq_in_qkv = true;
+    void* d_attn16 = nullptr;
     bool mlp_chain = false;
     unsigned int* d_epoch = nullptr;
     int n_cu = 0;
@@ -308,6 +310,7 @@
 int cross_attn(cw_ctx* c, LayerW& L, CrossSplitParams p);
 DecLayerParams dec_layer_params(cw_ctx* c, int l, int nb, const float* xin, float* xalt);
 int decode_step(cw_ctx* c, int nb, bool want_logits);
+bool step_plan_xq(const cw_ctx* c, int nb);
 int launch_sample(cw_ctx* c, int nb);
 void drop_step_graphs(cw_ctx* c);
 int epoch_hygiene(cw_ctx* c, long long upcoming_forwards);
diff --git a/crisperwhisper_amd/csrc/kernels.h b/crisperwhisper_amd/csrc/kernels.h
--- a/crisperwhisper_amd/csrc/kernels.h
+++ b/crisperwhisper_amd/csrc/kernels.h
@@ -145,6 +145,18 @@
     int zero_n4;
     int wnt;
 };
+struct StackA16Params {
+    const void* W;
+    const void* a16;
+    const float* resid;
+    const float* bias;
+    float* qb;
+    float* x1;
+    float* pstats;
+    int K, Mb;
+    int wnt;
+};
+struct StackA16Out { float *qb, *x1, *pstats; };
 struct Fc2xParams {
     const float* xstat;
     const float* u;
@@ -255,6 +267,11 @@
     int Mb, D, H;
     int fail_pos;
     int wnt;
+    const void* xq_W;
+    const float* xq_bias;
+    const float* xq_wsum;
+    float* xq_out;
+    void* out16;
 };
 
 struct MlpChainParams {
@@ -347,6 +364,7 @@
     int cw_launch_fold_product(const float* A, const float* s, float scale, const float* B, int N, int J, int K, void* C16, hipStream_t st); \
     int cw_launch_fold_rowvec(const float* A, const float* s, float scale, const float* v, const void* W16, int N, int J, float* c_out, float* w_out, hipStream_t st); \
     int cw_launch_gemv_stack(const StackParams& p, int nt, hipStream_t st); \
+    int cw_launch_gemv_stack_a16(const StackA16Params& p, hipStream_t st); \
     int cw_launch_dec_layer(const DecLayerParams& p, int n_cu, hipStream_t st); \
     bool cw_mlp_chain_ok(int Mb, int D, int F); \
     int cw_launch_mlp_chain(const MlpChainParams& p, hipStream_t st); \
diff --git a/crisperwhisper_amd/csrc/switches.cpp b/crisperwhisper_amd/csrc/switches.cpp
--- a/crisperwhisper_amd/csrc/switches.cpp
+++ b/crisperwhisper_amd/csrc/switches.cpp
@@ -29,6 +29,7 @@
     s.no_fuse_beam = flag("CW_NO_FUSE_BEAM");
     s.no_own_cols = flag("CW_NO_OWN_COLS");
     s.no_short_hist = flag("CW_NO_SHORT_HIST");
+    s.no_xq_in_qkv = flag("CW_NO_XQ_IN_QKV");
     s.skinny = num("CW_SKINNY", 0);
     s.prefetch = num("CW_PREFETCH", 0);
     s.prefetch_wide = num("CW_PREFETCH_WIDE", 0);
diff --git a/crisperwhisper_amd/csrc/switches.h b/crisperwhisper_amd/csrc/switches.h
--- a/crisperwhisper_amd/csrc/switches.h
+++ b/crisperwhisper_amd/csrc/switches.h
@@ -3,7 +3,7 @@
 namespace cw_sw {
 
 struct Switches {
-    bool no_graph, no_ln_fold, no_fuse6, rows_ln, no_rows_hilo, no_stack_center, no_mid16, dtw_block, fuse_mlp, no_wpack, no_wnt, mlp_pair, mlp_pair_fence, declayer, no_qkv_self, mlp_chain, no_fuse_rows, no_fuse_rows8, no_fuse_beam, no_own_cols, no_short_hist;
+    bool no_graph, no_ln_fold, no_fuse6, rows_ln, no_rows_hilo, no_stack_center, no_mid16, dtw_block, fuse_mlp, no_wpack, no_wnt, mlp_pair, mlp_pair_fence, declayer, no_qkv_self, mlp_chain, no_fuse_rows, no_fuse_rows8, no_fuse_beam, no_own_cols, no_short_hist, no_xq_in_qkv;
     int skinny, prefetch, prefetch_wide, prefetch_what, stack_nt3, stack_nt5;
     bool attn_v1, anc_attn_v1, cross_per_row, cross_valu, cross_no_tr, cross8_valu, cross_mfma1;
     int cross_lds_pad, cross8_nsb, dl_depth, dl_kvwait, mlp_chain_delay, qkv_self_dbg;
diff --git a/crisperwhisper_amd/engine.py b/crisperwhisper_amd/engine.py
--- a/crisperwhisper_amd/engine.py
+++ b/crisperwhisper_amd/engine.py
@@ -1023,6 +1023,17 @@
         self._chk(self.lib.cw_test_beam_x(self.ctx, int(rows), _ptr(x)))
         return x
 
+    def test_decode_state(self, what: str, rows: int, layer: int = 0, n_pos: int = 1) -> np.ndarray:
+        code = {"qa": 0, "k": 1, "v": 2, "xq_plan": 3}[what]
+        if code == 3:
+            out = np.zeros(1, np.int32)
+        elif code == 0:
+            out = np.zeros((int(rows), self.spec.d_model), np.float32)
+        else:
+            out = np.zeros((int(rows), self.spec.n_heads, int(n_pos), 64), np.float32 if self.dtype == "f32" else np.uint16)
+        self._chk(self.lib.cw_test_decode_state(self.ctx, code, int(layer), int(rows), int(n_pos), _ptr(out)))
+        return out
+
     def test_sample(self, logits: np.ndarray, ids: np.ndarray, n_prompt: int, min_new_tokens: int = 0,
                     max_length: Optional[int] = None) -> np.ndarray:
         lg = np.ascontiguousarray(logits, np.float32)
diff --git a/include/crisperwhisper.h b/include/crisperwhisper.h
--- a/include/crisperwhisper.h
+++ b/include/crisperwhisper.h
@@ -326,6 +326,7 @@
 int32_t cw_test_beam_topk(cw_ctx* ctx, int32_t nb, const float* logits, const int32_t* ids, int32_t t, int32_t n_prompt,
                           int32_t min_new_tokens, int32_t n_cand, float* cand_val, int32_t* cand_id);
 int32_t cw_test_beam_x(cw_ctx* ctx, int32_t rows, float* x);
+int32_t cw_test_decode_state(cw_ctx* ctx, int32_t what, int32_t layer, int32_t rows, int32_t n_pos, void* out);
 int32_t cw_test_sample(cw_ctx* ctx, int32_t nb, const float* logits, const int32_t* ids, int32_t t, int32_t n_prompt,
                        int32_t min_new_tokens, int32_t max_length, int32_t* choice_out);
 int32_t cw_test_sample_seeded(cw_ctx* ctx, int32_t nb, const float* logits, const int32_t* ids, int32_t t, int32_t n_prompt,
```

After: 807.6 (median of 6 runs). 2.3% higher.
